# Iamdarika/Spotify_recommender

Hardware: AMD Instinct MI355X
Metric: queries/sec, cosine top-100 over a 10M x 12 fp32 catalogue (higher is better)
Workload: dtype f32 (every score is the exact fp32 chain; a 12 B/row 8-bit replica only rules rows out); 1 GPU; 10000000 synthetic tracks x 12 fp32 features, top-100, 1 MI355X (BASELINE configs[2], HBM-roofline run); rows=10000000, topn=100, rows_per_gpu=10000000, lanes=2, seed=12345, generator=torch.rand(seed) uniform[0,1) on device

## Files before the change

### include/mi355rec_diag.h

```cpp
#ifndef MI355REC_DIAG_H
#define MI355REC_DIAG_H

#include "mi355rec.h"

#ifdef __cplusplus
extern "C" {
#endif

typedef struct {
    int64_t rows;
    int64_t row_base;
    int32_t device;
    int32_t compute_units;
    int32_t grid_blocks;
    int32_t block_threads;
    int64_t bytes_per_query;
    float last_scan_ms;
    float last_merge_ms;
    float last_pass_ms;
    int32_t batched_grid_blocks;
    float batched_margin;
    int64_t replica_bytes_per_query;
    int32_t replica_active;
    int32_t replica_grid_blocks;
    float replica_build_ms;
    float replica_margin_single;
    float replica_margin_multi;
    int64_t replica_single_bytes_per_query;
    int32_t replica_single_row_bytes;
    int32_t lone_fused_queries;
    int64_t route_fp32;
    int64_t route_fp16;
    int64_t route_q8;
    int64_t route_q8_lone;
    int64_t route_multi_fp32;
    int64_t route_multi_fp16;
    int64_t route_multi_q8;
    int64_t route_mfma_two_pass;
    int64_t route_exact_queue;
    int32_t device_bytes_per_row;
    int64_t stream_pair_launches;
} mi355rec_stats_t;

#define MI355REC_BUILD_EXPERIMENTS 1
#define MI355REC_BUILD_PHASE_CLOCK 2
#define MI355REC_BUILD_TEST_HOOKS 4
int mi355rec_build_flags(void);

int mi355rec_device_count(void);

const char* mi355rec_last_global_error(void);

#define MI355REC_CREATE_NO_REPLICA 1
int mi355rec_create_ex(const float* feats_host, int64_t n, int dim, int device, int64_t row_base, int flags,
                       mi355rec_t** out);
int mi355rec_create_device_ex(const float* feats_dev, int64_t n, int dim, int device, int64_t row_base, int flags,
                              mi355rec_t** out);

#define MI355REC_REPLICA_AUTO 0
#define MI355REC_REPLICA_OFF 1
#define MI355REC_REPLICA_ON 2
#define MI355REC_REPLICA_FP16 3
int mi355rec_set_replica(mi355rec_t* h, int mode);
int mi355rec_rebuild_replica(mi355rec_t* h);
int mi355rec_replica_counters(mi355rec_t* h, int64_t* scans, int64_t* rescored_rows);

#define MI355REC_SAMPLE_AUTO 0
#define MI355REC_SAMPLE_STRIDED 1
#define MI355REC_SAMPLE_BUCKETED 2
#define MI355REC_SAMPLE_AUTO_MIN_ROWS 6000000
int mi355rec_set_sample(mi355rec_t* h, int mode);

#define MI355REC_PAIRING_AUTO 0
#define MI355REC_PAIRING_OFF 1
#define MI355REC_PAIRING_ON 2
#define MI355REC_PAIRING_AUTO_MIN_ROWS 2500000
int mi355rec_set_stream_pairing(mi355rec_t* h, int mode);
typedef struct {
    int64_t base_rows;
    int32_t regions;
    int32_t centroids;
    int64_t bytes;
    int64_t stride_rows;
    int64_t centroid_stride;
    int32_t picks;
    int32_t mode;
    int32_t last_used;
    float build_ms;
} mi355rec_bucket_sample_info_t;
int mi355rec_bucket_sample_info(const mi355rec_t* h, mi355rec_bucket_sample_info_t* out);
int mi355rec_bucket_sample_rows(mi355rec_t* h, int32_t* rows_out, int32_t* region_tab_out);

int mi355rec_lane_status(const mi355rec_t* h, int* stream_attempts, int* overlaps_parent);

int mi355rec_stats(const mi355rec_t* h, mi355rec_stats_t* out);
int mi355rec_stats_sized(const mi355rec_t* h, void* out, size_t out_size, size_t* written);


int mi355rec_scores_row(mi355rec_t* h, int64_t local_row, float* out_host);

int mi355rec_scores(mi355rec_t* h, const float* query12, float* out_host);

int mi355rec_row_ptr(mi355rec_t* h, int64_t local_row, const float** out_dev);
int mi355rec_enqueue_ptr_keys(mi355rec_t* h, const float* query12_dev, int64_t exclude_global, int topn,
                              mi355rec_key_t* out_keys_dev, int64_t* out_idx_dev, float* out_score_dev,
                              void* stream);
int mi355rec_enqueue_ptr_keys_streamed(mi355rec_t* h, const float* query12_dev, int64_t exclude_global,
                                       int topn, mi355rec_key_t* out_keys_dev, void* stream);

int mi355rec_batch_pointers_ok(const mi355rec_t* h, int topn);
int mi355rec_enqueue_batch_mixed_keys(mi355rec_t* h, const float* queries, const float* const* query_ptrs_dev,
                                      const int64_t* exclude_global, int batch, int topn,
                                      mi355rec_key_t* out_keys_dev, void* stream);
int mi355rec_enqueue_batch_mixed_keys_streamed(mi355rec_t* h, const float* queries, const float* const* query_ptrs_dev,
                                               const int64_t* exclude_global, int batch, int topn,
                                               mi355rec_key_t* out_keys_dev, void* stream);

#define MI355REC_BATCH_AUTO 0
#define MI355REC_BATCH_MULTI 1
#define MI355REC_BATCH_MFMA 2
#define MI355REC_BATCH_HALF 3
#define MI355REC_BATCH_Q8 4
int mi355rec_batched_pass2_pairs(mi355rec_t* h, int64_t* pairs_done, int64_t* pairs_total);

#define MI355REC_BATCH_MFMA_NOSKIP 5
int mi355rec_set_batch_path(mi355rec_t* h, int path);

int mi355rec_batched_last_counters(mi355rec_t* h, int32_t* special_rows,
                                   int32_t* queued_queries, int64_t* candidates_total,
                                   int32_t* candidates_max);

int mi355rec_enqueue_merge_keys(mi355rec_t* h, const mi355rec_key_t* lists_dev,
                                int n_lists, int list_len, int topn,
                                mi355rec_key_t* out_keys_dev,
                                int64_t* out_idx_dev, float* out_score_dev,
                                void* stream);

int mi355rec_enqueue_merge_keys_batch(mi355rec_t* h, const mi355rec_key_t* lists_dev,
                                      int n_lists, int list_len, int64_t list_stride,
                                      int64_t query_stride, int batch, int topn,
                                      mi355rec_key_t* out_keys_dev, int64_t* out_idx_dev,
                                      float* out_score_dev, void* stream);

int mi355rec_enqueue_scores(mi355rec_t* h, int64_t local_row,
                            const float* query12, float* out_scores_dev,
                            void* stream);

int mi355rec_enqueue_stream_probe(mi355rec_t* h, uint32_t* sink_dev, void* stream);
#define MI355REC_PROBE_FP32_ROWS 0
#define MI355REC_PROBE_FP16_REPLICA 1
#define MI355REC_PROBE_Q8_REPLICA 2
int mi355rec_enqueue_stream_probe_of(mi355rec_t* h, int which, uint32_t* sink_dev, void* stream);

int mi355rec_set_timing(mi355rec_t* h, int enabled);

int mi355rec_fetch_row(mi355rec_t* h, int64_t local_row, float* out12_host);
int mi355rec_fetch_rows(mi355rec_t* h, const int64_t* local_rows, int64_t count, float* out_host);


int mi355rec_create_sharded(const float* feats_host, int64_t n, int dim, int n_devices,
                            mi355rec_sharded_t** out);
int mi355rec_auto_shards(int64_t n, int visible_devices);
int mi355rec_sharded_placement(const mi355rec_sharded_t* h);

int mi355rec_create_sharded_on(const float* feats_host, int64_t n, int dim, const int* devices,
                               int n_shards, mi355rec_sharded_t** out);

int mi355rec_sharded_set_transport(mi355rec_sharded_t* h, int transport);

int mi355rec_sharded_info(const mi355rec_sharded_t* h, int* n_shards, int* transport,
                          int64_t* rows, int* devices_out, int64_t* shard_rows_out);

int mi355rec_sharded_set_timing(mi355rec_sharded_t* h, int enabled);
int mi355rec_sharded_shard_stats(const mi355rec_sharded_t* h, int shard, mi355rec_stats_t* out);
int mi355rec_sharded_set_replica(mi355rec_sharded_t* h, int mode);

int mi355rec_sharded_rows_by_pointer(const mi355rec_sharded_t* h);
const char* mi355rec_sharded_note(const mi355rec_sharded_t* h);

int mi355rec_sharded_scores_row(mi355rec_sharded_t* h, int64_t global_row, float* out_host);

int mi355rec_sharded_set_window(mi355rec_sharded_t* h, int window);
int mi355rec_sharded_set_window_mode(mi355rec_sharded_t* h, int batched);
int mi355rec_sharded_stream_stats(const mi355rec_sharded_t* h, int64_t* queries, int64_t* exchanges,
                                  int64_t* host_ns);

int mi355rec_sharded_rccl_ranks(const mi355rec_sharded_t* h, int* comms, int* ranks, int* ranks_agree);

#define MI355REC_MAX_LABELS 1024
int mi355rec_set_labels(mi355rec_t* h, const int32_t* labels_host, int64_t n);
int mi355rec_query_row_topn_labels(mi355rec_t* h, int64_t local_row, const int32_t* labels, int n_labels, int topn,
                                   int64_t* out_idx, float* out_score, int* out_count);
int mi355rec_query_topn_labels(mi355rec_t* h, const float* query12, int64_t exclude_global, const int32_t* labels,
                               int n_labels, int topn, int64_t* out_idx, float* out_score, int* out_count);
int mi355rec_label_counters(const mi355rec_t* h, int64_t* queries, int64_t* rows_scanned);
int mi355rec_sharded_set_labels(mi355rec_sharded_t* h, const int32_t* labels_host, int64_t n);
int mi355rec_sharded_query_row_topn_labels(mi355rec_sharded_t* h, int64_t global_row, const int32_t* labels, int n_labels,
                                           int topn, int64_t* out_idx, float* out_score, int* out_count);
int mi355rec_sharded_query_topn_labels(mi355rec_sharded_t* h, const float* query12, int64_t exclude_global,
                                       const int32_t* labels, int n_labels, int topn, int64_t* out_idx, float* out_score,
                                       int* out_count);

#define MI355REC_MAX_PLAYLIST 32
#define MI355REC_MAX_EXCLUDE 1024
int mi355rec_query_mean_topn(mi355rec_t* h, const float* queries, int k, const int64_t* exclude_global, int n_exclude, int topn,
                             int64_t* out_idx, float* out_score, int* out_count);
int mi355rec_query_playlist_topn(mi355rec_t* h, const int64_t* local_rows, int k, const int64_t* exclude_global, int n_exclude,
                                 int topn, int64_t* out_idx, float* out_score, int* out_count);
int mi355rec_playlist_counters(const mi355rec_t* h, int64_t* queries, int64_t* rows_exact);
int mi355rec_sharded_query_mean_topn(mi355rec_sharded_t* h, const float* queries, int k, const int64_t* exclude_global,
                                     int n_exclude, int topn, int64_t* out_idx, float* out_score, int* out_count);
int mi355rec_sharded_query_playlist_topn(mi355rec_sharded_t* h, const int64_t* global_rows, int k, const int64_t* exclude_global,
                                         int n_exclude, int topn, int64_t* out_idx, float* out_score, int* out_count);

typedef struct {
    uint32_t active;
    float lo[12];
    float hi[12];
} mi355rec_filter_t;
int mi355rec_query_mean_topn_where(mi355rec_t* h, const float* queries, int k, const int64_t* exclude_global, int n_exclude,
                                   const mi355rec_filter_t* filter, int topn, int64_t* out_idx, float* out_score, int* out_count);
int mi355rec_query_playlist_topn_where(mi355rec_t* h, const int64_t* local_rows, int k, const int64_t* exclude_global,
                                       int n_exclude, const mi355rec_filter_t* filter, int topn, int64_t* out_idx, float* out_score,
                                       int* out_count);
int mi355rec_sharded_query_mean_topn_where(mi355rec_sharded_t* h, const float* queries, int k, const int64_t* exclude_global,
                                           int n_exclude, const mi355rec_filter_t* filter, int topn, int64_t* out_idx,
                                           float* out_score, int* out_count);
int mi355rec_sharded_query_playlist_topn_where(mi355rec_sharded_t* h, const int64_t* global_rows, int k,
                                               const int64_t* exclude_global, int n_exclude, const mi355rec_filter_t* filter,
// ... 237 lines not shown
```

### spotify_recommender_amd/capi.py

```python
from __future__ import annotations

import ctypes
import os
from ctypes import POINTER, c_char_p, c_float, c_int, c_int32, c_int64, c_uint32, c_uint64, c_void_p
from pathlib import Path

PKG = Path(__file__).resolve().parent
LIB_PATH = Path(os.environ["MI355REC_LIB"]) if os.environ.get("MI355REC_LIB") else PKG / "libmi355rec.so"

DIM = 12
MAX_TOPN_FAST = 1024
BATCH_AUTO, BATCH_MULTI, BATCH_MFMA, BATCH_HALF, BATCH_Q8, BATCH_MFMA_NOSKIP = 0, 1, 2, 3, 4, 5
REPLICA_AUTO, REPLICA_OFF, REPLICA_ON, REPLICA_FP16 = 0, 1, 2, 3
SAMPLE_AUTO, SAMPLE_STRIDED, SAMPLE_BUCKETED = 0, 1, 2
SAMPLE_AUTO_MIN_ROWS = 6_000_000
PAIRING_AUTO, PAIRING_OFF, PAIRING_ON = 0, 1, 2
PAIRING_AUTO_MIN_ROWS = 2_500_000
TRANSPORT_PEER, TRANSPORT_RCCL = 1, 2
PLACEMENT_AUTO, PLACEMENT_SHARDED, PLACEMENT_REPLICATED, PLACEMENT_CPU = 0, 1, 2, 3
CREATE_NO_REPLICA = 1
DEBUG_HANDOFF_POISON, DEBUG_HANDOFF_DROP_STORES, DEBUG_HANDOFF_NO_LAST_RIDER = 1, 2, 4
BUILD_EXPERIMENTS, BUILD_PHASE_CLOCK, BUILD_TEST_HOOKS = 1, 2, 4
PROBE_FP32_ROWS, PROBE_FP16_REPLICA, PROBE_Q8_REPLICA = 0, 1, 2

OK = 0
ERR_INVALID_ARG = -1
ERR_NO_DEVICE = -2
ERR_HIP = -3
ERR_OUT_OF_MEMORY = -4
MAX_LABELS = 1024
MAX_PLAYLIST = 32
MAX_EXCLUDE = 1024
FEATURE_NAMES = ("danceability", "energy", "key", "loudness", "mode", "speechiness", "acousticness", "instrumentalness",
                 "liveness", "valence", "tempo", "genre_id")


class Filter(ctypes.Structure):
    _fields_ = [("active", c_uint32), ("lo", c_float * DIM), ("hi", c_float * DIM)]


PQ_DIVERSE, PQ_CAPPED, PQ_PRIOR = 1, 2, 4
MAX_PRIOR_WEIGHT = 4.0
MAX_FEATURE_SCALE = 1024.0


class PlaylistQuery(ctypes.Structure):
    _fields_ = [("size", c_uint32), ("flags", c_uint32), ("members", c_void_p), ("rows", c_void_p), ("weights", c_void_p),
                ("exclude_global", c_void_p), ("filter", POINTER(Filter)), ("labels", c_void_p), ("k", c_int32),
                ("n_exclude", c_int32), ("n_labels", c_int32), ("topn", c_int32), ("lambda_", c_float), ("pool", c_int32),
                ("max_per_group", c_int32), ("prior_weight", c_float)]


class PlaylistResult(ctypes.Structure):
    _fields_ = [("out_idx", c_void_p), ("out_score", c_void_p), ("out_mmr", c_void_p), ("out_count", POINTER(c_int)),
                ("out_pool_rows", POINTER(c_int))]


class DistanceQuery(ctypes.Structure):
    _fields_ = [("size", c_uint32), ("flags", c_uint32), ("members", c_void_p), ("rows", c_void_p), ("exclude_global", c_void_p),
                ("filter", POINTER(Filter)), ("labels", c_void_p), ("k", c_int32), ("n_exclude", c_int32), ("n_labels", c_int32),
                ("topn", c_int32)]


class DistanceResult(ctypes.Structure):
    _fields_ = [("out_idx", c_void_p), ("out_distance", c_void_p), ("out_count", POINTER(c_int))]


class AnyOfQuery(ctypes.Structure):
    _fields_ = [("size", c_uint32), ("flags", c_uint32), ("members", c_void_p), ("rows", c_void_p), ("exclude_global", c_void_p),
                ("filter", POINTER(Filter)), ("labels", c_void_p), ("k", c_int32), ("n_exclude", c_int32), ("n_labels", c_int32),
                ("topn", c_int32)]


class AnyOfResult(ctypes.Structure):
    _fields_ = [("out_idx", c_void_p), ("out_score", c_void_p), ("out_member", c_void_p), ("out_count", POINTER(c_int))]


class ManhattanQuery(ctypes.Structure):
    _fields_ = [("size", c_uint32), ("flags", c_uint32), ("members", c_void_p), ("rows", c_void_p), ("exclude_global", c_void_p),
                ("filter", POINTER(Filter)), ("labels", c_void_p), ("k", c_int32), ("n_exclude", c_int32), ("n_labels", c_int32),
                ("topn", c_int32)]


class ManhattanResult(ctypes.Structure):
    _fields_ = [("out_idx", c_void_p), ("out_distance", c_void_p), ("out_count", POINTER(c_int))]


ROWSET_EXCLUDE, ROWSET_ONLY = 0, 1
MAX_CANDIDATES = 1 << 20


class RequestExt(ctypes.Structure):
    _fields_ = [("size", c_uint32), ("rowset_mode", c_uint32), ("feature_scales", c_void_p), ("rowset", c_void_p)]


class BucketSampleInfo(ctypes.Structure):
    _fields_ = [("base_rows", c_int64), ("regions", c_int32), ("centroids", c_int32), ("bytes", c_int64), ("stride_rows", c_int64),
                ("centroid_stride", c_int64), ("picks", c_int32), ("mode", c_int32), ("last_used", c_int32), ("build_ms", c_float)]


class UpdateInfo(ctypes.Structure):
    _fields_ = [("size", c_uint32), ("last_ms", c_float), ("calls", c_int64), ("rows", c_int64), ("rows_since_snapshot", c_int64)]


class Stats(ctypes.Structure):
    _fields_ = [
        ("rows", c_int64),
        ("row_base", c_int64),
        ("device", c_int32),
        ("compute_units", c_int32),
        ("grid_blocks", c_int32),
        ("block_threads", c_int32),
        ("bytes_per_query", c_int64),
        ("last_scan_ms", c_float),
        ("last_merge_ms", c_float),
        ("last_pass_ms", c_float),
        ("batched_grid_blocks", c_int32),
        ("batched_margin", c_float),
        ("replica_bytes_per_query", c_int64),
        ("replica_active", c_int32),
        ("replica_grid_blocks", c_int32),
        ("replica_build_ms", c_float),
        ("replica_margin_single", c_float),
        ("replica_margin_multi", c_float),
        ("replica_single_bytes_per_query", c_int64),
        ("replica_single_row_bytes", c_int32),
        ("lone_fused_queries", c_int32),
        ("route_fp32", c_int64),
        ("route_fp16", c_int64),
        ("route_q8", c_int64),
        ("route_q8_lone", c_int64),
        ("route_multi_fp32", c_int64),
        ("route_multi_fp16", c_int64),
        ("route_multi_q8", c_int64),
        ("route_mfma_two_pass", c_int64),
        ("route_exact_queue", c_int64),
        ("device_bytes_per_row", c_int32),
        ("stream_pair_launches", c_int64),
    ]


SIGNATURES = {
    "mi355rec_build_flags": (c_int, []),
    "mi355rec_device_count": (c_int, []),
    "mi355rec_last_global_error": (c_char_p, []),
    "mi355rec_create": (c_int, [c_void_p, c_int64, c_int, c_int, c_int64, POINTER(c_void_p)]),
    "mi355rec_create_device": (c_int, [c_void_p, c_int64, c_int, c_int, c_int64, POINTER(c_void_p)]),
    "mi355rec_create_ex": (c_int, [c_void_p, c_int64, c_int, c_int, c_int64, c_int, POINTER(c_void_p)]),
    "mi355rec_create_device_ex": (c_int, [c_void_p, c_int64, c_int, c_int, c_int64, c_int, POINTER(c_void_p)]),
    "mi355rec_destroy": (None, [c_void_p]),
    "mi355rec_last_error": (c_char_p, [c_void_p]),
    "mi355rec_create_lane": (c_int, [c_void_p, POINTER(c_void_p)]),
    "mi355rec_own_stream": (c_void_p, [c_void_p]),
    "mi355rec_lane_status": (c_int, [c_void_p, POINTER(c_int), POINTER(c_int)]),
    "mi355rec_stats": (c_int, [c_void_p, POINTER(Stats)]),
    "mi355rec_stats_sized": (c_int, [c_void_p, c_void_p, ctypes.c_size_t, POINTER(ctypes.c_size_t)]),
    "mi355rec_scores_row": (c_int, [c_void_p, c_int64, c_void_p]),
    "mi355rec_scores": (c_int, [c_void_p, c_void_p, c_void_p]),
    "mi355rec_query_row_topn": (c_int, [c_void_p, c_int64, c_int, c_void_p, c_void_p, POINTER(c_int)]),
    "mi355rec_query_topn": (c_int, [c_void_p, c_void_p, c_int64, c_int, c_void_p, c_void_p, POINTER(c_int)]),
    "mi355rec_query_batch_topn": (c_int, [c_void_p, c_void_p, c_int, c_void_p, c_int, c_void_p, c_void_p, c_void_p]),
    "mi355rec_enqueue_row_keys": (c_int, [c_void_p, c_int64, c_int, c_void_p, c_void_p]),
    "mi355rec_enqueue_query_keys": (c_int, [c_void_p, c_void_p, c_int64, c_int, c_void_p, c_void_p]),
    "mi355rec_enqueue_row_keys_streamed": (c_int, [c_void_p, c_int64, c_int, c_void_p, c_void_p]),
    "mi355rec_enqueue_query_keys_streamed": (c_int, [c_void_p, c_void_p, c_int64, c_int, c_void_p, c_void_p]),
    "mi355rec_enqueue_flush": (c_int, [c_void_p, c_void_p]),
    "mi355rec_enqueue_batch_keys": (c_int, [c_void_p, c_void_p, c_void_p, c_int, c_int, c_void_p, c_void_p]),
    "mi355rec_enqueue_batch_keys_streamed": (c_int, [c_void_p, c_void_p, c_void_p, c_int, c_int, c_void_p, c_void_p]),
    "mi355rec_batch_pointers_ok": (c_int, [c_void_p, c_int]),
    "mi355rec_enqueue_batch_mixed_keys": (c_int, [c_void_p, c_void_p, c_void_p, c_void_p, c_int, c_int, c_void_p, c_void_p]),
    "mi355rec_enqueue_batch_mixed_keys_streamed": (c_int, [c_void_p, c_void_p, c_void_p, c_void_p, c_int, c_int, c_void_p, c_void_p]),
    "mi355rec_enqueue_batch_keys_dev": (c_int, [c_void_p, c_void_p, c_void_p, c_int, c_int, c_void_p, c_void_p]),
    "mi355rec_set_batch_path": (c_int, [c_void_p, c_int]),
    "mi355rec_set_replica": (c_int, [c_void_p, c_int]),
    "mi355rec_rebuild_replica": (c_int, [c_void_p]),
    "mi355rec_replica_counters": (c_int, [c_void_p, POINTER(c_int64), POINTER(c_int64)]),
    "mi355rec_set_sample": (c_int, [c_void_p, c_int]),
    "mi355rec_set_stream_pairing": (c_int, [c_void_p, c_int]),
    "mi355rec_bucket_sample_info": (c_int, [c_void_p, c_void_p]),
    "mi355rec_bucket_sample_rows": (c_int, [c_void_p, c_void_p, c_void_p]),
    "mi355rec_batched_last_counters": (c_int, [c_void_p, POINTER(c_int32), POINTER(c_int32), POINTER(c_int64),
                                               POINTER(c_int32)]),
    "mi355rec_batched_pass2_pairs": (c_int, [c_void_p, POINTER(c_int64), POINTER(c_int64)]),
    "mi355rec_enqueue_merge_keys": (c_int, [c_void_p, c_void_p, c_int, c_int, c_int, c_void_p, c_void_p, c_void_p, c_void_p]),
    "mi355rec_enqueue_merge_keys_batch": (c_int, [c_void_p, c_void_p, c_int, c_int, c_int64, c_int64, c_int, c_int,
                                                  c_void_p, c_void_p, c_void_p, c_void_p]),
    "mi355rec_enqueue_scores": (c_int, [c_void_p, c_int64, c_void_p, c_void_p, c_void_p]),
    "mi355rec_enqueue_stream_probe": (c_int, [c_void_p, c_void_p, c_void_p]),
    "mi355rec_enqueue_stream_probe_of": (c_int, [c_void_p, c_int, c_void_p, c_void_p]),
    "mi355rec_set_timing": (c_int, [c_void_p, c_int]),
    "mi355rec_fetch_row": (c_int, [c_void_p, c_int64, c_void_p]),
    "mi355rec_create_sharded": (c_int, [c_void_p, c_int64, c_int, c_int, POINTER(c_void_p)]),
    "mi355rec_create_sharded_on": (c_int, [c_void_p, c_int64, c_int, c_void_p, c_int, POINTER(c_void_p)]),
    "mi355rec_create_placed": (c_int, [c_void_p, c_int64, c_int, c_void_p, c_int, c_int, POINTER(c_void_p)]),
    "mi355rec_auto_shards": (c_int, [c_int64, c_int]),
    "mi355rec_sharded_placement": (c_int, [c_void_p]),
    "mi355rec_sharded_destroy": (None, [c_void_p]),
    "mi355rec_sharded_last_error": (c_char_p, [c_void_p]),
    "mi355rec_sharded_set_transport": (c_int, [c_void_p, c_int]),
    "mi355rec_sharded_info": (c_int, [c_void_p, POINTER(c_int), POINTER(c_int), POINTER(c_int64), c_void_p, c_void_p]),
    "mi355rec_sharded_query_row_topn": (c_int, [c_void_p, c_int64, c_int, c_void_p, c_void_p, POINTER(c_int)]),
    "mi355rec_sharded_query_topn": (c_int, [c_void_p, c_void_p, c_int64, c_int, c_void_p, c_void_p, POINTER(c_int)]),
    "mi355rec_sharded_query_batch_topn": (c_int, [c_void_p, c_void_p, c_int, c_void_p, c_int, c_void_p, c_void_p, c_void_p]),
    "mi355rec_sharded_scores_row": (c_int, [c_void_p, c_int64, c_void_p]),
    "mi355rec_row_ptr": (c_int, [c_void_p, c_int64, POINTER(c_void_p)]),
    "mi355rec_enqueue_ptr_keys": (c_int, [c_void_p, c_void_p, c_int64, c_int, c_void_p, c_void_p, c_void_p, c_void_p]),
    "mi355rec_enqueue_ptr_keys_streamed": (c_int, [c_void_p, c_void_p, c_int64, c_int, c_void_p, c_void_p]),
    "mi355rec_sharded_set_timing": (c_int, [c_void_p, c_int]),
    "mi355rec_sharded_shard_stats": (c_int, [c_void_p, c_int, POINTER(Stats)]),
    "mi355rec_sharded_set_replica": (c_int, [c_void_p, c_int]),
    "mi355rec_sharded_rows_by_pointer": (c_int, [c_void_p]),
    "mi355rec_sharded_note": (c_char_p, [c_void_p]),
    "mi355rec_sharded_set_window": (c_int, [c_void_p, c_int]),
    "mi355rec_sharded_set_window_mode": (c_int, [c_void_p, c_int]),
    "mi355rec_sharded_enqueue_row": (c_int, [c_void_p, c_int64, c_int, POINTER(c_int64)]),
    "mi355rec_sharded_enqueue_query": (c_int, [c_void_p, c_void_p, c_int64, c_int, POINTER(c_int64)]),
    "mi355rec_sharded_enqueue_flush": (c_int, [c_void_p]),
    "mi355rec_sharded_wait": (c_int, [c_void_p, c_int64, c_void_p, c_void_p, POINTER(c_int)]),
    "mi355rec_sharded_stream_stats": (c_int, [c_void_p, POINTER(c_int64), POINTER(c_int64), POINTER(c_int64)]),
    "mi355rec_debug_handoff": (c_int, [c_void_p, c_int]),
    "mi355rec_sharded_rccl_ranks": (c_int, [c_void_p, POINTER(c_int), POINTER(c_int), POINTER(c_int)]),
    "mi355rec_set_labels": (c_int, [c_void_p, c_void_p, c_int64]),
    "mi355rec_query_row_topn_labels": (c_int, [c_void_p, c_int64, c_void_p, c_int, c_int, c_void_p, c_void_p, POINTER(c_int)]),
    "mi355rec_query_topn_labels": (c_int, [c_void_p, c_void_p, c_int64, c_void_p, c_int, c_int, c_void_p, c_void_p, POINTER(c_int)]),
    "mi355rec_label_counters": (c_int, [c_void_p, POINTER(c_int64), POINTER(c_int64)]),
    "mi355rec_sharded_set_labels": (c_int, [c_void_p, c_void_p, c_int64]),
    "mi355rec_sharded_query_row_topn_labels": (c_int, [c_void_p, c_int64, c_void_p, c_int, c_int, c_void_p, c_void_p,
                                                       POINTER(c_int)]),
    "mi355rec_sharded_query_topn_labels": (c_int, [c_void_p, c_void_p, c_int64, c_void_p, c_int, c_int, c_void_p, c_void_p,
                                                   POINTER(c_int)]),
    "mi355rec_query_mean_topn": (c_int, [c_void_p, c_void_p, c_int, c_void_p, c_int, c_int, c_void_p, c_void_p, POINTER(c_int)]),
    "mi355rec_query_playlist_topn": (c_int, [c_void_p, c_void_p, c_int, c_void_p, c_int, c_int, c_void_p, c_void_p, POINTER(c_int)]),
    "mi355rec_playlist_counters": (c_int, [c_void_p, POINTER(c_int64), POINTER(c_int64)]),
    "mi355rec_sharded_query_mean_topn": (c_int, [c_void_p, c_void_p, c_int, c_void_p, c_int, c_int, c_void_p, c_void_p,
                                                 POINTER(c_int)]),
    "mi355rec_sharded_query_playlist_topn": (c_int, [c_void_p, c_void_p, c_int, c_void_p, c_int, c_int, c_void_p, c_void_p,
                                                     POINTER(c_int)]),
    "mi355rec_query_mean_topn_where": (c_int, [c_void_p, c_void_p, c_int, c_void_p, c_int, c_void_p, c_int, c_void_p, c_void_p,
                                               POINTER(c_int)]),
    "mi355rec_query_playlist_topn_where": (c_int, [c_void_p, c_void_p, c_int, c_void_p, c_int, c_void_p, c_int, c_void_p, c_void_p,
                                                   POINTER(c_int)]),
    "mi355rec_sharded_query_mean_topn_where": (c_int, [c_void_p, c_void_p, c_int, c_void_p, c_int, c_void_p, c_int, c_void_p,
                                                       c_void_p, POINTER(c_int)]),
    "mi355rec_sharded_query_playlist_topn_where": (c_int, [c_void_p, c_void_p, c_int, c_void_p, c_int, c_void_p, c_int, c_void_p,
                                                           c_void_p, POINTER(c_int)]),
    "mi355rec_query_mean_topn_weighted": (c_int, [c_void_p, c_void_p, c_void_p, c_int, c_void_p, c_int, c_void_p, c_int, c_void_p,
                                                  c_void_p, POINTER(c_int)]),
    "mi355rec_query_playlist_topn_weighted": (c_int, [c_void_p, c_void_p, c_void_p, c_int, c_void_p, c_int, c_void_p, c_int,
                                                      c_void_p, c_void_p, POINTER(c_int)]),
    "mi355rec_sharded_query_mean_topn_weighted": (c_int, [c_void_p, c_void_p, c_void_p, c_int, c_void_p, c_int, c_void_p, c_int,
                                                          c_void_p, c_void_p, POINTER(c_int)]),
    "mi355rec_sharded_query_playlist_topn_weighted": (c_int, [c_void_p, c_void_p, c_void_p, c_int, c_void_p, c_int, c_void_p,
                                                              c_int, c_void_p, c_void_p, POINTER(c_int)]),
    "mi355rec_query_mean_topn_diverse": (c_int, [c_void_p, c_void_p, c_void_p, c_int, c_void_p, c_int, c_void_p, c_float, c_int, c_int,
                                                 c_void_p, c_void_p, c_void_p, POINTER(c_int)]),
    "mi355rec_query_playlist_topn_diverse": (c_int, [c_void_p, c_void_p, c_void_p, c_int, c_void_p, c_int, c_void_p, c_float, c_int,
                                                     c_int, c_void_p, c_void_p, c_void_p, POINTER(c_int)]),
    "mi355rec_sharded_query_mean_topn_diverse": (c_int, [c_void_p, c_void_p, c_void_p, c_int, c_void_p, c_int, c_void_p, c_float, c_int,
                                                         c_int, c_void_p, c_void_p, c_void_p, POINTER(c_int)]),
    "mi355rec_sharded_query_playlist_topn_diverse": (c_int, [c_void_p, c_void_p, c_void_p, c_int, c_void_p, c_int, c_void_p, c_float,
                                                             c_int, c_int, c_void_p, c_void_p, c_void_p, POINTER(c_int)]),
    "mi355rec_fetch_rows": (c_int, [c_void_p, c_void_p, c_int64, c_void_p]),
    "mi355rec_set_groups": (c_int, [c_void_p, c_void_p, c_int64]),
    "mi355rec_sharded_set_groups": (c_int, [c_void_p, c_void_p, c_int64]),
    "mi355rec_query_mean_topn_capped": (c_int, [c_void_p, c_void_p, c_void_p, c_int, c_void_p, c_int, c_void_p, c_float, c_int, c_int, c_int,
        c_void_p, c_void_p, c_void_p, POINTER(c_int), POINTER(c_int)]),
    "mi355rec_query_playlist_topn_capped": (c_int, [c_void_p, c_void_p, c_void_p, c_int, c_void_p, c_int, c_void_p, c_float, c_int, c_int, c_int,
        c_void_p, c_void_p, c_void_p, POINTER(c_int), POINTER(c_int)]),
    "mi355rec_sharded_query_mean_topn_capped": (c_int, [c_void_p, c_void_p, c_void_p, c_int, c_void_p, c_int, c_void_p, c_float, c_int, c_int, c_int,
        c_void_p, c_void_p, c_void_p, POINTER(c_int), POINTER(c_int)]),
    "mi355rec_sharded_query_playlist_topn_capped": (c_int, [c_void_p, c_void_p, c_void_p, c_int, c_void_p, c_int, c_void_p, c_float, c_int, c_int, c_int,
        c_void_p, c_void_p, c_void_p, POINTER(c_int), POINTER(c_int)]),
    "mi355rec_set_priors": (c_int, [c_void_p, c_void_p, c_int64]),
    "mi355rec_sharded_set_priors": (c_int, [c_void_p, c_void_p, c_int64]),
    "mi355rec_query_playlist_request": (c_int, [c_void_p, POINTER(PlaylistQuery), POINTER(PlaylistResult)]),
    "mi355rec_sharded_query_playlist_request": (c_int, [c_void_p, POINTER(PlaylistQuery), POINTER(PlaylistResult)]),
    "mi355rec_query_distance_request": (c_int, [c_void_p, POINTER(DistanceQuery), POINTER(DistanceResult)]),
    "mi355rec_sharded_query_distance_request": (c_int, [c_void_p, POINTER(DistanceQuery), POINTER(DistanceResult)]),
    "mi355rec_query_playlist_request_scaled": (c_int, [c_void_p, POINTER(PlaylistQuery), c_void_p, POINTER(PlaylistResult)]),
    "mi355rec_query_distance_request_scaled": (c_int, [c_void_p, POINTER(DistanceQuery), c_void_p, POINTER(DistanceResult)]),
    "mi355rec_sharded_query_playlist_request_scaled": (c_int, [c_void_p, POINTER(PlaylistQuery), c_void_p, POINTER(PlaylistResult)]),
    "mi355rec_sharded_query_distance_request_scaled": (c_int, [c_void_p, POINTER(DistanceQuery), c_void_p, POINTER(DistanceResult)]),
    "mi355rec_rowset_create": (c_int, [c_void_p, c_void_p, c_int64, POINTER(c_void_p)]),
    "mi355rec_sharded_rowset_create": (c_int, [c_void_p, c_void_p, c_int64, POINTER(c_void_p)]),
    "mi355rec_rowset_add": (c_int, [c_void_p, c_void_p, c_int64]),
    "mi355rec_rowset_count": (c_int64, [c_void_p]),
    "mi355rec_rowset_destroy": (None, [c_void_p]),
    "mi355rec_query_playlist_request_ext": (c_int, [c_void_p, POINTER(PlaylistQuery), POINTER(RequestExt), POINTER(PlaylistResult)]),
    "mi355rec_query_distance_request_ext": (c_int, [c_void_p, POINTER(DistanceQuery), POINTER(RequestExt), POINTER(DistanceResult)]),
    "mi355rec_sharded_query_playlist_request_ext": (c_int, [c_void_p, POINTER(PlaylistQuery), POINTER(RequestExt), POINTER(PlaylistResult)]),
    "mi355rec_sharded_query_distance_request_ext": (c_int, [c_void_p, POINTER(DistanceQuery), POINTER(RequestExt), POINTER(DistanceResult)]),
# ... 87 lines not shown
```

### spotify_recommender_amd/csrc/engine_single.hip.h

```cpp
#pragma once

#include "engine_state.hip.h"

#include <type_traits>

namespace {

int flush_mstream(mi355rec* h, hipStream_t s);

bool use_half(const mi355rec* h, const uint64_t* upper_dev) {
    if (!h->d_half || upper_dev || h->replica_mode == MI355REC_REPLICA_OFF) return false;
    return h->replica_mode == MI355REC_REPLICA_ON || h->replica_mode == MI355REC_REPLICA_FP16 || h->n >= kHalfAutoMinRows;
}

bool use_q8(const mi355rec* h) { return h->d_q8 && h->replica_mode != MI355REC_REPLICA_FP16; }

int single_kind(const mi355rec* h, const uint64_t* upper_dev) {
    if (!use_half(h, upper_dev)) return kFp32;
    return use_q8(h) ? kQ8 : kFp16;
}

bool q8_exact_sample(const mi355rec* h) { return h->geom[kQ8].iters >= 3; }

constexpr int kBucketAutoMaxTopn = 128;
// ... 280 lines not shown
}

int wait_done(mi355rec* h, uint32_t want) {
    for (uint64_t spins = 1;; ++spins) {
        if (__atomic_load_n(h->h_done, __ATOMIC_ACQUIRE) == want) return MI355REC_OK;
        __builtin_ia32_pause();
        if ((spins & 0x3ffff) == 0) {
            const hipError_t e = hipStreamQuery(h->stream);
            if (e == hipSuccess) {
                if (__atomic_load_n(h->h_done, __ATOMIC_ACQUIRE) == want) return MI355REC_OK;
                return fail(h, MI355REC_ERR_HIP, "the query's stream drained without its completion word");
            }
            if (e != hipErrorNotReady) return fail(h, MI355REC_ERR_HIP, "hipStreamQuery: %s", hipGetErrorString(e));
        }
    }
}

int ensure_streamed_alloc(mi355rec* h);
int ensure_streamed(mi355rec* h) {
    if (h->streamed_ready) return MI355REC_OK;
    const int rc = ensure_streamed_alloc(h);
    if (rc != MI355REC_OK) {
        for (int i = 0; i < 2; ++i) {
            if (h->d_stream_lists[i]) (void)hipFree(h->d_stream_lists[i]);
            h->d_stream_lists[i] = nullptr;
        }
        return rc;
    }
    h->streamed_ready = true;
    return MI355REC_OK;
}

int ensure_streamed_alloc(mi355rec* h) {
    const size_t words = static_cast<size_t>(most(h, &ScanGeom::sgrid)) * kMaxTopK;
    for (int i = 0; i < 2; ++i) HIP_TRY(h, hipMalloc(&h->d_stream_lists[i], sizeof(uint64_t) * words));
    return MI355REC_OK;
}

int merge_pending(mi355rec* h, hipStream_t s) {
    h->pending = false;
    return enqueue_merge(h, h->d_stream_lists[h->pending_buf], h->pending_lists, h->pending_topn, h->pending_topn,
                         h->pending_out, nullptr, nullptr, s);
}

int launch_stashed(mi355rec* h, hipStream_t s, bool with_next, const float* next_ptr, const float* next_q,
                   int64_t next_exclude, int next_topn, int next_buf, uint32_t next_epoch_tag);

int drain_pairs(mi355rec* h, hipStream_t s);

int flush_single_stream(mi355rec* h, hipStream_t s);
int flush_streamed(mi355rec* h, hipStream_t s) {
    const int rc = drain_pairs(h, s);
    return rc ? rc : flush_single_stream(h, s);
}

int flush_single_stream(mi355rec* h, hipStream_t s) {
    if (h->stashed.has) {
        const int rc = launch_stashed(h, s, false, nullptr, nullptr, -1, 0, 0, 0u);
        if (rc) return rc;
    }
    return h->pending ? merge_pending(h, s) : MI355REC_OK;
}

int launch_stashed(mi355rec* h, hipStream_t s, bool with_next, const float* next_ptr, const float* next_q,
                   int64_t next_exclude, int next_topn, int next_buf, uint32_t next_epoch_tag) {
    auto& st = h->stashed;
    const bool next_bucketed = with_next && use_bucket(h, st.kind, next_topn, h->geom_bucket.riders > 0);
    const ScanGeom& g = stream_geom(h, st.kind, next_bucketed);
    if (st.kind == kFp32 && h->pending && h->pending_topn > kRideTopnMax) {
        const int rc = merge_pending(h, s);
        if (rc) return rc;
    }
    ScanLaunch L;
    L.kind = st.kind;
    L.streamed = true;
    const int buf = h->pending ? 1 - h->pending_buf : 0;
    if (h->pending) L.prev = PrevMerge{h->d_stream_lists[h->pending_buf], h->pending_lists, h->pending_topn, h->pending_out};
    int scanners = g.sgrid;
    L.iters = g.siters;
    if (with_next && (g.riders > 0 || g.nbhd)) {
        scanners = g.r_scan;
        L.iters = g.r_iters;
        L.next = make_next_seed(h, st.kind, g.riders, g.nbhd, next_ptr, next_q, next_exclude, next_topn, next_epoch_tag,
                                h->d_stream_seed[next_buf], g.hoists ? h->d_stream_ctl + next_buf : nullptr, h->ctl_done[next_buf],
                                next_bucketed);
    }
    L.grid = scanners + 1 + L.next.n_wgs + L.next.nbhd;
    L.lists = h->d_stream_lists[buf];
    L.sample = h->d_stream_seed[st.seed_buf];
    L.bound = st.cutoff_ready ? &h->d_stream_ctl[st.seed_buf].cutoff : nullptr;
    L.epoch = st.epoch;
    L.bucketed = st.bucketed;
    const int rc = launch_scan(h, L, st.qptr, st.q, st.exclude, st.topn, s);
    if (rc) return rc;
    if (L.next.ctl) h->ctl_done[next_buf] += static_cast<unsigned>(L.next.n_wgs);
    h->pending = true;
    h->pending_buf = buf;
    h->pending_topn = st.topn;
    h->pending_out = st.out;
    h->pending_lists = scanners;
    st.has = false;
    return MI355REC_OK;
}

int enqueue_streamed_single(mi355rec* h, const float* qptr, const float* query12, int64_t exclude_global, int topn,
                            uint64_t* out_keys, hipStream_t s, int accepted_kind = -1) {
    int rc = MI355REC_OK;
    if (MI355REC_EXP_FLAG("MI355REC_EXP_RIDE_NOMERGE") && h->pending) {
        rc = flush_single_stream(h, s);
        if (rc) return rc;
    }
    const int kind = accepted_kind >= 0 ? accepted_kind : single_kind(h, nullptr);
    int seed_buf = 0;
    bool sampled = false, nbhd_taken = false;
    const uint32_t epoch = next_epoch(h);
    const bool bucketed = use_bucket(h, kind, topn, h->stashed.has && h->stashed.kind == kind && h->geom_bucket.riders > 0);
    const ScanGeom& ng = stream_geom(h, kind, bucketed);
    if (kind == kQ8) h->last_sample = bucketed ? MI355REC_SAMPLE_BUCKETED : MI355REC_SAMPLE_STRIDED;
    if (h->stashed.has) {
        seed_buf = 1 - h->stashed.seed_buf;
        const bool same = h->stashed.kind == kind;
        sampled = same && ng.riders > 0;
        nbhd_taken = same && ng.nbhd;
        rc = launch_stashed(h, s, same, qptr, query12, exclude_global, topn, seed_buf, epoch);
        if (rc) return rc;
    }
    bool bound_ready = sampled && ng.hoists;
    if (!sampled) {
        if (kind == kFp32) {
            if (h->n >= kF32LoneSeedMinRows)
                bound_ready = enqueue_f32_seed(h, qptr, query12, exclude_global, topn, h->d_stream_seed[seed_buf], h->d_stream_ctl + seed_buf,
                                               &h->ctl_done[seed_buf], epoch, s);
        } else if (!nbhd_taken) {
            enqueue_half_seed(h, kind, qptr, query12, exclude_global, topn, h->d_stream_seed[seed_buf], epoch, s, bucketed);
        }
        HIP_TRY(h, hipGetLastError());
    }
    auto& st = h->stashed;
    st.has = true;
    st.qptr = qptr;
    if (!qptr) std::memcpy(st.q, query12, sizeof st.q);
    st.exclude = exclude_global;
    st.topn = topn;
    st.out = out_keys;
    st.seed_buf = seed_buf;
    st.epoch = epoch;
    st.kind = kind;
    st.bucketed = bucketed;
    st.cutoff_ready = bound_ready;
    return MI355REC_OK;
}

bool pairing_on(const mi355rec* h) {
    if (h->pairing == MI355REC_PAIRING_ON) return true;
    if (h->pairing == MI355REC_PAIRING_OFF) return false;
    return h->n >= MI355REC_PAIRING_AUTO_MIN_ROWS;
}
bool pairs_open(const mi355rec* h) { return h->pairs.waiting || h->pairs.has_first || h->pairs.pending; }

void free_pairs(mi355rec* h) {
    auto& P = h->pairs;
    for (int i = 0; i < 4; ++i) {
        if (P.lists[i]) (void)hipFree(P.lists[i]);
        if (P.seed[i]) (void)hipFree(P.seed[i]);
        P.lists[i] = nullptr;
        P.seed[i] = nullptr;
    }
    if (P.ctl) (void)hipFree(P.ctl);
    P.ctl = nullptr;
    P.ready = false;
}

int ensure_pairs_alloc(mi355rec* h) {
    auto& P = h->pairs;
    const size_t words = static_cast<size_t>(h->geom[kQ8].grid > 0 ? h->geom[kQ8].grid : 1) * kPairMaxTopk;
    for (int i = 0; i < 4; ++i) {
        HIP_TRY(h, hipMalloc(&P.lists[i], sizeof(uint64_t) * words));
        HIP_TRY(h, hipMalloc(&P.seed[i], sizeof(unsigned long long) * kSampleSlots));
        HIP_TRY(h, hipMemset(P.seed[i], 0, sizeof(unsigned long long) * kSampleSlots));
    }
    HIP_TRY(h, hipMalloc(&P.ctl, sizeof(SeedCtl) * 4));
    HIP_TRY(h, hipMemset(P.ctl, 0, sizeof(SeedCtl) * 4));
    return MI355REC_OK;
}
int ensure_pairs(mi355rec* h) {
    if (h->pairs.ready) return MI355REC_OK;
    const int rc = ensure_pairs_alloc(h);
    if (rc != MI355REC_OK) {
        free_pairs(h);
        return rc;
    }
    for (unsigned& d : h->pairs.ctl_done) d = 0u;
    h->pairs.ready = true;
    return MI355REC_OK;
}

int merge_pair_pending(mi355rec* h, hipStream_t s) {
    auto& P = h->pairs;
    P.pending = false;
    for (int x = 0; x < 2; ++x) {
        const int rc = enqueue_merge(h, P.lists[2 * P.pending_set + x], P.pending_lists, P.pending_topn, P.pending_topn, P.pending_out[x],
                                     nullptr, nullptr, s);
        if (rc) return rc;
    }
    return MI355REC_OK;
}

int launch_pair(mi355rec* h, hipStream_t s, const mi355rec::Stashed* next, bool next_bucketed) {
    auto& P = h->pairs;
    const mi355rec::Stashed& a = P.wait[0];
    const mi355rec::Stashed& b = P.wait[1];
    const int topn = a.topn;
    if (P.pending) {
        const uint64_t* lo = P.pending_out[0] < P.pending_out[1] ? P.pending_out[0] : P.pending_out[1];
        const uint64_t* hi = P.pending_out[0] < P.pending_out[1] ? P.pending_out[1] : P.pending_out[0];
        if (hi < lo + P.pending_topn) {
            const int rc = merge_pair_pending(h, s);
            if (rc) return rc;
        }
    }
    const ScanGeom& g = stream_geom(h, kQ8, next != nullptr && next_bucketed);
    const bool riders = next != nullptr && (g.riders > 0 || g.nbhd);
    const int extra = 2 + (riders ? 2 * (g.riders + (g.nbhd ? 1 : 0)) : 0);
    const int64_t tiles = (h->n + Q8PairConfig::kTileRows - 1) / Q8PairConfig::kTileRows;
    int64_t scanners = g.grid - extra;
    if (scanners > kRideMaxLists - 1) scanners = kRideMaxLists - 1;
    if (scanners > tiles) scanners = tiles;
    if (scanners < 1) scanners = 1;
    const int iters = static_cast<int>((tiles + scanners - 1) / scanners);
    const int set = P.pending ? 1 - P.pending_set : 0;
    Q8PairSide side;
    std::memset(&side, 0, sizeof side);
    side.prev[0] = side.prev[1] = no_prev_merge();
    if (P.pending)
        for (int x = 0; x < 2; ++x) side.prev[x] = PrevMerge{P.lists[2 * P.pending_set + x], P.pending_lists, P.pending_topn, P.pending_out[x]};
    if (riders)
        for (int x = 0; x < 2; ++x)
            side.next[x] = make_next_seed(h, kQ8, g.riders, g.nbhd, next[x].qptr, next[x].q, next[x].exclude, next[x].topn, next[x].epoch,
                                          P.seed[next[x].seed_buf], g.hoists ? P.ctl + next[x].seed_buf : nullptr,
                                          P.ctl_done[next[x].seed_buf], next_bucketed);
    Q8PairArg arg[2];
    const mi355rec::Stashed* const q[2] = {&a, &b};
    for (int x = 0; x < 2; ++x) {
        std::memset(&arg[x], 0, sizeof arg[x]);
        arg[x].qarg = make_query_arg(h, q[x]->qptr, q[x]->q);
        arg[x].query_ptr = q[x]->qptr;
        arg[x].exclude_global = q[x]->exclude;
        arg[x].block_lists = P.lists[2 * set + x];
        arg[x].seed_vals = P.seed[q[x]->seed_buf];
        arg[x].cutoff_ready = q[x]->cutoff_ready ? &P.ctl[q[x]->seed_buf].cutoff : nullptr;
        arg[x].n_seed = q8_seed_count(h, q[x]->bucketed);
        arg[x].epoch = q[x]->epoch;
    }
    const dim3 grid(static_cast<unsigned>(scanners + 2 + 2 * (side.next[0].n_wgs + side.next[0].nbhd)));
    LAUNCH_TIMED(h, h->ev_scan, h->n_scan_pairs, h->scan_launches, scan_q8_kernel_pair<Q8PairConfig>, grid, dim3(Q8PairConfig::kBlock), s,
                 h->d_feats, h->d_q8, h->n, iters, h->row_base, arg[0], arg[1], topn, h->d_half_rescored, side);
    HIP_TRY(h, hipGetLastError());
    h->half_scans += 2;
    h->q8_scans += 2;
    h->routes.q8 += 2;
    ++h->stream_pair_launches;
    for (int x = 0; x < 2; ++x)
        if (side.next[x].ctl) P.ctl_done[next[x].seed_buf] += static_cast<unsigned>(side.next[x].n_wgs);
    P.pending = true;
    P.pending_set = set;
    P.pending_lists = static_cast<int>(scanners);
    P.pending_topn = topn;
    P.pending_out[0] = a.out;
    P.pending_out[1] = b.out;
    P.waiting = false;
    return MI355REC_OK;
}

int drain_pairs(mi355rec* h, hipStream_t s) {
    auto& P = h->pairs;
    if (P.waiting) {
        const int rc = launch_pair(h, s, nullptr, false);
        if (rc) return rc;
    }
    if (P.pending) {
        const int rc = merge_pair_pending(h, s);
        if (rc) return rc;
    }
    if (P.has_first) {
        const mi355rec::Stashed f = P.first;
        P.has_first = false;
        return enqueue_streamed_single(h, f.qptr, f.q, f.exclude, f.topn, f.out, s, h->d_q8 ? f.kind : -1);
    }
    return MI355REC_OK;
}

int enqueue_streamed(mi355rec* h, const float* qptr, const float* query12, int64_t exclude_global, int topn,
                     uint64_t* out_keys, hipStream_t s) {
    int rc = ensure_streamed(h);
    if (rc) return rc;
    rc = flush_mstream(h, s);
    if (rc) return rc;
    auto& P = h->pairs;
    bool pair = single_kind(h, nullptr) == kQ8 && topn <= kPairMaxTopk && pairing_on(h);
    if (pair && ensure_pairs(h) != MI355REC_OK) {
        (void)hipGetLastError();
        pair = false;
    }
    if (pair && P.has_first && (P.first.topn != topn || P.first_replica_mode != h->replica_mode || P.first_sample_mode != h->sample_mode)) {
        rc = drain_pairs(h, s);
        if (rc) return rc;
    }
    if (!pair) {
        if (pairs_open(h)) {
            rc = drain_pairs(h, s);
            if (rc) return rc;
        }
        return enqueue_streamed_single(h, qptr, query12, exclude_global, topn, out_keys, s);
    }
    if (h->stashed.has || h->pending) {
        rc = flush_single_stream(h, s);
        if (rc) return rc;
    }
    mi355rec::Stashed x;
    x.has = true;
    x.qptr = qptr;
    if (!qptr) std::memcpy(x.q, query12, sizeof x.q);
    x.exclude = exclude_global;
    x.topn = topn;
    x.out = out_keys;
    x.kind = kQ8;
    if (!P.has_first) {
        P.first = x;
        P.has_first = true;
        P.first_replica_mode = h->replica_mode;
        P.first_sample_mode = h->sample_mode;
        return MI355REC_OK;
    }
    const int set = P.waiting ? 1 - (P.wait[0].seed_buf >> 1) : 0;
    const bool bucketed = use_bucket(h, kQ8, topn, h->geom_bucket.riders > 0);
    const ScanGeom& ng = stream_geom(h, kQ8, bucketed);
    mi355rec::Stashed nx[2] = {P.first, x};
    for (int i = 0; i < 2; ++i) {
        nx[i].seed_buf = 2 * set + i;
        nx[i].epoch = next_epoch(h);
        nx[i].bucketed = bucketed;
    }
    h->last_sample = bucketed ? MI355REC_SAMPLE_BUCKETED : MI355REC_SAMPLE_STRIDED;
    bool sampled = false;
    if (P.waiting) {
        sampled = ng.riders > 0;
        rc = launch_pair(h, s, nx, bucketed);
        if (rc) return rc;
    }
    if (!sampled) {
        for (int i = 0; i < 2; ++i)
            enqueue_half_seed(h, kQ8, nx[i].qptr, nx[i].q, nx[i].exclude, topn, P.seed[nx[i].seed_buf], nx[i].epoch, s, bucketed);
        HIP_TRY(h, hipGetLastError());
    }
    for (int i = 0; i < 2; ++i) {
        nx[i].cutoff_ready = sampled && ng.hoists;
        P.wait[i] = nx[i];
    }
    P.waiting = true;
    P.has_first = false;
    return MI355REC_OK;
}

}
```

### spotify_recommender_amd/csrc/engine_state.hip.h

```cpp
#pragma once

#if defined(MI355REC_EXPERIMENTS) && !defined(MI355REC_TEST_HOOKS)
#define MI355REC_TEST_HOOKS 1
#endif
#include "mi355rec_diag.h"

#include <hip/hip_runtime.h>
#include <hip/hip_ext.h>

#include <cstdarg>
#include <cstdio>
#include <cstdlib>
#include <atomic>
#include <chrono>
#include <new>
#include <cstring>
#include <string>
#include <vector>

#include "batched.hip.h"
#include "bucket_sample.h"
#include "kernels.hip.h"
#include "replica.hip.h"
#include "replica_q8.hip.h"
// ... 12 lines not shown
        if (hipGetDevice(&prev) != hipSuccess) prev = -1;
        if (prev != dev) ok = (hipSetDevice(dev) == hipSuccess);
    }
    ~DeviceGuard() {
        int cur = -1;
        if (prev >= 0 && hipGetDevice(&cur) == hipSuccess && cur != prev) (void)hipSetDevice(prev);
    }
};

constexpr int kTimingPairs = 8192;
constexpr int kDirectResultSlots = 2048;

using ScanConfig = DefaultScanCfg;
using MultiConfig = DefaultMultiCfg;
using HalfConfig = DefaultHalfCfg;
using Q8Config = DefaultQ8Cfg;
using Q8PairConfig = DefaultQ8PairCfg;
constexpr int kRideTopnMax = 640;
constexpr int64_t kReplicaMinRows = 65536;
constexpr int64_t kHalfAutoMinRows = 1000000;
constexpr int kScanBlock = ScanConfig::kBlock;
constexpr int kScanTileRows = ScanConfig::kTileRows;
constexpr int64_t kF32SampleMinRows = 2000000;
constexpr int kFp32 = 0, kFp16 = 1, kQ8 = 2;
const float* const kNoQueryPtr = nullptr;

struct ScanGeom {
    int grid = 0, iters = 0;
    int sgrid = 0, siters = 0;
    int seed_grid = 0;
    int64_t seed_stride = 0;
    int riders = 0;
    bool nbhd = false;
    bool hoists = false;
    int r_scan = 0, r_iters = 0;
};

}

struct BucketBufs {
    void* q8 = nullptr;
    int32_t* rows = nullptr;
    float* centroids = nullptr;
    int32_t* region_tab = nullptr;
    int regions = 0, n_centroids = 0;
    int64_t base_rows = 0;
    int64_t stride = 0;
    int64_t centroid_stride = 0;
    float build_ms = 0.f;
    int64_t bytes() const {
        return rows ? static_cast<int64_t>(regions) * 2048 * (12 + 4) + static_cast<int64_t>(n_centroids) * 48 + static_cast<int64_t>(regions) * 8 : 0;
    }
};

struct mi355rec_labels;
struct mi355rec_playlist;

struct RowSide {
    mi355rec_labels* labels = nullptr;
    int32_t* d_groups = nullptr;
    float* d_priors = nullptr;
};

struct mi355rec {
    int device = 0;
    int64_t n = 0;
    int64_t row_base = 0;
    const float* d_feats = nullptr;
    float* owned_feats = nullptr;
    struct SharedRows {
        std::atomic<int> refs{1};
        void* owned_feats = nullptr;
        void* d_half = nullptr;
        void* d_q8 = nullptr;
        BucketBufs bsample;
        float margin_mix = 0.0f, margin_mfma = 0.0f;
        RowSide side;
        std::vector<mi355rec*> members;
    };
    SharedRows* shared = nullptr;
    bool is_lane = false;
    int lane_stream_attempts = 0;
    int lane_overlaps = -1;
    RowSide own_side;
    RowSide* side = &own_side;
    int64_t label_queries = 0;
    int64_t label_rows_scanned = 0;
    mi355rec_playlist* playlist = nullptr;
    int64_t playlist_queries = 0;

    int cus = 0;
    ScanGeom geom[3];
    ScanGeom geom_bucket;
    BucketBufs bsample;
    int sample_mode = 0;
    int last_sample = 0;
    int mgrid = 0;
    int64_t mrows_per_block = 0;
    int miters = 0;

    uint64_t* d_block_lists = nullptr;
    uint64_t* d_stream_lists[2] = {nullptr, nullptr};
    bool streamed_ready = false;
    bool pending = false;
    int pending_buf = 0, pending_topn = 0;
    uint64_t* pending_out = nullptr;
    uint4* d_half = nullptr;
    unsigned long long* d_half_seed = nullptr;
    SeedCtl* d_lone_ctl = nullptr;
    unsigned lone_ctl_done = 0;
    unsigned long long* d_half_mseed = nullptr;
    unsigned long long* d_half_mcuts = nullptr;
    SeedCtl* d_half_mctl = nullptr;
    unsigned half_mctl_done = 0;
    uint32_t epoch_ctr = 0;
    unsigned ctl_done[2] = {0u, 0u};
    unsigned mctl_done[2] = {0u, 0u};
    unsigned lone_base[9] = {0u, 0u, 0u, 0u, 0u, 0u, 0u, 0u, 0u};
    int dbg_skip_regions = 0;
    bool dbg_no_last = false;
    unsigned long long* d_half_rescored = nullptr;
    unsigned* d_lone_ctr = nullptr;
    int64_t lone_fused = 0;
    int64_t half_scans = 0;
    int64_t q8_scans = 0;
    struct Routes {
        int64_t fp32 = 0, fp16 = 0, q8 = 0, q8_lone = 0, multi_fp32 = 0, multi_fp16 = 0, multi_q8 = 0, mfma_two_pass = 0;
    } routes;
    uint4* d_q8 = nullptr;
    float* d_anchor = nullptr;
    int replica_mode = 0;
    bool replica_allowed = true;
    float replica_build_ms = 0.f;
    float margin_mix = kBqMarginFlush;
    float margin_mfma = kBqMarginFlush;
    int pending_lists = 0;
    struct Stashed {
        bool has = false;
        const float* qptr = nullptr;
        float q[kDim] = {0};
        int64_t exclude = -1;
        int topn = 0;
        uint64_t* out = nullptr;
        int seed_buf = 0;
        uint32_t epoch = 0;
        int kind = 0;
        bool cutoff_ready = false;
        bool bucketed = false;
    } stashed;
    unsigned long long* d_stream_seed[2] = {nullptr, nullptr};
    SeedCtl* d_stream_ctl = nullptr;
    int pairing = 0;
    int64_t stream_pair_launches = 0;
    struct Pairs {
        bool ready = false;
        uint64_t* lists[4] = {nullptr, nullptr, nullptr, nullptr};
        unsigned long long* seed[4] = {nullptr, nullptr, nullptr, nullptr};
        SeedCtl* ctl = nullptr;
        unsigned ctl_done[4] = {0u, 0u, 0u, 0u};
        bool waiting = false;
        Stashed wait[2];
        bool has_first = false;
        Stashed first;
        int first_replica_mode = 0, first_sample_mode = 0;
        bool pending = false;
        int pending_set = 0, pending_lists = 0, pending_topn = 0;
        uint64_t* pending_out[2] = {nullptr, nullptr};
    } pairs;
    bool mstream_ready = false;
    uint64_t* d_mstream_lists[2] = {nullptr, nullptr};
    unsigned long long* d_mstream_seed[2] = {nullptr, nullptr};
    unsigned long long* d_mstream_cuts = nullptr;
    SeedCtl* d_mstream_ctl = nullptr;
    struct MStash {
        bool has = false;
        HalfMultiArg arg;
        int nq = 0, topn = 0;
        uint64_t* out = nullptr;
        int seed_buf = 0;
        uint32_t epoch = 0;
        bool cuts_ready = false;
    } mstash;
    struct MPending {
        bool has = false;
        int buf = 0, nq = 0, topn = 0, n_lists = 0;
        uint64_t* out = nullptr;
    } mpending;
    uint32_t* d_seed_vals = nullptr;
    uint64_t* d_seed_keys = nullptr;

    hipStream_t last_stream = nullptr;
    bool has_last_stream = false;
    hipEvent_t order_ev = nullptr;

    hipStream_t stream = nullptr;
    size_t slot_cap = 0;
    uint64_t* d_keys = nullptr;
    int64_t* d_idx = nullptr;
    float* d_score = nullptr;
    int64_t* h_idx = nullptr;
    float* h_score = nullptr;
    int64_t* hd_idx = nullptr;
    float* hd_score = nullptr;
    uint32_t* h_done = nullptr;
    uint32_t* hd_done = nullptr;
    uint32_t done_seq = 0;
    float* d_scores_full = nullptr;

    struct Batched {
        bool ready = false;
        int grid = 0;
        int grid2 = 0;
        int occ1 = 0, occ2 = 0;
        float margin = kBqMarginFlush;
        int step1 = 4;
        int qgrid = 0, qiters = 0;
        uint32_t* bfrag = nullptr;
        float* qnorm = nullptr;
        float* qthr = nullptr;
        uint32_t* qflags = nullptr;
        int* cand_count = nullptr;
        uint64_t* cand_rows = nullptr;
        int* cand_examined = nullptr;
        int cand_cap = 0;
        int* counters = nullptr;
        uint32_t* special_rows = nullptr;
        uint32_t* nb_vals = nullptr;
        volatile int* h_nb_report = nullptr;
        int* d_nb_report = nullptr;
        int nb_skipped = 0;
        bool nb_sparse = false;
        bool nbhd_this_chunk = false;
        float* gmax = nullptr;
        uint4* tile_max = nullptr;
        int64_t tile_max_tiles = 0;
        int* queue = nullptr;
        uint64_t* qlists = nullptr;
        float* d_queries = nullptr;
        long long* d_exclude = nullptr;
        static constexpr int kSlots = 4;
        float* h_queries[kSlots] = {nullptr, nullptr, nullptr, nullptr};
        long long* h_exclude[kSlots] = {nullptr, nullptr, nullptr, nullptr};
        hipEvent_t slot_ev[kSlots] = {nullptr, nullptr, nullptr, nullptr};
        bool slot_used[kSlots] = {false, false, false, false};
        int next_slot = 0;
        int launches = 0;
        int last_count = 0;
    } bq;
    int batch_path = 0;

    struct Update {
        int64_t calls = 0, rows = 0;
        int64_t rows_since_snapshot = 0;
        float last_ms = 0.f;
        int64_t cap = 0;
        char* h_stage = nullptr;
        char* d_stage = nullptr;
    } upd;

    bool timing = false;
    int timing_stride = 1;
    int scan_launches = 0, merge_launches = 0;
    std::vector<hipEvent_t> ev_scan, ev_merge, ev_pass;
    int n_scan_pairs = 0, n_merge_pairs = 0, n_pass_pairs = 0;
    int pass_launches = 0;
    float last_scan_ms = 0.f, last_merge_ms = 0.f, last_pass_ms = 0.f;

    std::string err;
};

namespace {

int fail(mi355rec* h, int code, const char* fmt, ...) {
    char buf[512];
    va_list ap;
    va_start(ap, fmt);
    vsnprintf(buf, sizeof buf, fmt, ap);
    va_end(ap);
    if (h) h->err = buf;
    g_last_error = buf;
    return code;
}

uint32_t next_epoch(mi355rec* h) {
    if (++h->epoch_ctr == 0u) ++h->epoch_ctr;
    return h->epoch_ctr;
}

#define HIP_TRY(h, expr)                                                          \
    do {                                                                          \
        hipError_t e_ = (expr);                                                   \
        if (e_ != hipSuccess)                                                     \
            return fail((h), e_ == hipErrorOutOfMemory ? MI355REC_ERR_OUT_OF_MEMORY \
                                                       : MI355REC_ERR_HIP,        \
                        "%s failed: %s (%s:%d)", #expr, hipGetErrorString(e_),   \
                        __FILE__, __LINE__);                                      \
    } while (0)

int order_stream(mi355rec* h, hipStream_t s) {
    if (h->has_last_stream && h->last_stream != s) {
        if (hipEventRecord(h->order_ev, h->last_stream) == hipSuccess) {
            HIP_TRY(h, hipStreamWaitEvent(s, h->order_ev, 0));
        } else {
            (void)hipGetLastError();
        }
    }
    h->last_stream = s;
    h->has_last_stream = true;
    return MI355REC_OK;
}

int most(const mi355rec* h, int ScanGeom::*field) {
    int m = 0;
    for (const ScanGeom& g : h->geom)
        if (g.*field > m) m = g.*field;
    return m;
}

int sync_api_begin(mi355rec* h) { return order_stream(h, h->stream); }

// ... 478 lines not shown
```

### spotify_recommender_amd/csrc/mi355rec.hip

```cpp
#include "engine_batch.hip.h"
#include "engine_sync.hip.h"
#include "engine_labels.hip.h"
#include "engine_playlist.hip.h"
#include "engine_diverse.hip.h"
#include "engine_update.hip.h"

extern "C" {

int mi355rec_build_flags(void) {
    int flags = 0;
#ifdef MI355REC_EXPERIMENTS
    flags |= MI355REC_BUILD_EXPERIMENTS;
#endif
#ifdef MI355REC_PHASE_CLOCK
    flags |= MI355REC_BUILD_PHASE_CLOCK;
#endif
#ifdef MI355REC_TEST_HOOKS
    flags |= MI355REC_BUILD_TEST_HOOKS;
#endif
    return flags;
}

int mi355rec_device_count(void) {
    int count = 0;
// ... 166 lines not shown
        return rc;
    }
    lane->is_lane = true;
    lane->replica_allowed = parent->replica_allowed;
    lane->replica_mode = parent->replica_mode;
    lane->batch_path = parent->batch_path;
    lane->pairing = parent->pairing;
    if (parent->d_half) {
        const int src = alloc_replica_state(lane);
        if (src != MI355REC_OK) {
            parent->err = lane->err;
            mi355rec_destroy(lane);
            return src;
        }
        if (hipStreamSynchronize(lane->stream) != hipSuccess) {
            mi355rec_destroy(lane);
            return fail(parent, MI355REC_ERR_HIP, "hipStreamSynchronize(lane)");
        }
    }
    if (!parent->shared) {
        mi355rec::SharedRows* group = new (std::nothrow) mi355rec::SharedRows();
        if (group) {
            try {
                group->members.reserve(8);
                group->members.push_back(parent);
            } catch (const std::bad_alloc&) {
                delete group;
                group = nullptr;
            }
        }
        if (!group) {
            mi355rec_destroy(lane);
            return fail(parent, MI355REC_ERR_OUT_OF_MEMORY, "out of host memory for the lane group");
        }
        parent->shared = group;
        group->owned_feats = parent->owned_feats;
        group->d_half = parent->d_half;
        group->d_q8 = parent->d_q8;
        group->bsample = parent->bsample;
        group->margin_mix = parent->margin_mix;
        group->margin_mfma = parent->margin_mfma;
        group->side = parent->own_side;
        parent->own_side = RowSide();
        parent->side = &group->side;
    }
    try {
        parent->shared->members.push_back(lane);
    } catch (const std::bad_alloc&) {
        mi355rec_destroy(lane);
        return fail(parent, MI355REC_ERR_OUT_OF_MEMORY, "out of host memory for the lane group");
    }
    parent->shared->refs.fetch_add(1);
    lane->shared = parent->shared;
    lane->upd.rows_since_snapshot = parent->upd.rows_since_snapshot;
    lane->side = &parent->shared->side;
    lane->d_half = parent->d_half;
    lane->d_q8 = parent->d_q8;
    lane->bsample = parent->bsample;
    lane->sample_mode = parent->sample_mode;
    lane->margin_mix = parent->margin_mix;
    lane->margin_mfma = parent->margin_mfma;
    lane->replica_build_ms = 0.f;
    constexpr int kLaneStreamAttempts = 6;
    for (int attempt = 1; attempt <= kLaneStreamAttempts; ++attempt) {
        lane->lane_stream_attempts = attempt;
        lane->lane_overlaps = streams_overlap(parent, lane);
        if (lane->lane_overlaps != 0 || attempt == kLaneStreamAttempts) break;
        hipStream_t fresh = nullptr;
        if (hipStreamCreateWithFlags(&fresh, hipStreamNonBlocking) != hipSuccess) break;
        (void)hipStreamDestroy(lane->stream);
        lane->stream = fresh;
    }
    preallocate_stream_state(lane);
    *out = lane;
    return MI355REC_OK;
}

const char* mi355rec_last_error(const mi355rec_t* h) {
    return h ? h->err.c_str() : g_last_error.c_str();
}

int mi355rec_set_timing(mi355rec_t* h, int enabled) {
    if (!h) return fail(nullptr, MI355REC_ERR_INVALID_ARG, "null handle");
    h->timing = enabled != 0;
    h->timing_stride = enabled > 1 ? enabled : 1;
    h->n_scan_pairs = 0;
    h->n_merge_pairs = 0;
    h->n_pass_pairs = 0;
    h->scan_launches = 0;
    h->merge_launches = 0;
    h->pass_launches = 0;
    return MI355REC_OK;
}

int mi355rec_stats(const mi355rec_t* hc, mi355rec_stats_t* out) {
    mi355rec_t* h = const_cast<mi355rec_t*>(hc);
    if (!h || !out) return fail(h, MI355REC_ERR_INVALID_ARG, "null argument");
    DeviceGuard guard(h->device);
    auto avg = [&](std::vector<hipEvent_t>& evs, int pairs, float& last) {
        if (pairs <= 0) return;
        double sum = 0.0;
        int good = 0;
        for (int i = 0; i < pairs; ++i) {
            float ms = 0.f;
            if (hipEventSynchronize(evs[2 * i + 1]) == hipSuccess &&
                hipEventElapsedTime(&ms, evs[2 * i], evs[2 * i + 1]) == hipSuccess) {
                sum += ms;
                ++good;
            }
        }
        if (good) last = static_cast<float>(sum / good);
    };
    avg(h->ev_scan, h->n_scan_pairs, h->last_scan_ms);
    avg(h->ev_merge, h->n_merge_pairs, h->last_merge_ms);
    avg(h->ev_pass, h->n_pass_pairs, h->last_pass_ms);
    out->rows = h->n;
    out->row_base = h->row_base;
    out->device = h->device;
    out->compute_units = h->cus;
    out->grid_blocks = h->geom[kFp32].grid;
    out->block_threads = kScanBlock;
    out->bytes_per_query = h->n * kDim * static_cast<int64_t>(sizeof(float));
    out->last_scan_ms = h->last_scan_ms;
    out->last_merge_ms = h->last_merge_ms;
    out->last_pass_ms = h->last_pass_ms;
    out->batched_grid_blocks = h->bq.ready ? h->bq.grid : 0;
    out->batched_margin = h->bq.ready ? h->bq.margin : 0.0f;
    out->replica_bytes_per_query = h->d_half ? ((h->n + 1) / 2) * 48 : 0;
    out->replica_active = use_half(h, nullptr) ? 1 : 0;
    out->replica_grid_blocks = h->d_half ? h->geom[use_q8(h) ? kQ8 : kFp16].grid : 0;
    out->replica_build_ms = h->replica_build_ms;
    out->replica_margin_single = h->d_half ? h->margin_mix : 0.0f;
    out->replica_margin_multi = h->d_half ? h->margin_mfma : 0.0f;
    out->replica_single_row_bytes = !h->d_half ? 0 : (use_q8(h) ? 12 : 24);
    out->replica_single_bytes_per_query = !h->d_half ? 0 : (use_q8(h) ? ((h->n + 3) / 4) * 48 : ((h->n + 1) / 2) * 48);
    out->lone_fused_queries = static_cast<int32_t>(h->lone_fused & 0x7fffffff);
    out->route_fp32 = h->routes.fp32;
    out->route_fp16 = h->routes.fp16;
    out->route_q8 = h->routes.q8;
    out->route_q8_lone = h->routes.q8_lone;
    out->route_multi_fp32 = h->routes.multi_fp32;
    out->route_multi_fp16 = h->routes.multi_fp16;
    out->route_multi_q8 = h->routes.multi_q8;
    out->route_mfma_two_pass = h->routes.mfma_two_pass;
    out->route_exact_queue = 0;
    if (h->bq.ready) {
        int queued = 0;
        if (hipMemcpyAsync(&queued, h->bq.counters + 5, sizeof queued, hipMemcpyDeviceToHost, h->stream) == hipSuccess &&
            hipStreamSynchronize(h->stream) == hipSuccess)
            out->route_exact_queue = queued;
    }
    out->device_bytes_per_row = 48 + (h->d_half ? 24 : 0) + (h->d_q8 ? 12 : 0);
    out->stream_pair_launches = h->stream_pair_launches;
    return MI355REC_OK;
}

int mi355rec_stats_sized(const mi355rec_t* h, void* out, size_t out_size, size_t* written) {
    if (!out || out_size == 0) return fail(const_cast<mi355rec_t*>(h), MI355REC_ERR_INVALID_ARG, "null argument");
    mi355rec_stats_t full;
    std::memset(&full, 0, sizeof full);
    const int rc = mi355rec_stats(h, &full);
    if (rc) return rc;
    const size_t n = out_size < sizeof full ? out_size : sizeof full;
    std::memcpy(out, &full, n);
    if (written) *written = n;
    return MI355REC_OK;
}


namespace {

struct EnqueueCall {
    DeviceGuard guard;
    hipStream_t s;
    int rc;
    EnqueueCall(mi355rec* h, int topn, bool allow_rounds, void* stream)
        : guard(h->device), s(static_cast<hipStream_t>(stream)), rc(check_topn(h, topn, allow_rounds)) {
        if (!rc) rc = order_stream(h, s);
    }
};

static int answer_empty(mi355rec* h, mi355rec_key_t* out_keys_dev, size_t slots, hipStream_t s) {
    HIP_TRY(h, hipMemsetAsync(out_keys_dev, 0, sizeof(uint64_t) * slots, s));
    return MI355REC_OK;
}

}

int mi355rec_enqueue_row_keys(mi355rec_t* h, int64_t local_row, int topn,
                              mi355rec_key_t* out_keys_dev, void* stream) {
    if (!h || !out_keys_dev) return fail(h, MI355REC_ERR_INVALID_ARG, "null argument");
    if (local_row < 0 || local_row >= h->n)
        return fail(h, MI355REC_ERR_INVALID_ARG, "Invalid song index: %lld", (long long)local_row);
    EnqueueCall call(h, topn, true, stream);
    if (call.rc) return call.rc;
    return enqueue_query(h, h->d_feats + local_row * kDim, nullptr, h->row_base + local_row, topn, out_keys_dev, nullptr,
                         nullptr, call.s);
}

int mi355rec_enqueue_query_keys(mi355rec_t* h, const float* query12, int64_t exclude_global,
                                int topn, mi355rec_key_t* out_keys_dev, void* stream) {
    if (!h || !out_keys_dev || !query12) return fail(h, MI355REC_ERR_INVALID_ARG, "null argument");
    EnqueueCall call(h, topn, true, stream);
    if (call.rc) return call.rc;
    return enqueue_query(h, nullptr, query12, exclude_global, topn, out_keys_dev, nullptr, nullptr, call.s);
}

int mi355rec_enqueue_row_keys_streamed(mi355rec_t* h, int64_t local_row, int topn, mi355rec_key_t* out_keys_dev,
                                       void* stream) {
    if (!h || !out_keys_dev) return fail(h, MI355REC_ERR_INVALID_ARG, "null argument");
    if (local_row < 0 || local_row >= h->n)
        return fail(h, MI355REC_ERR_INVALID_ARG, "Invalid song index: %lld", (long long)local_row);
    EnqueueCall call(h, topn, false, stream);
    if (call.rc) return call.rc;
    return enqueue_streamed(h, h->d_feats + local_row * kDim, nullptr, h->row_base + local_row, topn, out_keys_dev, call.s);
}

int mi355rec_enqueue_query_keys_streamed(mi355rec_t* h, const float* query12, int64_t exclude_global, int topn,
                                         mi355rec_key_t* out_keys_dev, void* stream) {
    if (!h || !out_keys_dev || !query12) return fail(h, MI355REC_ERR_INVALID_ARG, "null argument");
    EnqueueCall call(h, topn, false, stream);
    if (call.rc) return call.rc;
    if (h->n < 1) return answer_empty(h, out_keys_dev, static_cast<size_t>(topn), call.s);
    return enqueue_streamed(h, nullptr, query12, exclude_global, topn, out_keys_dev, call.s);
}

int mi355rec_enqueue_batch_keys_streamed(mi355rec_t* h, const float* queries, const int64_t* exclude_global, int batch,
                                         int topn, mi355rec_key_t* out_keys_dev, void* stream) {
    if (!queries) return fail(h, MI355REC_ERR_INVALID_ARG, "null argument");
    return mi355rec_enqueue_batch_mixed_keys_streamed(h, queries, nullptr, exclude_global, batch, topn, out_keys_dev, stream);
}

int mi355rec_enqueue_batch_mixed_keys_streamed(mi355rec_t* h, const float* queries, const float* const* query_ptrs_dev,
                                               const int64_t* exclude_global, int batch, int topn,
                                               mi355rec_key_t* out_keys_dev, void* stream) {
    if (!h || !out_keys_dev || (!queries && !query_ptrs_dev)) return fail(h, MI355REC_ERR_INVALID_ARG, "null argument");
    if (batch < 1) return fail(h, MI355REC_ERR_INVALID_ARG, "batch must be positive");
    const bool streamable = h->n >= kBqMinRows && half_multi_ok(h, topn) && h->batch_path != MI355REC_BATCH_MULTI &&
                            h->batch_path != MI355REC_BATCH_MFMA && h->batch_path != MI355REC_BATCH_MFMA_NOSKIP;
    if (!streamable) {
        if (query_ptrs_dev) return mi355rec_enqueue_batch_mixed_keys(h, queries, query_ptrs_dev, exclude_global, batch, topn, out_keys_dev, stream);
        return mi355rec_enqueue_batch_keys(h, queries, exclude_global, batch, topn, out_keys_dev, stream);
    }
    EnqueueCall call(h, topn, false, stream);
    if (call.rc) return call.rc;
    hipStream_t s = call.s;
    int rc = flush_streamed(h, s);
    if (rc) return rc;
    for (int g0 = 0; g0 < batch; g0 += kHmQueries) {
        const int nq = batch - g0 < kHmQueries ? batch - g0 : kHmQueries;
        rc = enqueue_mstream(h, queries, query_ptrs_dev, exclude_global, g0, nq, topn, out_keys_dev + static_cast<size_t>(g0) * topn, s);
        if (rc) return rc;
    }
    return MI355REC_OK;
}


int mi355rec_batch_pointers_ok(const mi355rec_t* h, int topn) {
    return h && h->n >= kBqMinRows && half_multi_ok(h, topn) ? 1 : 0;
}

int mi355rec_enqueue_batch_mixed_keys(mi355rec_t* h, const float* queries, const float* const* query_ptrs_dev,
                                      const int64_t* exclude_global, int batch, int topn, mi355rec_key_t* out_keys_dev,
                                      void* stream) {
    if (!h || !out_keys_dev || (!queries && !query_ptrs_dev)) return fail(h, MI355REC_ERR_INVALID_ARG, "null argument");
    if (batch < 1) return fail(h, MI355REC_ERR_INVALID_ARG, "batch must be positive");
    EnqueueCall call(h, topn, false, stream);
    if (call.rc) return call.rc;
    hipStream_t s = call.s;
    int rc = MI355REC_OK;
    if (h->n < 1) return answer_empty(h, out_keys_dev, static_cast<size_t>(batch) * topn, s);
    if (batch >= 2 && mi355rec_batch_pointers_ok(h, topn) && h->batch_path != MI355REC_BATCH_MULTI) {
        for (int b = 0; b < batch; b += kMultiChain) {
            const int count = batch - b < kMultiChain ? batch - b : kMultiChain;
            rc = enqueue_half_multi(h, queries ? queries + static_cast<size_t>(b) * kDim : nullptr,
                                    query_ptrs_dev ? query_ptrs_dev + b : nullptr, exclude_global ? exclude_global + b : nullptr,
                                    count, topn, out_keys_dev + static_cast<size_t>(b) * topn, nullptr, nullptr, s);
            if (rc) return rc;
        }
        return MI355REC_OK;
    }
    for (int b = 0; b < batch; ++b) {
        const float* ptr = query_ptrs_dev ? query_ptrs_dev[b] : nullptr;
        if (!ptr && !queries) return fail(h, MI355REC_ERR_INVALID_ARG, "query %d has neither a vector nor a pointer", b);
        rc = enqueue_query(h, ptr, queries ? queries + static_cast<size_t>(b) * kDim : nullptr,
                           exclude_global ? exclude_global[b] : -1, topn, out_keys_dev + static_cast<size_t>(b) * topn, nullptr,
                           nullptr, s);
        if (rc) return rc;
    }
    return MI355REC_OK;
}


int mi355rec_row_ptr(mi355rec_t* h, int64_t local_row, const float** out_dev) {
    if (!h || !out_dev) return fail(h, MI355REC_ERR_INVALID_ARG, "null argument");
    if (local_row < 0 || local_row >= h->n)
        return fail(h, MI355REC_ERR_INVALID_ARG, "Invalid song index: %lld", (long long)local_row);
    *out_dev = h->d_feats + local_row * kDim;
    return MI355REC_OK;
}

int mi355rec_enqueue_ptr_keys(mi355rec_t* h, const float* query12_dev, int64_t exclude_global, int topn,
                              mi355rec_key_t* out_keys_dev, int64_t* out_idx_dev, float* out_score_dev, void* stream) {
    if (!h || !out_keys_dev || !query12_dev) return fail(h, MI355REC_ERR_INVALID_ARG, "null argument");
    EnqueueCall call(h, topn, true, stream);
    if (call.rc) return call.rc;
// ... 21 lines not shown
    return flush_mstream(h, s);
}

int mi355rec_enqueue_batch_keys(mi355rec_t* h, const float* queries, const int64_t* exclude_global,
                                int batch, int topn, mi355rec_key_t* out_keys_dev, void* stream) {
    if (!h || !queries || !out_keys_dev) return fail(h, MI355REC_ERR_INVALID_ARG, "null argument");
    if (batch < 1) return fail(h, MI355REC_ERR_INVALID_ARG, "batch must be positive");
    EnqueueCall call(h, topn, true, stream);
    if (call.rc) return call.rc;
    return enqueue_batch(h, queries, exclude_global, batch, topn, out_keys_dev, nullptr, nullptr, call.s);
}

int mi355rec_enqueue_batch_keys_dev(mi355rec_t* h, const float* queries_dev, const int64_t* exclude_global_dev,
                                    int batch, int topn, mi355rec_key_t* out_keys_dev, void* stream) {
    if (!h || !queries_dev || !out_keys_dev) return fail(h, MI355REC_ERR_INVALID_ARG, "null argument");
    if (batch < 1) return fail(h, MI355REC_ERR_INVALID_ARG, "batch must be positive");
    if (topn <= 0 || topn > kMultiMaxTopK)
        return fail(h, MI355REC_ERR_INVALID_ARG, "topn must be in [1, %d] for device-resident batches, got %d",
                    kMultiMaxTopK, topn);
    if (h->n < 1) return fail(h, MI355REC_ERR_INVALID_ARG, "empty shard: use the host-query entry point");
    DeviceGuard guard(h->device);
    hipStream_t s = static_cast<hipStream_t>(stream);
    int rc = order_stream(h, s);
    if (rc) return rc;
    rc = ensure_bq(h);
    if (rc) return rc;
    static_assert(sizeof(long long) == sizeof(int64_t), "exclude ids are passed through unchanged");
    for (int b0 = 0; b0 < batch; b0 += kBqMaxQueries) {
        const int count = batch - b0 < kBqMaxQueries ? batch - b0 : kBqMaxQueries;
        rc = enqueue_bq_chunk(h, queries_dev + static_cast<size_t>(b0) * kDim,
                              exclude_global_dev ? reinterpret_cast<const long long*>(exclude_global_dev) + b0 : nullptr,
                              count, topn, out_keys_dev + static_cast<size_t>(b0) * topn, nullptr, nullptr, s);
        if (rc) return rc;
    }
    return MI355REC_OK;
}

int mi355rec_batched_last_counters(mi355rec_t* h, int32_t* special_rows, int32_t* queued_queries,
                                   int64_t* candidates_total, int32_t* candidates_max) {
    if (!h) return fail(nullptr, MI355REC_ERR_INVALID_ARG, "null handle");
    if (!h->bq.ready) return fail(h, MI355REC_ERR_INVALID_ARG, "no batched call has been made on this handle");
    DeviceGuard guard(h->device);
    HIP_TRY(h, hipDeviceSynchronize());
    int counters[4] = {0, 0, 0, 0};
    std::vector<int> cand(kBqMaxQueries);
    std::vector<uint32_t> flags(kBqMaxQueries);
    HIP_TRY(h, hipMemcpy(counters, h->bq.counters, sizeof counters, hipMemcpyDeviceToHost));
    HIP_TRY(h, hipMemcpy(cand.data(), h->bq.cand_examined, sizeof(int) * kBqMaxQueries, hipMemcpyDeviceToHost));
    HIP_TRY(h, hipMemcpy(flags.data(), h->bq.qflags, sizeof(uint32_t) * kBqMaxQueries, hipMemcpyDeviceToHost));
    int64_t total = 0;
    int mx = 0;
    for (int q = 0; q < h->bq.last_count; ++q) {
        if (flags[q] != kBqFlagOk) continue;
        total += cand[q];
        if (cand[q] > mx) mx = cand[q];
    }
    if (special_rows) *special_rows = counters[0];
    if (queued_queries) *queued_queries = counters[1];
    if (candidates_total) *candidates_total = total;
    if (candidates_max) *candidates_max = mx;
    return MI355REC_OK;
}

int mi355rec_batched_pass2_pairs(mi355rec_t* h, int64_t* pairs_done, int64_t* pairs_total) {
    if (!h) return fail(nullptr, MI355REC_ERR_INVALID_ARG, "null handle");
    if (!h->bq.ready) return fail(h, MI355REC_ERR_INVALID_ARG, "no batched call has been made on this handle");
    DeviceGuard guard(h->device);
    HIP_TRY(h, hipDeviceSynchronize());
    int counters[4] = {0, 0, 0, 0};
    HIP_TRY(h, hipMemcpy(counters, h->bq.counters, sizeof counters, hipMemcpyDeviceToHost));
    const int blocks = (h->bq.last_count + 31) / 32;
    int nb = 1;
    while (nb < blocks) nb *= 2;
    const int64_t total = ((h->n + 63) / 64) * nb;
    if (pairs_total) *pairs_total = total;
    if (pairs_done) *pairs_done = counters[3] > 0 ? counters[3] : total;
    return MI355REC_OK;
}

int mi355rec_set_batch_path(mi355rec_t* h, int path) {
    if (!h) return fail(nullptr, MI355REC_ERR_INVALID_ARG, "null handle");
    if (path != MI355REC_BATCH_AUTO && path != MI355REC_BATCH_MULTI && path != MI355REC_BATCH_MFMA && path != MI355REC_BATCH_HALF &&
        path != MI355REC_BATCH_Q8 && path != MI355REC_BATCH_MFMA_NOSKIP)
        return fail(h, MI355REC_ERR_INVALID_ARG, "unknown batch path %d", path);
#ifndef MI355REC_EXPERIMENTS
    if (path == MI355REC_BATCH_Q8)
        return fail(h, MI355REC_ERR_INVALID_ARG, "MI355REC_BATCH_Q8 (the 8-bit front end of the multi-query pass) exists in MI355REC_EXPERIMENTS builds only");
#endif
    h->batch_path = path;
    return MI355REC_OK;
}

namespace {
int adopt_group_replica(mi355rec* h) {
    if (!h->shared || h->d_half || !h->shared->d_half) return MI355REC_OK;
    DeviceGuard guard(h->device);
    const int rc = alloc_replica_state(h);
    if (rc == MI355REC_OK && hipStreamSynchronize(h->stream) != hipSuccess)
        return fail(h, MI355REC_ERR_HIP, "hipStreamSynchronize(replica state)");
    if (rc != MI355REC_OK) {
        void* bufs[] = {h->d_half_mseed, h->d_half_rescored, h->d_half_mcuts, h->d_half_mctl};
        for (void* b : bufs)
            if (b) (void)hipFree(b);
        h->d_half_mseed = nullptr;
        h->d_half_rescored = nullptr;
        h->d_half_mcuts = nullptr;
        h->d_half_mctl = nullptr;
        return rc;
    }
    h->d_half = static_cast<decltype(h->d_half)>(h->shared->d_half);
    h->d_q8 = static_cast<decltype(h->d_q8)>(h->shared->d_q8);
    h->bsample = h->shared->bsample;
    h->margin_mix = h->shared->margin_mix;
    h->margin_mfma = h->shared->margin_mfma;
    return MI355REC_OK;
}
}

int mi355rec_set_replica(mi355rec_t* h, int mode) {
    if (!h) return fail(nullptr, MI355REC_ERR_INVALID_ARG, "null handle");
    if (mode != MI355REC_REPLICA_AUTO && mode != MI355REC_REPLICA_OFF && mode != MI355REC_REPLICA_ON && mode != MI355REC_REPLICA_FP16)
        return fail(h, MI355REC_ERR_INVALID_ARG, "unknown replica mode %d", mode);
#ifndef MI355REC_EXPERIMENTS
    if (mode == MI355REC_REPLICA_FP16)
        return fail(h, MI355REC_ERR_INVALID_ARG, "MI355REC_REPLICA_FP16 (single queries over the fp16 replica) exists in MI355REC_EXPERIMENTS builds only");
#endif
    if ((mode == MI355REC_REPLICA_ON || mode == MI355REC_REPLICA_FP16) && !h->d_half && h->n > 0) {
        if (!h->replica_allowed)
            return fail(h, MI355REC_ERR_INVALID_ARG, "this handle was created without a replica (MI355REC_CREATE_NO_REPLICA)");
        int rc = adopt_group_replica(h);
        if (rc) return rc;
        if (!h->d_half) {
            rc = mi355rec_rebuild_replica(h);
            if (rc) return rc;
        }
        preallocate_stream_state(h);
    }
    h->replica_mode = mode;
    return MI355REC_OK;
}

int mi355rec_set_sample(mi355rec_t* h, int mode) {
    if (!h) return fail(nullptr, MI355REC_ERR_INVALID_ARG, "null handle");
    if (mode != MI355REC_SAMPLE_AUTO && mode != MI355REC_SAMPLE_STRIDED && mode != MI355REC_SAMPLE_BUCKETED)
        return fail(h, MI355REC_ERR_INVALID_ARG, "unknown sample mode %d", mode);
    if (mode == MI355REC_SAMPLE_BUCKETED && !h->bsample.rows)
        return fail(h, MI355REC_ERR_INVALID_ARG, "this handle has no bucketed sample (mi355rec_bucket_sample_info)");
    h->sample_mode = mode;
    return MI355REC_OK;
}

int mi355rec_set_stream_pairing(mi355rec_t* h, int mode) {
    if (!h) return fail(nullptr, MI355REC_ERR_INVALID_ARG, "null handle");
    if (mode != MI355REC_PAIRING_AUTO && mode != MI355REC_PAIRING_OFF && mode != MI355REC_PAIRING_ON)
        return fail(h, MI355REC_ERR_INVALID_ARG, "unknown pairing mode %d", mode);
    h->pairing = mode;
    return MI355REC_OK;
}

int mi355rec_bucket_sample_info(const mi355rec_t* h, mi355rec_bucket_sample_info_t* out) {
    if (!h || !out) return fail(nullptr, MI355REC_ERR_INVALID_ARG, "null argument");
    std::memset(out, 0, sizeof *out);
    const BucketBufs& b = h->bsample;
    out->mode = h->sample_mode;
    out->last_used = h->last_sample;
    if (!b.rows) return MI355REC_OK;
    out->base_rows = b.base_rows;
    out->regions = b.regions;
    out->centroids = b.n_centroids;
    out->bytes = b.bytes();
    out->stride_rows = b.stride;
    out->centroid_stride = b.centroid_stride;
    out->picks = b.regions < kBucketPicks ? b.regions : kBucketPicks;
    out->build_ms = b.build_ms;
    return MI355REC_OK;
}

int mi355rec_bucket_sample_rows(mi355rec_t* h, int32_t* rows_out, int32_t* region_tab_out) {
    if (!h) return fail(nullptr, MI355REC_ERR_INVALID_ARG, "null handle");
    const BucketBufs& b = h->bsample;
    if (!b.rows) return fail(h, MI355REC_ERR_INVALID_ARG, "this handle has no bucketed sample (mi355rec_bucket_sample_info)");
    DeviceGuard guard(h->device);
    HIP_TRY(h, hipStreamSynchronize(h->stream));
    if (rows_out) HIP_TRY(h, hipMemcpy(rows_out, b.rows, sizeof(int32_t) * static_cast<size_t>(b.regions) * kBucketRegionRows, hipMemcpyDeviceToHost));
    if (region_tab_out) HIP_TRY(h, hipMemcpy(region_tab_out, b.region_tab, sizeof(int32_t) * 2 * static_cast<size_t>(b.regions), hipMemcpyDeviceToHost));
    return MI355REC_OK;
}

#ifdef MI355REC_TEST_HOOKS
int mi355rec_debug_handoff(mi355rec_t* h, int flags) {
    if (!h) return fail(nullptr, MI355REC_ERR_INVALID_ARG, "null handle");
    DeviceGuard guard(h->device);
    if (flags & MI355REC_DEBUG_HANDOFF_POISON) {
        HIP_TRY(h, hipDeviceSynchronize());
        const uint32_t one = score_to_ordered(1.0f);
        const size_t per = static_cast<size_t>(kSampleSlots);
        std::vector<unsigned long long> vals(static_cast<size_t>(kHmSampleSlots));
        for (size_t i = 0; i < vals.size(); ++i)
            vals[i] = (static_cast<unsigned long long>(h->epoch_ctr - 1u - static_cast<uint32_t>(i % 3)) << 32) | one;
        unsigned long long* single[] = {h->d_half_seed, h->d_stream_seed[0], h->d_stream_seed[1]};
        for (unsigned long long* b : single)
            if (b) HIP_TRY(h, hipMemcpy(b, vals.data(), sizeof(unsigned long long) * per, hipMemcpyHostToDevice));
        unsigned long long* multi[] = {h->d_half_mseed, h->d_mstream_seed[0], h->d_mstream_seed[1]};
        for (unsigned long long* b : multi)
            if (b) HIP_TRY(h, hipMemcpy(b, vals.data(), sizeof(unsigned long long) * vals.size(), hipMemcpyHostToDevice));
        unsigned int one_bits;
        const float onef = 1.0f;
        std::memcpy(&one_bits, &onef, sizeof one_bits);
        const unsigned long long stale_cut = (static_cast<unsigned long long>(h->epoch_ctr - 1u) << 32) | one_bits;
        if (h->d_stream_ctl) {
            SeedCtl ctl[2];
            HIP_TRY(h, hipMemcpy(ctl, h->d_stream_ctl, sizeof ctl, hipMemcpyDeviceToHost));
            ctl[0].cutoff = ctl[1].cutoff = stale_cut;
            HIP_TRY(h, hipMemcpy(h->d_stream_ctl, ctl, sizeof ctl, hipMemcpyHostToDevice));
        }
        if (h->pairs.ready) {
            std::vector<unsigned long long> older(per);
            for (size_t i = 0; i < per; ++i)
                older[i] = (static_cast<unsigned long long>(h->epoch_ctr - 2u - static_cast<uint32_t>(i % 3)) << 32) | one;
            for (unsigned long long* b : h->pairs.seed)
                if (b) HIP_TRY(h, hipMemcpy(b, older.data(), sizeof(unsigned long long) * per, hipMemcpyHostToDevice));
            SeedCtl ctl[4];
            HIP_TRY(h, hipMemcpy(ctl, h->pairs.ctl, sizeof ctl, hipMemcpyDeviceToHost));
            for (SeedCtl& c : ctl) c.cutoff = (static_cast<unsigned long long>(h->epoch_ctr - 2u) << 32) | one_bits;
            HIP_TRY(h, hipMemcpy(h->pairs.ctl, ctl, sizeof ctl, hipMemcpyHostToDevice));
        }
        if (h->d_lone_ctl) {
            SeedCtl ctl;
            HIP_TRY(h, hipMemcpy(&ctl, h->d_lone_ctl, sizeof ctl, hipMemcpyDeviceToHost));
            ctl.cutoff = stale_cut;
            HIP_TRY(h, hipMemcpy(h->d_lone_ctl, &ctl, sizeof ctl, hipMemcpyHostToDevice));
        }
        std::vector<unsigned long long> cuts(2 * kHmQueries, stale_cut);
        if (h->d_mstream_cuts)
            HIP_TRY(h, hipMemcpy(h->d_mstream_cuts, cuts.data(), sizeof(unsigned long long) * cuts.size(), hipMemcpyHostToDevice));
        if (h->d_half_mcuts)
            HIP_TRY(h, hipMemcpy(h->d_half_mcuts, cuts.data(), sizeof(unsigned long long) * kHmQueries, hipMemcpyHostToDevice));
    }
    if (flags & MI355REC_DEBUG_HANDOFF_DROP_STORES) h->dbg_skip_regions = kHalfSeedMaxGrid / 2;
    if (flags & MI355REC_DEBUG_HANDOFF_NO_LAST_RIDER) h->dbg_no_last = true;
    return MI355REC_OK;
}

#endif

#ifdef MI355REC_PHASE_CLOCK
int mi355rec_debug_phase_clock(unsigned long long* out, int n_words) {
    if (hipDeviceSynchronize() != hipSuccess) return MI355REC_ERR_HIP;
    return hipMemcpyFromSymbol(out, HIP_SYMBOL(mi355::g_phase_clock), sizeof(unsigned long long) * n_words) == hipSuccess
               ? MI355REC_OK : MI355REC_ERR_HIP;
}
#endif

int mi355rec_replica_counters(mi355rec_t* h, int64_t* scans, int64_t* rescored_rows) {
    if (!h) return fail(nullptr, MI355REC_ERR_INVALID_ARG, "null handle");
    if (scans) *scans = h->half_scans;
    if (rescored_rows) *rescored_rows = 0;
    if (!h->d_half_rescored || !rescored_rows) return MI355REC_OK;
    DeviceGuard guard(h->device);
    std::vector<unsigned long long> slots(kRideMaxLists);
    HIP_TRY(h, hipDeviceSynchronize());
    HIP_TRY(h, hipMemcpy(slots.data(), h->d_half_rescored, sizeof(unsigned long long) * kRideMaxLists, hipMemcpyDeviceToHost));
    unsigned long long sum = 0;
    for (unsigned long long v : slots) sum += v;
    *rescored_rows = static_cast<int64_t>(sum);
    return MI355REC_OK;
}

int mi355rec_rebuild_replica(mi355rec_t* h) {
    if (!h) return fail(nullptr, MI355REC_ERR_INVALID_ARG, "null handle");
    if (h->n == 0) return MI355REC_OK;
    if (!h->replica_allowed)
        return fail(h, MI355REC_ERR_INVALID_ARG, "this handle was created without a replica (MI355REC_CREATE_NO_REPLICA)");
    if (h->shared && h->shared->d_half)
        return fail(h, MI355REC_ERR_INVALID_ARG, "the replicas are shared with lanes (mi355rec_create_lane): destroy the lanes, rebuild, create them again");
    DeviceGuard guard(h->device);
    int rc = sync_api_begin(h);
    if (rc) return rc;
    rc = flush_streamed(h, h->stream);
    if (rc) return rc;
    rc = flush_mstream(h, h->stream);
    if (rc) return rc;
    rc = build_anchors(h);
    if (rc) return rc;
    rc = build_replica(h);
    drop_distance_norms(h);
    if (rc == MI355REC_OK && h->shared) {
        h->shared->d_half = h->d_half;
        h->shared->d_q8 = h->d_q8;
        h->shared->bsample = h->bsample;
        h->shared->margin_mix = h->margin_mix;
        h->shared->margin_mfma = h->margin_mfma;
    }
    return rc;
}

int mi355rec_enqueue_merge_keys(mi355rec_t* h, const mi355rec_key_t* lists_dev, int n_lists,
                                int list_len, int topn, mi355rec_key_t* out_keys_dev,
                                int64_t* out_idx_dev, float* out_score_dev, void* stream) {
    if (!h || !lists_dev || !out_keys_dev) return fail(h, MI355REC_ERR_INVALID_ARG, "null argument");
    if (n_lists < 1 || n_lists > kMergeMaxLists || list_len < 1)
        return fail(h, MI355REC_ERR_INVALID_ARG, "n_lists %d / list_len %d out of range", n_lists, list_len);
    int rc = check_topn(h, topn, false);
    if (rc) return rc;
    DeviceGuard guard(h->device);
    rc = order_stream(h, static_cast<hipStream_t>(stream));
    if (rc) return rc;
    return enqueue_merge(h, lists_dev, n_lists, list_len, topn, out_keys_dev, out_idx_dev,
                         out_score_dev, static_cast<hipStream_t>(stream));
}

int mi355rec_enqueue_merge_keys_batch(mi355rec_t* h, const mi355rec_key_t* lists_dev, int n_lists,
                                      int list_len, int64_t list_stride, int64_t query_stride, int batch,
                                      int topn, mi355rec_key_t* out_keys_dev, int64_t* out_idx_dev,
                                      float* out_score_dev, void* stream) {
    if (!h || !lists_dev || !out_keys_dev) return fail(h, MI355REC_ERR_INVALID_ARG, "null argument");
    if (n_lists < 1 || n_lists > kMergeMaxLists || list_len < 1 || batch < 1 || list_stride < list_len)
        return fail(h, MI355REC_ERR_INVALID_ARG, "merge geometry out of range");
    int rc = check_topn(h, topn, false);
    if (rc) return rc;
    DeviceGuard guard(h->device);
    hipStream_t s = static_cast<hipStream_t>(stream);
    rc = order_stream(h, s);
    if (rc) return rc;
    const int slot = timing_begin(h, h->ev_merge, h->n_merge_pairs, h->merge_launches, s);
    hipLaunchKernelGGL(merge_kernel, dim3(batch), dim3(kMergeBlock), 0, s, lists_dev, n_lists, list_len,
                       list_stride, query_stride, topn, out_keys_dev, out_idx_dev, out_score_dev,
                       static_cast<int64_t>(topn), static_cast<uint32_t*>(nullptr), 0u);
    timing_end(h, h->ev_merge, h->n_merge_pairs, slot, s);
    HIP_TRY(h, hipGetLastError());
    return MI355REC_OK;
}

int mi355rec_enqueue_scores(mi355rec_t* h, int64_t local_row, const float* query12,
                            float* out_scores_dev, void* stream) {
    if (!h || !out_scores_dev) return fail(h, MI355REC_ERR_INVALID_ARG, "null argument");
    if (local_row >= h->n) return fail(h, MI355REC_ERR_INVALID_ARG, "Invalid song index: %lld", (long long)local_row);
    if (local_row < 0 && !query12) return fail(h, MI355REC_ERR_INVALID_ARG, "null query");
    if (h->n == 0) return MI355REC_OK;
    DeviceGuard guard(h->device);
    hipStream_t s = static_cast<hipStream_t>(stream);
    int rc = order_stream(h, s);
    if (rc) return rc;
    const float* const qrow = local_row >= 0 ? h->d_feats + local_row * kDim : nullptr;
    const QueryArg qa = make_query_arg(h, qrow, query12);
    const ScanGeom& g = h->geom[kFp32];
    hipLaunchKernelGGL((scan_kernel<ScanConfig, false, true>), dim3(g.grid), dim3(kScanBlock), 0, s, h->d_feats,
                       h->n, static_cast<int64_t>(0), g.iters, h->row_base, qa, qrow,
                       static_cast<int64_t>(-1), 1, static_cast<uint64_t*>(nullptr), out_scores_dev,
                       static_cast<const uint64_t*>(nullptr), no_prev_merge(),
                       static_cast<const unsigned long long*>(nullptr), static_cast<const unsigned long long*>(nullptr), 0u, no_next_seed());
    HIP_TRY(h, hipGetLastError());
    return MI355REC_OK;
}

int mi355rec_enqueue_stream_probe(mi355rec_t* h, uint32_t* sink_dev, void* stream) {
    return mi355rec_enqueue_stream_probe_of(h, MI355REC_PROBE_FP32_ROWS, sink_dev, stream);
}

int mi355rec_enqueue_stream_probe_of(mi355rec_t* h, int which, uint32_t* sink_dev, void* stream) {
    if (!h || !sink_dev) return fail(h, MI355REC_ERR_INVALID_ARG, "null argument");
    if (h->n == 0) return MI355REC_OK;
    const float4* buf = nullptr;
    int64_t n_vec = 0;
    if (which == MI355REC_PROBE_FP32_ROWS) {
        buf = reinterpret_cast<const float4*>(h->d_feats);
        n_vec = h->n * 3;
    } else if (which == MI355REC_PROBE_FP16_REPLICA && h->d_half) {
        buf = reinterpret_cast<const float4*>(h->d_half);
        n_vec = ((h->n + 1) / 2) * 3;
    } else if (which == MI355REC_PROBE_Q8_REPLICA && h->d_q8) {
        buf = reinterpret_cast<const float4*>(h->d_q8);
        n_vec = ((h->n + 3) / 4) * 3;
    } else {
        return fail(h, MI355REC_ERR_INVALID_ARG, "no such buffer to probe (%d)", which);
    }
    DeviceGuard guard(h->device);
// ... 104 lines not shown
```

### spotify_recommender_amd/csrc/replica_q8.hip.h

```cpp
#pragma once

#include "replica.hip.h"

#ifndef MI355_Q8_QUERY_BITS
#define MI355_Q8_QUERY_BITS 16
#endif

namespace mi355 {

constexpr int kQ8QueryBits = MI355_Q8_QUERY_BITS;
static_assert(kQ8QueryBits == 16 || kQ8QueryBits == 8, "the query is one or two int8 digits per component");
constexpr float kQ8Step = 1.0f / 254.0f;
constexpr float kQ8QueryScale = kQ8QueryBits == 16 ? 32000.0f : 127.0f;
constexpr float kQ8DotScale = 127.0f * kQ8QueryScale;
constexpr float kQ8QueryResidual = 3.4642f * 0.5f / kQ8QueryScale;
constexpr float kQ8Slack = 3e-5f;
constexpr uint32_t kQ8Special = 0x80u;


__device__ __forceinline__ void q8_pack_row(const float4& a, const float4& b, const float4& c, float tot, uint32_t& d0, uint32_t& d1,
                                            uint32_t& d2) {
    const bool valid = tot >= kBqMinNorm2 && tot <= kBqMaxNorm2;
    if (valid || tot == 0.0f) {
        const float inv = valid ? __builtin_amdgcn_rsqf(tot) * 127.0f : 0.0f;
        auto q = [&](float x) {
            int k = static_cast<int>(__builtin_rintf(x * inv));
            k = k > 127 ? 127 : (k < -127 ? -127 : k);
            return static_cast<uint32_t>(k) & 0xffu;
        };
        d0 = q(a.x) | (q(a.y) << 8) | (q(a.z) << 16) | (q(a.w) << 24);
        d1 = q(b.x) | (q(b.y) << 8) | (q(b.z) << 16) | (q(b.w) << 24);
        d2 = q(c.x) | (q(c.y) << 8) | (q(c.z) << 16) | (q(c.w) << 24);
    }
}

__global__ __launch_bounds__(256) void q8_build_kernel(const float* __restrict__ feats, int64_t n, int64_t n_padded,
                                                       uint32_t* __restrict__ q8, float* __restrict__ norms,
                                                       const int32_t* __restrict__ pick, const float* __restrict__ centroids,
                                                       int n_centroids, int32_t* __restrict__ bucket,
                                                       const int64_t* __restrict__ upd_src, const int64_t* __restrict__ upd_dst,
                                                       uint2* __restrict__ half, float* __restrict__ rows_out) {
    __shared__ float s_inv[1024];
    if (centroids) {
        n_centroids = n_centroids < 1024 ? n_centroids : 1024;
        for (int c = threadIdx.x; c < n_centroids; c += blockDim.x) {
            float tot = 0.0f;
            for (int j = 0; j < kDim; ++j) tot = __builtin_fmaf(centroids[c * kDim + j], centroids[c * kDim + j], tot);
            const float inv = 1.0f / sqrtf(tot);
            s_inv[c] = (tot > 0.0f && inv == inv && inv < 3.0e38f) ? inv : 0.0f;
        }
        __syncthreads();
    }
    const int64_t slot = static_cast<int64_t>(blockIdx.x) * blockDim.x + threadIdx.x;
    if (slot >= n_padded) return;
    int64_t row = slot, out = slot;
    if (pick) {
        row = pick[slot];
        row = row >= 0 ? row : n;
    }
    if (upd_dst) {
        row = upd_src ? upd_src[slot] : slot;
        out = upd_dst[slot];
        if (row < 0 || row >= n) return;
    }
    uint32_t d0 = 0x80808080u, d1 = 0x80808080u, d2 = 0x80808080u;
    uint32_t hp[6] = {kHalfNaN2, kHalfNaN2, kHalfNaN2, kHalfNaN2, kHalfNaN2, kHalfNaN2};
    float seq = 0.0f;
    if (row < n) {
        const float4* p = reinterpret_cast<const float4*>(feats) + row * 3;
        const float4 a = p[0], b = p[1], c = p[2];
        if (rows_out) {
            float4* dst = reinterpret_cast<float4*>(rows_out) + out * 3;
            dst[0] = a;
            dst[1] = b;
            dst[2] = c;
        }
        if (centroids) {
            const float f[kDim] = {a.x, a.y, a.z, a.w, b.x, b.y, b.z, b.w, c.x, c.y, c.z, c.w};
            float best = -__builtin_inff();
            int best_c = 0;
            for (int k = 0; k < n_centroids; ++k) {
                float dot = 0.0f;
#pragma unroll
                for (int j = 0; j < kDim; ++j) dot = __builtin_fmaf(f[j], centroids[k * kDim + j], dot);
                const float v = dot * s_inv[k];
                if (v > best) {
                    best = v;
                    best_c = k;
                }
            }
            bucket[slot] = best_c;
        }
        if (norms) {
            const float f[kDim] = {a.x, a.y, a.z, a.w, b.x, b.y, b.z, b.w, c.x, c.y, c.z, c.w};
#pragma unroll
            for (int j = 0; j < kDim; ++j) seq = seq + f[j] * f[j];
        }
        const float tot = replica_norm2(a, b, c);
        q8_pack_row(a, b, c, tot, d0, d1, d2);
        if (half) half_pack_row(a, b, c, tot, hp);
    } else if (centroids) {
        bucket[slot] = 0;
    }
    if (q8) {
        uint32_t* dst = q8 + out * 3;
        dst[0] = d0;
        dst[1] = d1;
        dst[2] = d2;
    }
    if (half) {
        uint2* dst = half + out * 3;
        dst[0] = make_uint2(hp[0], hp[1]);
        dst[1] = make_uint2(hp[2], hp[3]);
        dst[2] = make_uint2(hp[4], hp[5]);
    }
    if (norms) norms[out] = sqrtf(seq);
}

struct Q8Query {
    int hi[3];
    int lo[3];
    float inv;
    float margin;
    bool ok;
};

__device__ __forceinline__ Q8Query q8_query(const float (&q)[kDim], float qn) {
    Q8Query r;
    r.ok = qn >= kBqMinNorm && qn <= kBqMaxNorm;
    const float inv = r.ok ? 1.0f / qn : 0.0f;
    r.hi[0] = r.hi[1] = r.hi[2] = 0;
    r.lo[0] = r.lo[1] = r.lo[2] = 0;
    int l1 = 0;
    constexpr int kMax = static_cast<int>(kQ8QueryScale);
#pragma unroll
    for (int j = 0; j < kDim; ++j) {
        int Q = static_cast<int>(__builtin_rintf(q[j] * inv * kQ8QueryScale));
        Q = Q > kMax ? kMax : (Q < -kMax ? -kMax : Q);
        l1 += Q < 0 ? -Q : Q;
        if constexpr (kQ8QueryBits == 16) {
            const int h = (Q + 128) >> 8;
            const int l = Q - 256 * h;
            r.hi[j >> 2] |= (h & 0xff) << (8 * (j & 3));
            r.lo[j >> 2] |= (l & 0xff) << (8 * (j & 3));
        } else {
            r.hi[j >> 2] |= (Q & 0xff) << (8 * (j & 3));
        }
    }
    r.inv = 1.0f / kQ8DotScale;
    r.margin = static_cast<float>(l1) * (kQ8Step / kQ8QueryScale) * (1.0f + 1e-5f) + kQ8QueryResidual + kQ8Slack;
    return r;
}

__device__ __forceinline__ int q8_dot(const Q8Query& q, uint32_t d0, uint32_t d1, uint32_t d2, bool& special) {
    special = (d0 & 0xffu) == kQ8Special;
// ... 430 lines not shown
        dst.t0 = p[0];
        dst.t1 = p[1];
        dst.t2 = p[2];
    };

    constexpr int kDepth = Cfg::kDepth;
    float cutoff_left = 0.0f;
    const unsigned long long nbhd_raw = seed_vals[kNbhdSlot];
    SampleRaw sample_raw;
#pragma unroll
    for (int r = 0; r < kHalfSeedPerThread; ++r) sample_raw.t[r] = 0ull;
    const int n_sample = n_seed < 0 ? -n_seed : n_seed;
    if (cutoff_ready) {
        cutoff_left = untag_cutoff(*cutoff_ready, epoch);
    } else {
        sample_raw = sample_request<kBlock>(seed_vals, n_sample);
    }
    HalfTile ring[kDepth];
#pragma unroll
    for (int d = 0; d < kDepth - 1; ++d) load_tile(ring[d], d);
    float q[kDim];
    q8_load_query((kQueryFromRow || kWithMerge) ? query_ptr : nullptr, qarg.q, q);
    const float qn = query_norm(q);
    const Q8Query hq = q8_query(q, qn);
    const Sample sample = sample_finish(sample_raw, epoch);
    if (hq.hi[0] != 0 || n >= 0) MI355REC_PHASE(1);
    if (sample.v[0] != 0x12345u || n >= 0) MI355REC_PHASE(6);

    if (tid == 0) {
        s_count = 0;
        sm->seeds = 0;
        sm->rescored = 0;
    }
    int n_rescored = 0;
    __syncthreads();
    float cutoff;
    if (cutoff_ready) {
        cutoff = cutoff_left;
    } else {
        cutoff = q8_cutoff_from_sample<kBlock>(sample, n_sample, topk, n_seed < 0, hq, &sm->seeds, s_sel, reinterpret_cast<int*>(s_cand));
    }
    uint64_t thr = 0;
    if (const uint32_t nbv = untag_value(nbhd_raw, epoch)) {
        thr = (static_cast<uint64_t>(nbv) << 32) - 1ull;
        if (hq.ok) {
            const float nb_cut = ordered_to_score(nbv) - hq.margin;
            cutoff = nb_cut > cutoff ? nb_cut : cutoff;
        }
    }
    int cut_d = q8_threshold(cutoff);
    MI355REC_PHASE(2);
    int compact_at = 2 * topk > 256 ? 2 * topk : 256;
    if (compact_at > kCandLimit) compact_at = kCandLimit;

    Row pend;
    pend.a = pend.b = pend.c = make_float4(0.0f, 0.0f, 0.0f, 0.0f);
    int64_t pend_r = 0;
    bool pend_on = false;

    auto append = [&](bool have, const Row& row, int64_t r) {
        const float s = cosine_score(q, qn, row);
        const int64_t g = row_base + r;
        uint64_t key = pack_key(s, static_cast<uint32_t>(g));
        if (g == exclude_global) key = 0;
        const bool pass = have && key > thr;
        const uint64_t ballot = __ballot(pass);
        if (ballot) {
            int base = 0;
            if (lane == 0) base = atomicAdd(&s_count, __popcll(ballot));
            base = __builtin_amdgcn_readfirstlane(base);
            const int pos = base + lanes_below(ballot);
            if (pass) s_cand[pos] = key;
        }
    };
    auto consume = [&]() {
        if (__ballot(pend_on)) append(pend_on, pend, pend_r);
        pend_on = false;
    };

    auto process_tile = [&](const HalfTile& t, int it) {
        const int64_t quad = quad_begin + static_cast<int64_t>(it) * quad_stride;
        const int64_t r0 = quad * 4;
        int a[4];
        bool special[4];
        q8_dot4(hq, t, a, special);
        bool hit[4];
#pragma unroll
        for (int u = 0; u < 4; ++u) hit[u] = special[u] | (a[u] >= cut_d);
        const uint64_t maybe = __ballot(hit[0] | hit[1] | hit[2] | hit[3]);
        consume();
        uint32_t mask = 0u;
        if (maybe) {
            const int64_t left = n - r0;
            const int valid = quad < n_quads ? (left < 4 ? static_cast<int>(left) : 4) : 0;
#pragma unroll
            for (int u = 0; u < 4; ++u) mask |= (hit[u] && u < valid) ? (1u << u) : 0u;
        }
        const uint64_t any = maybe ? __ballot(mask != 0u) : 0ull;
        if (any) {
            n_rescored += __popcll(any);
            const int first = mask ? __builtin_ctz(mask) : 0;
            pend_r = r0 + first;
            pend = load_row(feats, mask ? pend_r : static_cast<int64_t>(0));
            pend_on = mask != 0u;
            uint32_t rest = mask & (mask - 1u);
            while (__ballot(rest != 0u)) {
                const int u = rest ? __builtin_ctz(rest) : 0;
                const bool have = rest != 0u;
                n_rescored += __popcll(__ballot(have));
                const Row extra = load_row(feats, have ? r0 + u : static_cast<int64_t>(0));
                append(have, extra, r0 + u);
                rest &= rest - 1u;
            }
        }
        __syncthreads();
        const int c = s_count;
        __syncthreads();
        if (c >= compact_at) {
            const uint64_t local_thr = compact_candidates<kBlock, Cfg::kCandPerThread>(s_cand, &s_count, topk, false, s_sel);
            if (local_thr > thr) {
                thr = local_thr;
                if (hq.ok) {
                    const float local_cut = ordered_to_score(static_cast<uint32_t>(thr >> 32)) - hq.margin;
                    cutoff = local_cut > cutoff ? local_cut : cutoff;
                    cut_d = q8_threshold(cutoff);
                }
            }
        }
    };

    for (int it = 0; it < iters; it += kDepth) {
#pragma unroll
        for (int sidx = 0; sidx < kDepth; ++sidx) {
            load_tile(ring[(sidx + kDepth - 1) % kDepth], it + sidx + kDepth - 1);
            if (it + sidx < iters) process_tile(ring[sidx], it + sidx);
        }
    }
    consume();

    if (lane == 0 && n_rescored) atomicAdd(&sm->rescored, n_rescored);
    __syncthreads();
    MI355REC_PHASE(3);
    if (tid == 0) rescored[bid] += static_cast<unsigned long long>(sm->rescored);
    if (s_count > kRankCountMax && s_count > topk)
        compact_candidates<kBlock, Cfg::kCandPerThread>(s_cand, &s_count, topk, false, s_sel);
    __syncthreads();
    block_rank_and_store<kBlock, kLoneTail>(s_cand, s_count, block_lists + static_cast<int64_t>(bid) * topk, topk);
    if constexpr (kLoneTail) lone_tail(s_mem.merge, &s_lone_flag, block_lists, topk, lone);
    __syncthreads();
    MI355REC_PHASE(4);
}

constexpr int kPairMaxTopk = 128;

__device__ __forceinline__ int q8_uniform(int v) { return __builtin_amdgcn_readfirstlane(v); }
__device__ __forceinline__ float q8_uniform(float v) { return __int_as_float(__builtin_amdgcn_readfirstlane(__float_as_int(v))); }
__device__ __forceinline__ uint64_t q8_uniform(uint64_t v) {
    const uint32_t lo = static_cast<uint32_t>(__builtin_amdgcn_readfirstlane(static_cast<int>(static_cast<uint32_t>(v))));
    const uint32_t hi = static_cast<uint32_t>(__builtin_amdgcn_readfirstlane(static_cast<int>(static_cast<uint32_t>(v >> 32))));
    return (static_cast<uint64_t>(hi) << 32) | lo;
}
__device__ __forceinline__ Q8Query q8_uniform(const Q8Query& q) {
    Q8Query r;
#pragma unroll
    for (int j = 0; j < 3; ++j) {
        r.hi[j] = q8_uniform(q.hi[j]);
        r.lo[j] = q8_uniform(q.lo[j]);
    }
    r.inv = q.inv;
    r.margin = q8_uniform(q.margin);
    r.ok = q8_uniform(q.ok ? 1 : 0) != 0;
    return r;
}
constexpr int kPairCandLimit = 2 * kPairMaxTopk;

template <int kBlockT, int kMinWavesT, int kDepthT>
struct Q8PairCfg {
    static constexpr int kBlock = kBlockT;
    static constexpr int kMinWaves = kMinWavesT;
    static constexpr int kDepth = kDepthT;
    static constexpr int kTileRows = 4 * kBlockT;
    static constexpr int kCandCap = kPairCandLimit + kTileRows;
    static constexpr int kCandPerThread = (kCandCap + kBlockT - 1) / kBlockT;
};
using DefaultQ8PairCfg = Q8PairCfg<512, 4, 2>;

template <typename Cfg>
struct Q8PairSmemT {
    uint64_t cand[2][Cfg::kCandCap];
    SelectSmem sel;
    int count[2];
    int seeds[2];
    int rescored;
};
template <typename Cfg>
union Q8PairOrMergeSmem {
    Q8PairSmemT<Cfg> scan;
    MergeSmemT<Cfg::kBlock, kRideMaxLists, kHalfRideSurvCap> merge;
};

struct Q8PairArg {
    QueryArg qarg;
    const float* query_ptr;
    long long exclude_global;
    uint64_t* block_lists;
    const unsigned long long* seed_vals;
    const unsigned long long* cutoff_ready;
    int n_seed;
    uint32_t epoch;
};

struct Q8PairSide {
    PrevMerge prev[2];
    NextSeed next[2];
};

template <typename Cfg>
__global__ __launch_bounds__(Cfg::kBlock, Cfg::kMinWaves) void scan_q8_kernel_pair(
    const float* __restrict__ feats, const uint4* __restrict__ q8, int64_t n, int iters, int64_t row_base, Q8PairArg arg_a,
    Q8PairArg arg_b, int topk, unsigned long long* __restrict__ rescored , Q8PairSide side) {
    constexpr int kBlock = Cfg::kBlock;
    __shared__ Q8PairOrMergeSmem<Cfg> s_mem;
    const unsigned riders = static_cast<unsigned>(side.next[0].n_wgs), nbhds = static_cast<unsigned>(side.next[0].nbhd);
    const unsigned extra = 2u + 2u * (riders + nbhds);
    const unsigned nblocks = gridDim.x - extra;
    const unsigned vb = blockIdx.x >= extra ? blockIdx.x - extra : nblocks + blockIdx.x;
    if (vb >= nblocks) {
        static_assert(kBlock == kHalfSeedBlock && sizeof(s_mem.scan.cand) >= sizeof(int) * kBucketScratch &&
                          sizeof(s_mem.scan.cand) >= sizeof(int) * Nbhd<kBlock>::kScratch, "the riders' geometry");
        int* const s_scratch = reinterpret_cast<int*>(s_mem.scan.cand);
        const unsigned e = vb - nblocks;
        if (e < 2u) {
            q8_ride_merge(s_mem.merge, side.prev[e]);
        } else if (e < 2u + 2u * riders) {
            const unsigned which = e - 2u >= riders ? 1u : 0u;
            q8_ride_sample<kBlock>(feats, q8, n, row_base, side.next[which], static_cast<int>(e - 2u - which * riders), s_scratch,
                                   &s_mem.scan.count[0], &s_mem.scan.seeds[0], s_mem.scan.sel);
        } else {
            q8_ride_nbhd<kBlock>(feats, n, row_base, side.next[e - 2u - 2u * riders], s_scratch);
        }
        __syncthreads();
        return;
    }
    Q8PairSmemT<Cfg>* const sm = &s_mem.scan;
    SelectSmem& s_sel = sm->sel;

    const unsigned bid = vb;
    const int tid = threadIdx.x;
    const int lane = tid & 63;

    const int64_t n_quads = (n + 3) >> 2;
    const int64_t last_quad = n_quads - 1;
    const int64_t quad_begin = static_cast<int64_t>(bid) * kBlock + tid;
    const int64_t quad_stride = static_cast<int64_t>(nblocks) * kBlock;

    auto load_tile = [&](HalfTile& dst, int it) {
        int64_t quad = quad_begin + static_cast<int64_t>(it) * quad_stride;
        quad = quad < n_quads ? quad : last_quad;
        const uint4* p = q8 + quad * 3;
        dst.t0 = p[0];
        dst.t1 = p[1];
        dst.t2 = p[2];
    };

    struct Mine {
        float q[kDim];
        float qn;
        Q8Query hq;
        float cutoff;
        uint64_t thr;
        int cut_d;
        int n_rescored;
        uint64_t* s_cand;
        int* s_count;
    };
    Mine A, B;
    A.s_cand = sm->cand[0];
    B.s_cand = sm->cand[1];
    A.s_count = &sm->count[0];
    B.s_count = &sm->count[1];

    constexpr int kDepth = Cfg::kDepth;
    const unsigned long long nbhd_raw_a = arg_a.seed_vals[kNbhdSlot], nbhd_raw_b = arg_b.seed_vals[kNbhdSlot];
    float left_a = 0.0f, left_b = 0.0f;
    SampleRaw raw_a, raw_b;
#pragma unroll
    for (int r = 0; r < kHalfSeedPerThread; ++r) raw_a.t[r] = raw_b.t[r] = 0ull;
    const int n_sample_a = arg_a.n_seed < 0 ? -arg_a.n_seed : arg_a.n_seed, n_sample_b = arg_b.n_seed < 0 ? -arg_b.n_seed : arg_b.n_seed;
    if (arg_a.cutoff_ready) left_a = untag_cutoff(*arg_a.cutoff_ready, arg_a.epoch);
    else raw_a = sample_request<kBlock>(arg_a.seed_vals, n_sample_a);
    if (arg_b.cutoff_ready) left_b = untag_cutoff(*arg_b.cutoff_ready, arg_b.epoch);
    else raw_b = sample_request<kBlock>(arg_b.seed_vals, n_sample_b);
    HalfTile ring[kDepth];
#pragma unroll
    for (int d = 0; d < kDepth - 1; ++d) load_tile(ring[d], d);
    q8_load_query(arg_a.query_ptr, arg_a.qarg.q, A.q);
    q8_load_query(arg_b.query_ptr, arg_b.qarg.q, B.q);
    A.qn = q8_uniform(query_norm(A.q));
    B.qn = q8_uniform(query_norm(B.q));
    A.hq = q8_uniform(q8_query(A.q, A.qn));
    B.hq = q8_uniform(q8_query(B.q, B.qn));

    if (tid == 0) {
        sm->count[0] = sm->count[1] = 0;
        sm->seeds[0] = sm->seeds[1] = 0;
        sm->rescored = 0;
    }
    __syncthreads();
    auto start = [&](Mine& m, const Q8PairArg& arg, const SampleRaw& raw, int n_sample, float left, unsigned long long nbhd_raw, int* s_seeds) {
        if (arg.cutoff_ready) {
            m.cutoff = left;
        } else {
            const Sample sample = sample_finish(raw, arg.epoch);
            m.cutoff = q8_cutoff_from_sample<kBlock>(sample, n_sample, topk, arg.n_seed < 0, m.hq, s_seeds, s_sel, reinterpret_cast<int*>(m.s_cand));
        }
        m.thr = 0;
        if (const uint32_t nbv = untag_value(nbhd_raw, arg.epoch)) {
            m.thr = (static_cast<uint64_t>(nbv) << 32) - 1ull;
            if (m.hq.ok) {
                const float nb_cut = ordered_to_score(nbv) - m.hq.margin;
                m.cutoff = nb_cut > m.cutoff ? nb_cut : m.cutoff;
            }
        }
        m.cutoff = q8_uniform(m.cutoff);
        m.thr = q8_uniform(m.thr);
        m.cut_d = q8_uniform(q8_threshold(m.cutoff));
        m.n_rescored = 0;
    };
    start(A, arg_a, raw_a, n_sample_a, left_a, nbhd_raw_a, &sm->seeds[0]);
    __syncthreads();
    start(B, arg_b, raw_b, n_sample_b, left_b, nbhd_raw_b, &sm->seeds[1]);
    int compact_at = 2 * topk > 256 ? 2 * topk : 256;
    if (compact_at > kPairCandLimit) compact_at = kPairCandLimit;

    auto append = [&](Mine& m, int64_t exclude_global, bool have, const Row& row, int64_t r) {
        const float s = cosine_score(m.q, m.qn, row);
        const int64_t g = row_base + r;
        uint64_t key = pack_key(s, static_cast<uint32_t>(g));
        if (g == exclude_global) key = 0;
        const bool pass = have && key > m.thr;
        const uint64_t ballot = __ballot(pass);
        if (ballot) {
            int base = 0;
            if (lane == 0) base = atomicAdd(m.s_count, __popcll(ballot));
            base = __builtin_amdgcn_readfirstlane(base);
            const int pos = base + lanes_below(ballot);
            if (pass) m.s_cand[pos] = key;
        }
    };
    Row pend;
    pend.a = pend.b = pend.c = make_float4(0.0f, 0.0f, 0.0f, 0.0f);
    int64_t pend_r = 0;
    uint32_t pend_for = 0u;
    auto score_row = [&](uint32_t who, const Row& row, int64_t r) {
        if (__ballot((who & 1u) != 0u)) append(A, arg_a.exclude_global, (who & 1u) != 0u, row, r);
        if (__ballot((who & 2u) != 0u)) append(B, arg_b.exclude_global, (who & 2u) != 0u, row, r);
    };
    auto consume = [&]() {
        if (__ballot(pend_for != 0u)) score_row(pend_for, pend, pend_r);
        pend_for = 0u;
    };
    auto fetch = [&](uint32_t mask_a, uint32_t mask_b, int64_t r0) {
        const uint32_t both = mask_a | mask_b;
        if (!__ballot(both != 0u)) return;
        auto whose = [&](int u) { return ((mask_a >> u) & 1u) | (((mask_b >> u) & 1u) << 1); };
        auto count = [&](uint32_t who) {
            A.n_rescored += __popcll(__ballot((who & 1u) != 0u));
            B.n_rescored += __popcll(__ballot((who & 2u) != 0u));
        };
        const int first = both ? __builtin_ctz(both) : 0;
        pend_r = r0 + first;
        pend = load_row(feats, both ? pend_r : static_cast<int64_t>(0));
        pend_for = both ? whose(first) : 0u;
        count(pend_for);
        uint32_t rest = both & (both - 1u);
        while (__ballot(rest != 0u)) {
            const int u = rest ? __builtin_ctz(rest) : 0;
            const uint32_t who = rest ? whose(u) : 0u;
            count(who);
            const Row extra = load_row(feats, rest ? r0 + u : static_cast<int64_t>(0));
            score_row(who, extra, r0 + u);
            rest &= rest - 1u;
        }
    };
    auto tighten = [&](Mine& m) {
        const uint64_t local_thr = compact_candidates<kBlock, Cfg::kCandPerThread>(m.s_cand, m.s_count, topk, false, s_sel);
        if (local_thr > m.thr) {
            m.thr = q8_uniform(local_thr);
            if (m.hq.ok) {
                const float local_cut = ordered_to_score(static_cast<uint32_t>(m.thr >> 32)) - m.hq.margin;
                m.cutoff = q8_uniform(local_cut > m.cutoff ? local_cut : m.cutoff);
                m.cut_d = q8_uniform(q8_threshold(m.cutoff));
            }
        }
    };

    auto process_tile = [&](const HalfTile& t, int it) {
        const int64_t quad = quad_begin + static_cast<int64_t>(it) * quad_stride;
        const int64_t r0 = quad * 4;
        uint32_t hit_a = 0u, hit_b = 0u;
        {
            int a[4];
            bool special[4];
            q8_dot4(A.hq, t, a, special);
#pragma unroll
            for (int u = 0; u < 4; ++u) hit_a |= (special[u] | (a[u] >= A.cut_d)) ? (1u << u) : 0u;
            q8_dot4(B.hq, t, a, special);
#pragma unroll
            for (int u = 0; u < 4; ++u) hit_b |= (special[u] | (a[u] >= B.cut_d)) ? (1u << u) : 0u;
        }
        const uint64_t maybe = __ballot((hit_a | hit_b) != 0u);
        consume();
        if (maybe) {
            const int64_t left = n - r0;
            const int valid = quad < n_quads ? (left < 4 ? static_cast<int>(left) : 4) : 0;
            const uint32_t inside = (1u << valid) - 1u;
            fetch(hit_a & inside, hit_b & inside, r0);
        }
        __syncthreads();
        const int ca = *A.s_count, cb = *B.s_count;
        __syncthreads();
        if (ca >= compact_at) tighten(A);
        if (cb >= compact_at) tighten(B);
    };

    for (int it = 0; it < iters; it += kDepth) {
#pragma unroll
        for (int sidx = 0; sidx < kDepth; ++sidx) {
            load_tile(ring[(sidx + kDepth - 1) % kDepth], it + sidx + kDepth - 1);
            if (it + sidx < iters) process_tile(ring[sidx], it + sidx);
        }
    }
    consume();

    if (lane == 0 && A.n_rescored + B.n_rescored) atomicAdd(&sm->rescored, A.n_rescored + B.n_rescored);
    __syncthreads();
    if (tid == 0) rescored[bid] += static_cast<unsigned long long>(sm->rescored);
    auto finish = [&](Mine& m, uint64_t* block_lists) {
        if (*m.s_count > kRankCountMax && *m.s_count > topk)
            compact_candidates<kBlock, Cfg::kCandPerThread>(m.s_cand, m.s_count, topk, false, s_sel);
        __syncthreads();
        block_rank_and_store<kBlock>(m.s_cand, *m.s_count, block_lists + static_cast<int64_t>(bid) * topk, topk);
        __syncthreads();
    };
    finish(A, arg_a.block_lists);
    finish(B, arg_b.block_lists);
}

}
```

Baseline: 106,000 queries/s.

## Generalize paired Q8 stream scan to groups of up to four queries

Replaces the fixed two-query paired scan with a grouping state machine that can batch up to four streamed queries into one Q8 scan launch, so each pass over the catalogue replica serves more queries. The kernel now keeps per-query thresholds, candidate lists and merges in arrays and adds a two-stage high/low digit pre-filter. Group mode only turns on automatically above an effectively unreachable row threshold, so by default it still forms pairs, now through the new generalized kernel with extra per-slot bookkeeping and register pressure.

After: 106,100 queries/s, median of 5. No clear change (+0.0%).

```diff
diff --git a/include/mi355rec_diag.h b/include/mi355rec_diag.h
--- a/include/mi355rec_diag.h
+++ b/include/mi355rec_diag.h
@@ -40,6 +40,8 @@
     int64_t route_exact_queue;
     int32_t device_bytes_per_row;
     int64_t stream_pair_launches;
+    int64_t stream_group_launches;
+    int64_t stream_group_queries;
 } mi355rec_stats_t;
 
 #define MI355REC_BUILD_EXPERIMENTS 1
@@ -74,7 +76,9 @@
 #define MI355REC_PAIRING_AUTO 0
 #define MI355REC_PAIRING_OFF 1
 #define MI355REC_PAIRING_ON 2
+#define MI355REC_PAIRING_GROUPS 3
 #define MI355REC_PAIRING_AUTO_MIN_ROWS 2500000
+#define MI355REC_GROUPS_AUTO_MIN_ROWS 9223372036854775807
 int mi355rec_set_stream_pairing(mi355rec_t* h, int mode);
 typedef struct {
     int64_t base_rows;
diff --git a/spotify_recommender_amd/capi.py b/spotify_recommender_amd/capi.py
--- a/spotify_recommender_amd/capi.py
+++ b/spotify_recommender_amd/capi.py
@@ -14,8 +14,9 @@
 REPLICA_AUTO, REPLICA_OFF, REPLICA_ON, REPLICA_FP16 = 0, 1, 2, 3
 SAMPLE_AUTO, SAMPLE_STRIDED, SAMPLE_BUCKETED = 0, 1, 2
 SAMPLE_AUTO_MIN_ROWS = 6_000_000
-PAIRING_AUTO, PAIRING_OFF, PAIRING_ON = 0, 1, 2
+PAIRING_AUTO, PAIRING_OFF, PAIRING_ON, PAIRING_GROUPS = 0, 1, 2, 3
 PAIRING_AUTO_MIN_ROWS = 2_500_000
+GROUPS_AUTO_MIN_ROWS = 9223372036854775807
 TRANSPORT_PEER, TRANSPORT_RCCL = 1, 2
 PLACEMENT_AUTO, PLACEMENT_SHARDED, PLACEMENT_REPLICATED, PLACEMENT_CPU = 0, 1, 2, 3
 CREATE_NO_REPLICA = 1
@@ -137,6 +138,8 @@
         ("route_exact_queue", c_int64),
         ("device_bytes_per_row", c_int32),
         ("stream_pair_launches", c_int64),
+        ("stream_group_launches", c_int64),
+        ("stream_group_queries", c_int64),
     ]
 
 
diff --git a/spotify_recommender_amd/csrc/engine_single.hip.h b/spotify_recommender_amd/csrc/engine_single.hip.h
--- a/spotify_recommender_amd/csrc/engine_single.hip.h
+++ b/spotify_recommender_amd/csrc/engine_single.hip.h
@@ -456,15 +456,19 @@
 }
 
 bool pairing_on(const mi355rec* h) {
-    if (h->pairing == MI355REC_PAIRING_ON) return true;
+    if (h->pairing == MI355REC_PAIRING_ON || h->pairing == MI355REC_PAIRING_GROUPS) return true;
     if (h->pairing == MI355REC_PAIRING_OFF) return false;
-    return h->n >= MI355REC_PAIRING_AUTO_MIN_ROWS;
-}
-bool pairs_open(const mi355rec* h) { return h->pairs.waiting || h->pairs.has_first || h->pairs.pending; }
+    return h->n >= MI355REC_PAIRING_AUTO_MIN_ROWS || h->n >= MI355REC_GROUPS_AUTO_MIN_ROWS;
+}
+bool groups_on(const mi355rec* h) {
+    if (h->pairing == MI355REC_PAIRING_GROUPS) return true;
+    return h->pairing == MI355REC_PAIRING_AUTO && h->n >= MI355REC_GROUPS_AUTO_MIN_ROWS;
+}
+bool pairs_open(const mi355rec* h) { return h->pairs.sg.open(); }
 
 void free_pairs(mi355rec* h) {
     auto& P = h->pairs;
-    for (int i = 0; i < 4; ++i) {
+    for (int i = 0; i < mi355rec::Pairs::kBufs; ++i) {
         if (P.lists[i]) (void)hipFree(P.lists[i]);
         if (P.seed[i]) (void)hipFree(P.seed[i]);
         P.lists[i] = nullptr;
@@ -477,14 +481,15 @@
 
 int ensure_pairs_alloc(mi355rec* h) {
     auto& P = h->pairs;
+    constexpr int kBufs = mi355rec::Pairs::kBufs;
     const size_t words = static_cast<size_t>(h->geom[kQ8].grid > 0 ? h->geom[kQ8].grid : 1) * kPairMaxTopk;
-    for (int i = 0; i < 4; ++i) {
+    for (int i = 0; i < kBufs; ++i) {
         HIP_TRY(h, hipMalloc(&P.lists[i], sizeof(uint64_t) * words));
         HIP_TRY(h, hipMalloc(&P.seed[i], sizeof(unsigned long long) * kSampleSlots));
         HIP_TRY(h, hipMemset(P.seed[i], 0, sizeof(unsigned long long) * kSampleSlots));
     }
-    HIP_TRY(h, hipMalloc(&P.ctl, sizeof(SeedCtl) * 4));
-    HIP_TRY(h, hipMemset(P.ctl, 0, sizeof(SeedCtl) * 4));
+    HIP_TRY(h, hipMalloc(&P.ctl, sizeof(SeedCtl) * kBufs));
+    HIP_TRY(h, hipMemset(P.ctl, 0, sizeof(SeedCtl) * kBufs));
     return MI355REC_OK;
 }
 int ensure_pairs(mi355rec* h) {
@@ -499,99 +504,164 @@
     return MI355REC_OK;
 }
 
-int merge_pair_pending(mi355rec* h, hipStream_t s) {
+int group_cap(const mi355rec* h, int topn) {
+    if (!groups_on(h)) return 2;
+    const ScanGeom& g = stream_geom(h, kQ8, use_bucket(h, kQ8, topn, h->geom_bucket.riders > 0));
+    if (g.riders == 0) return kGroupMax;
+    const int extra = kGroupMax * (1 + g.riders + (g.nbhd ? 1 : 0));
+    return 4 * extra <= g.grid ? kGroupMax : 2;
+}
+
+int merge_pair_pending(mi355rec* h, hipStream_t s, int count) {
     auto& P = h->pairs;
-    P.pending = false;
-    for (int x = 0; x < 2; ++x) {
-        const int rc = enqueue_merge(h, P.lists[2 * P.pending_set + x], P.pending_lists, P.pending_topn, P.pending_topn, P.pending_out[x],
+    for (int x = 0; x < count; ++x) {
+        const int rc = enqueue_merge(h, P.lists[kGroupMax * P.pending_set + x], P.pending_lists, P.pending_topn, P.pending_topn, P.pending_out[x],
                                      nullptr, nullptr, s);
         if (rc) return rc;
     }
     return MI355REC_OK;
 }
 
-int launch_pair(mi355rec* h, hipStream_t s, const mi355rec::Stashed* next, bool next_bucketed) {
+int launch_group(mi355rec* h, hipStream_t s, int nq, int n_pend, mi355rec::Stashed* next, int n_next, bool next_bucketed, bool* sampled) {
     auto& P = h->pairs;
-    const mi355rec::Stashed& a = P.wait[0];
-    const mi355rec::Stashed& b = P.wait[1];
-    const int topn = a.topn;
-    if (P.pending) {
-        const uint64_t* lo = P.pending_out[0] < P.pending_out[1] ? P.pending_out[0] : P.pending_out[1];
-        const uint64_t* hi = P.pending_out[0] < P.pending_out[1] ? P.pending_out[1] : P.pending_out[0];
-        if (hi < lo + P.pending_topn) {
-            const int rc = merge_pair_pending(h, s);
-            if (rc) return rc;
-        }
-    }
-    const ScanGeom& g = stream_geom(h, kQ8, next != nullptr && next_bucketed);
-    const bool riders = next != nullptr && (g.riders > 0 || g.nbhd);
-    const int extra = 2 + (riders ? 2 * (g.riders + (g.nbhd ? 1 : 0)) : 0);
+    const int topn = P.wait[0].topn;
+    bool overlap = false;
+    for (int i = 0; i < n_pend; ++i)
+        for (int j = i + 1; j < n_pend; ++j) {
+            const uint64_t* lo = P.pending_out[i] < P.pending_out[j] ? P.pending_out[i] : P.pending_out[j];
+            const uint64_t* hi = P.pending_out[i] < P.pending_out[j] ? P.pending_out[j] : P.pending_out[i];
+            overlap = overlap || hi < lo + P.pending_topn;
+        }
+    if (overlap) {
+        const int rc = merge_pair_pending(h, s, n_pend);
+        if (rc) return rc;
+        n_pend = 0;
+    }
+    const ScanGeom& g = stream_geom(h, kQ8, n_next > 0 && next_bucketed);
+    const bool riders = n_next > 0 && (g.riders > 0 || g.nbhd);
+    const int n_merge = n_pend > 0 ? n_pend : 2;
+    const int extra = n_merge + (riders ? n_next * (g.riders + (g.nbhd ? 1 : 0)) : 0);
     const int64_t tiles = (h->n + Q8PairConfig::kTileRows - 1) / Q8PairConfig::kTileRows;
     int64_t scanners = g.grid - extra;
     if (scanners > kRideMaxLists - 1) scanners = kRideMaxLists - 1;
     if (scanners > tiles) scanners = tiles;
     if (scanners < 1) scanners = 1;
     const int iters = static_cast<int>((tiles + scanners - 1) / scanners);
-    const int set = P.pending ? 1 - P.pending_set : 0;
+    const int set = n_pend > 0 ? 1 - P.pending_set : 0;
     Q8PairSide side;
     std::memset(&side, 0, sizeof side);
-    side.prev[0] = side.prev[1] = no_prev_merge();
-    if (P.pending)
-        for (int x = 0; x < 2; ++x) side.prev[x] = PrevMerge{P.lists[2 * P.pending_set + x], P.pending_lists, P.pending_topn, P.pending_out[x]};
-    if (riders)
-        for (int x = 0; x < 2; ++x)
+    for (int x = 0; x < kGroupMax; ++x) side.prev[x] = no_prev_merge();
+    for (int x = 0; x < n_pend; ++x)
+        side.prev[x] = PrevMerge{P.lists[kGroupMax * P.pending_set + x], P.pending_lists, P.pending_topn, P.pending_out[x]};
+    side.n_merge = n_merge;
+    if (riders) {
+        side.nq_next = n_next;
+        for (int x = 0; x < n_next; ++x)
             side.next[x] = make_next_seed(h, kQ8, g.riders, g.nbhd, next[x].qptr, next[x].q, next[x].exclude, next[x].topn, next[x].epoch,
                                           P.seed[next[x].seed_buf], g.hoists ? P.ctl + next[x].seed_buf : nullptr,
                                           P.ctl_done[next[x].seed_buf], next_bucketed);
-    Q8PairArg arg[2];
-    const mi355rec::Stashed* const q[2] = {&a, &b};
-    for (int x = 0; x < 2; ++x) {
-        std::memset(&arg[x], 0, sizeof arg[x]);
-        arg[x].qarg = make_query_arg(h, q[x]->qptr, q[x]->q);
-        arg[x].query_ptr = q[x]->qptr;
-        arg[x].exclude_global = q[x]->exclude;
-        arg[x].block_lists = P.lists[2 * set + x];
-        arg[x].seed_vals = P.seed[q[x]->seed_buf];
-        arg[x].cutoff_ready = q[x]->cutoff_ready ? &P.ctl[q[x]->seed_buf].cutoff : nullptr;
-        arg[x].n_seed = q8_seed_count(h, q[x]->bucketed);
-        arg[x].epoch = q[x]->epoch;
-    }
-    const dim3 grid(static_cast<unsigned>(scanners + 2 + 2 * (side.next[0].n_wgs + side.next[0].nbhd)));
+    }
+    Q8GroupArgs args;
+    std::memset(&args, 0, sizeof args);
+    for (int x = 0; x < nq; ++x) {
+        const mi355rec::Stashed& q = P.wait[x];
+        Q8PairArg& a = args.a[x];
+        a.qarg = make_query_arg(h, q.qptr, q.q);
+        a.query_ptr = q.qptr;
+        a.exclude_global = q.exclude;
+        a.block_lists = P.lists[kGroupMax * set + x];
+        a.seed_vals = P.seed[q.seed_buf];
+        a.cutoff_ready = q.cutoff_ready ? &P.ctl[q.seed_buf].cutoff : nullptr;
+        a.n_seed = q8_seed_count(h, q.bucketed);
+        a.epoch = q.epoch;
+    }
+    const dim3 grid(static_cast<unsigned>(scanners + side.n_merge + side.nq_next * (side.next[0].n_wgs + side.next[0].nbhd)));
     LAUNCH_TIMED(h, h->ev_scan, h->n_scan_pairs, h->scan_launches, scan_q8_kernel_pair<Q8PairConfig>, grid, dim3(Q8PairConfig::kBlock), s,
-                 h->d_feats, h->d_q8, h->n, iters, h->row_base, arg[0], arg[1], topn, h->d_half_rescored, side);
+                 h->d_feats, h->d_q8, h->n, iters, h->row_base, args, nq, topn, h->d_half_rescored, side);
     HIP_TRY(h, hipGetLastError());
-    h->half_scans += 2;
-    h->q8_scans += 2;
-    h->routes.q8 += 2;
-    ++h->stream_pair_launches;
-    for (int x = 0; x < 2; ++x)
+    h->half_scans += nq;
+    h->q8_scans += nq;
+    h->routes.q8 += nq;
+    if (nq == 2) {
+        ++h->stream_pair_launches;
+    } else {
+        ++h->stream_group_launches;
+        h->stream_group_queries += nq;
+    }
+    for (int x = 0; x < side.nq_next; ++x)
         if (side.next[x].ctl) P.ctl_done[next[x].seed_buf] += static_cast<unsigned>(side.next[x].n_wgs);
-    P.pending = true;
+    if (sampled) *sampled = riders && g.riders > 0;
     P.pending_set = set;
     P.pending_lists = static_cast<int>(scanners);
     P.pending_topn = topn;
-    P.pending_out[0] = a.out;
-    P.pending_out[1] = b.out;
-    P.waiting = false;
+    for (int x = 0; x < nq; ++x) P.pending_out[x] = P.wait[x].out;
+    return MI355REC_OK;
+}
+
+int run_group_steps(mi355rec* h, hipStream_t s, const GroupSteps& steps, int n_pend_before) {
+    auto& P = h->pairs;
+    int n_pend = n_pend_before;
+    bool sampled = false, bucketed = false;
+    for (int i = 0; i < steps.count; ++i) {
+        const GroupStep& st = steps.step[i];
+        if (st.kind == kGroupLaunch) {
+            const int set = 1 - P.wait_set;
+            if (st.n_next > 0) {
+                bucketed = use_bucket(h, kQ8, P.form[0].topn, h->geom_bucket.riders > 0);
+                for (int x = 0; x < st.n_next; ++x) {
+                    P.form[x].seed_buf = kGroupMax * set + x;
+                    P.form[x].epoch = next_epoch(h);
+                    P.form[x].bucketed = bucketed;
+                }
+            }
+            sampled = false;
+            const int rc = launch_group(h, s, st.n, n_pend, st.n_next > 0 ? P.form : nullptr, st.n_next, bucketed, &sampled);
+            if (rc) return rc;
+            n_pend = st.n;
+        } else if (st.kind == kGroupPromote) {
+            const int topn = P.form[0].topn;
+            if (!st.sampled) {
+                const int set = 0;
+                bucketed = use_bucket(h, kQ8, topn, h->geom_bucket.riders > 0);
+                for (int x = 0; x < st.n; ++x) {
+                    P.form[x].seed_buf = kGroupMax * set + x;
+                    P.form[x].epoch = next_epoch(h);
+                    P.form[x].bucketed = bucketed;
+                }
+                sampled = false;
+            }
+            const ScanGeom& ng = stream_geom(h, kQ8, bucketed);
+            h->last_sample = bucketed ? MI355REC_SAMPLE_BUCKETED : MI355REC_SAMPLE_STRIDED;
+            if (!sampled) {
+                for (int x = 0; x < st.n; ++x)
+                    enqueue_half_seed(h, kQ8, P.form[x].qptr, P.form[x].q, P.form[x].exclude, topn, P.seed[P.form[x].seed_buf], P.form[x].epoch, s,
+                                      bucketed);
+                HIP_TRY(h, hipGetLastError());
+            }
+            for (int x = 0; x < st.n; ++x) {
+                P.form[x].cutoff_ready = sampled && ng.hoists;
+                P.wait[x] = P.form[x];
+            }
+            P.wait_set = P.wait[0].seed_buf / kGroupMax;
+        } else if (st.kind == kGroupMerge) {
+            const int rc = merge_pair_pending(h, s, st.n);
+            if (rc) return rc;
+            n_pend = 0;
+        } else {
+            const mi355rec::Stashed f = P.form[0];
+            const int rc = enqueue_streamed_single(h, f.qptr, f.q, f.exclude, f.topn, f.out, s, h->d_q8 ? f.kind : -1);
+            if (rc) return rc;
+        }
+    }
     return MI355REC_OK;
 }
 
 int drain_pairs(mi355rec* h, hipStream_t s) {
     auto& P = h->pairs;
-    if (P.waiting) {
-        const int rc = launch_pair(h, s, nullptr, false);
-        if (rc) return rc;
-    }
-    if (P.pending) {
-        const int rc = merge_pair_pending(h, s);
-        if (rc) return rc;
-    }
-    if (P.has_first) {
-        const mi355rec::Stashed f = P.first;
-        P.has_first = false;
-        return enqueue_streamed_single(h, f.qptr, f.q, f.exclude, f.topn, f.out, s, h->d_q8 ? f.kind : -1);
-    }
-    return MI355REC_OK;
+    GroupSteps steps;
+    const int n_pend = P.sg.n_pend;
+    P.sg.drain(steps);
+    return run_group_steps(h, s, steps, n_pend);
 }
 
 int enqueue_streamed(mi355rec* h, const float* qptr, const float* query12, int64_t exclude_global, int topn,
@@ -606,10 +676,6 @@
         (void)hipGetLastError();
         pair = false;
     }
-    if (pair && P.has_first && (P.first.topn != topn || P.first_replica_mode != h->replica_mode || P.first_sample_mode != h->sample_mode)) {
-        rc = drain_pairs(h, s);
-        if (rc) return rc;
-    }
     if (!pair) {
         if (pairs_open(h)) {
             rc = drain_pairs(h, s);
@@ -617,10 +683,11 @@
         }
         return enqueue_streamed_single(h, qptr, query12, exclude_global, topn, out_keys, s);
     }
-    if (h->stashed.has || h->pending) {
-        rc = flush_single_stream(h, s);
-        if (rc) return rc;
-    }
+    const uint64_t key = static_cast<uint64_t>(static_cast<uint32_t>(topn)) | (static_cast<uint64_t>(static_cast<uint32_t>(h->replica_mode) & 0xffu) << 32) |
+                         (static_cast<uint64_t>(static_cast<uint32_t>(h->sample_mode) & 0xffu) << 40);
+    GroupSteps steps;
+    const int n_pend = P.sg.n_pend;
+    const int slot = (P.sg.n_form > 0 && key != P.sg.key) ? 0 : P.sg.n_form;
     mi355rec::Stashed x;
     x.has = true;
     x.qptr = qptr;
@@ -629,41 +696,19 @@
     x.topn = topn;
     x.out = out_keys;
     x.kind = kQ8;
-    if (!P.has_first) {
-        P.first = x;
-        P.has_first = true;
-        P.first_replica_mode = h->replica_mode;
-        P.first_sample_mode = h->sample_mode;
-        return MI355REC_OK;
-    }
-    const int set = P.waiting ? 1 - (P.wait[0].seed_buf >> 1) : 0;
-    const bool bucketed = use_bucket(h, kQ8, topn, h->geom_bucket.riders > 0);
-    const ScanGeom& ng = stream_geom(h, kQ8, bucketed);
-    mi355rec::Stashed nx[2] = {P.first, x};
-    for (int i = 0; i < 2; ++i) {
-        nx[i].seed_buf = 2 * set + i;
-        nx[i].epoch = next_epoch(h);
-        nx[i].bucketed = bucketed;
-    }
-    h->last_sample = bucketed ? MI355REC_SAMPLE_BUCKETED : MI355REC_SAMPLE_STRIDED;
-    bool sampled = false;
-    if (P.waiting) {
-        sampled = ng.riders > 0;
-        rc = launch_pair(h, s, nx, bucketed);
-        if (rc) return rc;
-    }
-    if (!sampled) {
-        for (int i = 0; i < 2; ++i)
-            enqueue_half_seed(h, kQ8, nx[i].qptr, nx[i].q, nx[i].exclude, topn, P.seed[nx[i].seed_buf], nx[i].epoch, s, bucketed);
-        HIP_TRY(h, hipGetLastError());
-    }
-    for (int i = 0; i < 2; ++i) {
-        nx[i].cutoff_ready = sampled && ng.hoists;
-        P.wait[i] = nx[i];
-    }
-    P.waiting = true;
-    P.has_first = false;
-    return MI355REC_OK;
-}
-
-}
+    P.sg.add(key, group_cap(h, topn), steps);
+    if (slot == 0 && steps.count > 0) {
+        rc = run_group_steps(h, s, steps, n_pend);
+        if (rc) return rc;
+        steps.count = 0;
+    }
+    if (h->stashed.has || h->pending) {
+        rc = flush_single_stream(h, s);
+        if (rc) return rc;
+    }
+    P.form[slot] = x;
+    return run_group_steps(h, s, steps, n_pend);
+}
+
+
+}
diff --git a/spotify_recommender_amd/csrc/engine_state.hip.h b/spotify_recommender_amd/csrc/engine_state.hip.h
--- a/spotify_recommender_amd/csrc/engine_state.hip.h
+++ b/spotify_recommender_amd/csrc/engine_state.hip.h
@@ -188,20 +188,21 @@
     SeedCtl* d_stream_ctl = nullptr;
     int pairing = 0;
     int64_t stream_pair_launches = 0;
+    int64_t stream_group_launches = 0;
+    int64_t stream_group_queries = 0;
     struct Pairs {
+        static constexpr int kBufs = 2 * kGroupMax;
         bool ready = false;
-        uint64_t* lists[4] = {nullptr, nullptr, nullptr, nullptr};
-        unsigned long long* seed[4] = {nullptr, nullptr, nullptr, nullptr};
+        uint64_t* lists[kBufs] = {};
+        unsigned long long* seed[kBufs] = {};
         SeedCtl* ctl = nullptr;
-        unsigned ctl_done[4] = {0u, 0u, 0u, 0u};
-        bool waiting = false;
-        Stashed wait[2];
-        bool has_first = false;
-        Stashed first;
-        int first_replica_mode = 0, first_sample_mode = 0;
-        bool pending = false;
+        unsigned ctl_done[kBufs] = {};
+        StreamGroups sg;
+        Stashed wait[kGroupMax];
+        int wait_set = 0;
+        Stashed form[kGroupMax];
         int pending_set = 0, pending_lists = 0, pending_topn = 0;
-        uint64_t* pending_out[2] = {nullptr, nullptr};
+        uint64_t* pending_out[kGroupMax] = {};
     } pairs;
     bool mstream_ready = false;
     uint64_t* d_mstream_lists[2] = {nullptr, nullptr};
diff --git a/spotify_recommender_amd/csrc/mi355rec.hip b/spotify_recommender_amd/csrc/mi355rec.hip
--- a/spotify_recommender_amd/csrc/mi355rec.hip
+++ b/spotify_recommender_amd/csrc/mi355rec.hip
@@ -342,6 +342,8 @@
     }
     out->device_bytes_per_row = 48 + (h->d_half ? 24 : 0) + (h->d_q8 ? 12 : 0);
     out->stream_pair_launches = h->stream_pair_launches;
+    out->stream_group_launches = h->stream_group_launches;
+    out->stream_group_queries = h->stream_group_queries;
     return MI355REC_OK;
 }
 
@@ -669,7 +671,7 @@
 
 int mi355rec_set_stream_pairing(mi355rec_t* h, int mode) {
     if (!h) return fail(nullptr, MI355REC_ERR_INVALID_ARG, "null handle");
-    if (mode != MI355REC_PAIRING_AUTO && mode != MI355REC_PAIRING_OFF && mode != MI355REC_PAIRING_ON)
+    if (mode != MI355REC_PAIRING_AUTO && mode != MI355REC_PAIRING_OFF && mode != MI355REC_PAIRING_ON && mode != MI355REC_PAIRING_GROUPS)
         return fail(h, MI355REC_ERR_INVALID_ARG, "unknown pairing mode %d", mode);
     h->pairing = mode;
     return MI355REC_OK;
@@ -732,14 +734,15 @@
             HIP_TRY(h, hipMemcpy(h->d_stream_ctl, ctl, sizeof ctl, hipMemcpyHostToDevice));
         }
         if (h->pairs.ready) {
+            constexpr uint32_t kLive = static_cast<uint32_t>(kGroupMax);
             std::vector<unsigned long long> older(per);
             for (size_t i = 0; i < per; ++i)
-                older[i] = (static_cast<unsigned long long>(h->epoch_ctr - 2u - static_cast<uint32_t>(i % 3)) << 32) | one;
+                older[i] = (static_cast<unsigned long long>(h->epoch_ctr - kLive - static_cast<uint32_t>(i % 3)) << 32) | one;
             for (unsigned long long* b : h->pairs.seed)
                 if (b) HIP_TRY(h, hipMemcpy(b, older.data(), sizeof(unsigned long long) * per, hipMemcpyHostToDevice));
-            SeedCtl ctl[4];
+            SeedCtl ctl[mi355rec::Pairs::kBufs];
             HIP_TRY(h, hipMemcpy(ctl, h->pairs.ctl, sizeof ctl, hipMemcpyDeviceToHost));
-            for (SeedCtl& c : ctl) c.cutoff = (static_cast<unsigned long long>(h->epoch_ctr - 2u) << 32) | one_bits;
+            for (SeedCtl& c : ctl) c.cutoff = (static_cast<unsigned long long>(h->epoch_ctr - kLive) << 32) | one_bits;
             HIP_TRY(h, hipMemcpy(h->pairs.ctl, ctl, sizeof ctl, hipMemcpyHostToDevice));
         }
         if (h->d_lone_ctl) {
diff --git a/spotify_recommender_amd/csrc/replica_q8.hip.h b/spotify_recommender_amd/csrc/replica_q8.hip.h
--- a/spotify_recommender_amd/csrc/replica_q8.hip.h
+++ b/spotify_recommender_amd/csrc/replica_q8.hip.h
@@ -1,6 +1,7 @@
 #pragma once
 
 #include "replica.hip.h"
+#include "stream_groups.h"
 
 #ifndef MI355_Q8_QUERY_BITS
 #define MI355_Q8_QUERY_BITS 16
@@ -737,6 +738,7 @@
 }
 
 constexpr int kPairMaxTopk = 128;
+static_assert(kGroupMax >= 2 && kGroupMax <= 4, "the hot loop is unrolled for up to four queries");
 
 __device__ __forceinline__ int q8_uniform(int v) { return __builtin_amdgcn_readfirstlane(v); }
 __device__ __forceinline__ float q8_uniform(float v) { return __int_as_float(__builtin_amdgcn_readfirstlane(__float_as_int(v))); }
@@ -758,6 +760,21 @@
     return r;
 }
 constexpr int kPairCandLimit = 2 * kPairMaxTopk;
+
+__device__ __forceinline__ int q8_low_bound(const Q8Query& q) {
+    int sq = 0;
+#pragma unroll
+    for (int j = 0; j < kDim; ++j) {
+        const int l = static_cast<int>(static_cast<int8_t>((static_cast<uint32_t>(q.lo[j >> 2]) >> (8 * (j & 3))) & 0xffu));
+        sq += l * l;
+    }
+    return static_cast<int>(129.0f * sqrtf(static_cast<float>(sq)) * (1.0f + 1e-6f)) + 2;
+}
+__device__ __forceinline__ int q8_hi_threshold(int cut_d, int low_bound) {
+    if (cut_d == static_cast<int>(0x80000000u)) return cut_d;
+    const long long c = static_cast<long long>(cut_d) - low_bound;
+    return static_cast<int>((c + 255) >> 8);
+}
 
 template <int kBlockT, int kMinWavesT, int kDepthT>
 struct Q8PairCfg {
@@ -770,13 +787,28 @@
 };
 using DefaultQ8PairCfg = Q8PairCfg<512, 4, 2>;
 
+struct alignas(16) Q8GroupCold {
+    float q[kDim];
+    float qn;
+    float margin;
+    float cutoff;
+    int ok;
+    uint64_t thr;
+    long long exclude_global;
+    uint64_t* block_lists;
+    int cut_d;
+    int low_bound;
+};
+
 template <typename Cfg>
 struct Q8PairSmemT {
-    uint64_t cand[2][Cfg::kCandCap];
+    uint64_t cand[kGroupMax][Cfg::kCandCap];
     SelectSmem sel;
-    int count[2];
-    int seeds[2];
+    int count[kGroupMax];
+    int seeds[kGroupMax];
     int rescored;
+    int pad;
+    Q8GroupCold cold[kGroupMax];
 };
 template <typename Cfg>
 union Q8PairOrMergeSmem {
@@ -796,18 +828,25 @@
 };
 
 struct Q8PairSide {
-    PrevMerge prev[2];
-    NextSeed next[2];
+    PrevMerge prev[kGroupMax];
+    NextSeed next[kGroupMax];
+    int n_merge;
+    int nq_next;
+};
+
+struct Q8GroupArgs {
+    Q8PairArg a[kGroupMax];
 };
 
 template <typename Cfg>
 __global__ __launch_bounds__(Cfg::kBlock, Cfg::kMinWaves) void scan_q8_kernel_pair(
-    const float* __restrict__ feats, const uint4* __restrict__ q8, int64_t n, int iters, int64_t row_base, Q8PairArg arg_a,
-    Q8PairArg arg_b, int topk, unsigned long long* __restrict__ rescored , Q8PairSide side) {
+    const float* __restrict__ feats, const uint4* __restrict__ q8, int64_t n, int iters, int64_t row_base, Q8GroupArgs args,
+    int nq , int topk, unsigned long long* __restrict__ rescored , Q8PairSide side) {
     constexpr int kBlock = Cfg::kBlock;
     __shared__ Q8PairOrMergeSmem<Cfg> s_mem;
     const unsigned riders = static_cast<unsigned>(side.next[0].n_wgs), nbhds = static_cast<unsigned>(side.next[0].nbhd);
-    const unsigned extra = 2u + 2u * (riders + nbhds);
+    const unsigned mergers = static_cast<unsigned>(side.n_merge), after = static_cast<unsigned>(side.nq_next);
+    const unsigned extra = mergers + after * (riders + nbhds);
     const unsigned nblocks = gridDim.x - extra;
     const unsigned vb = blockIdx.x >= extra ? blockIdx.x - extra : nblocks + blockIdx.x;
     if (vb >= nblocks) {
@@ -815,14 +854,14 @@
                           sizeof(s_mem.scan.cand) >= sizeof(int) * Nbhd<kBlock>::kScratch, "the riders' geometry");
         int* const s_scratch = reinterpret_cast<int*>(s_mem.scan.cand);
         const unsigned e = vb - nblocks;
-        if (e < 2u) {
+        if (e < mergers) {
             q8_ride_merge(s_mem.merge, side.prev[e]);
-        } else if (e < 2u + 2u * riders) {
-            const unsigned which = e - 2u >= riders ? 1u : 0u;
-            q8_ride_sample<kBlock>(feats, q8, n, row_base, side.next[which], static_cast<int>(e - 2u - which * riders), s_scratch,
+        } else if (e < mergers + after * riders) {
+            const unsigned which = (e - mergers) / riders;
+            q8_ride_sample<kBlock>(feats, q8, n, row_base, side.next[which], static_cast<int>(e - mergers - which * riders), s_scratch,
                                    &s_mem.scan.count[0], &s_mem.scan.seeds[0], s_mem.scan.sel);
         } else {
-            q8_ride_nbhd<kBlock>(feats, n, row_base, side.next[e - 2u - 2u * riders], s_scratch);
+            q8_ride_nbhd<kBlock>(feats, n, row_base, side.next[e - mergers - after * riders], s_scratch);
         }
         __syncthreads();
         return;
@@ -848,89 +887,303 @@
         dst.t2 = p[2];
     };
 
-    struct Mine {
-        float q[kDim];
-        float qn;
-        Q8Query hq;
-        float cutoff;
-        uint64_t thr;
-        int cut_d;
-        int n_rescored;
-        uint64_t* s_cand;
-        int* s_count;
-    };
-    Mine A, B;
-    A.s_cand = sm->cand[0];
-    B.s_cand = sm->cand[1];
-    A.s_count = &sm->count[0];
-    B.s_count = &sm->count[1];
+    if (nq == 2) {
+        struct Mine {
+            float q[kDim];
+            float qn;
+            Q8Query hq;
+            float cutoff;
+            uint64_t thr;
+            int cut_d;
+            int n_rescored;
+            uint64_t* s_cand;
+            int* s_count;
+        };
+        Mine A, B;
+        A.s_cand = sm->cand[0];
+        B.s_cand = sm->cand[1];
+        A.s_count = &sm->count[0];
+        B.s_count = &sm->count[1];
+
+        constexpr int kDepth = Cfg::kDepth;
+        const unsigned long long nbhd_raw_a = args.a[0].seed_vals[kNbhdSlot], nbhd_raw_b = args.a[1].seed_vals[kNbhdSlot];
+        float left_a = 0.0f, left_b = 0.0f;
+        SampleRaw raw_a, raw_b;
+    #pragma unroll
+        for (int r = 0; r < kHalfSeedPerThread; ++r) raw_a.t[r] = raw_b.t[r] = 0ull;
+        const int n_sample_a = args.a[0].n_seed < 0 ? -args.a[0].n_seed : args.a[0].n_seed, n_sample_b = args.a[1].n_seed < 0 ? -args.a[1].n_seed : args.a[1].n_seed;
+        if (args.a[0].cutoff_ready) left_a = untag_cutoff(*args.a[0].cutoff_ready, args.a[0].epoch);
+        else raw_a = sample_request<kBlock>(args.a[0].seed_vals, n_sample_a);
+        if (args.a[1].cutoff_ready) left_b = untag_cutoff(*args.a[1].cutoff_ready, args.a[1].epoch);
+        else raw_b = sample_request<kBlock>(args.a[1].seed_vals, n_sample_b);
+        HalfTile ring[kDepth];
+    #pragma unroll
+        for (int d = 0; d < kDepth - 1; ++d) load_tile(ring[d], d);
+        q8_load_query(args.a[0].query_ptr, args.a[0].qarg.q, A.q);
+        q8_load_query(args.a[1].query_ptr, args.a[1].qarg.q, B.q);
+        A.qn = q8_uniform(query_norm(A.q));
+        B.qn = q8_uniform(query_norm(B.q));
+        A.hq = q8_uniform(q8_query(A.q, A.qn));
+        B.hq = q8_uniform(q8_query(B.q, B.qn));
+
+        if (tid == 0) {
+            sm->count[0] = sm->count[1] = 0;
+            sm->seeds[0] = sm->seeds[1] = 0;
+            sm->rescored = 0;
+        }
+        __syncthreads();
+        auto start = [&](Mine& m, const Q8PairArg& arg, const SampleRaw& raw, int n_sample, float left, unsigned long long nbhd_raw, int* s_seeds) {
+            if (arg.cutoff_ready) {
+                m.cutoff = left;
+            } else {
+                const Sample sample = sample_finish(raw, arg.epoch);
+                m.cutoff = q8_cutoff_from_sample<kBlock>(sample, n_sample, topk, arg.n_seed < 0, m.hq, s_seeds, s_sel, reinterpret_cast<int*>(m.s_cand));
+            }
+            m.thr = 0;
+            if (const uint32_t nbv = untag_value(nbhd_raw, arg.epoch)) {
+                m.thr = (static_cast<uint64_t>(nbv) << 32) - 1ull;
+                if (m.hq.ok) {
+                    const float nb_cut = ordered_to_score(nbv) - m.hq.margin;
+                    m.cutoff = nb_cut > m.cutoff ? nb_cut : m.cutoff;
+                }
+            }
+            m.cutoff = q8_uniform(m.cutoff);
+            m.thr = q8_uniform(m.thr);
+            m.cut_d = q8_uniform(q8_threshold(m.cutoff));
+            m.n_rescored = 0;
+        };
+        start(A, args.a[0], raw_a, n_sample_a, left_a, nbhd_raw_a, &sm->seeds[0]);
+        __syncthreads();
+        start(B, args.a[1], raw_b, n_sample_b, left_b, nbhd_raw_b, &sm->seeds[1]);
+        int compact_at = 2 * topk > 256 ? 2 * topk : 256;
+        if (compact_at > kPairCandLimit) compact_at = kPairCandLimit;
+
+        auto append = [&](Mine& m, int64_t exclude_global, bool have, const Row& row, int64_t r) {
+            const float s = cosine_score(m.q, m.qn, row);
+            const int64_t g = row_base + r;
+            uint64_t key = pack_key(s, static_cast<uint32_t>(g));
+            if (g == exclude_global) key = 0;
+            const bool pass = have && key > m.thr;
+            const uint64_t ballot = __ballot(pass);
+            if (ballot) {
+                int base = 0;
+                if (lane == 0) base = atomicAdd(m.s_count, __popcll(ballot));
+                base = __builtin_amdgcn_readfirstlane(base);
+                const int pos = base + lanes_below(ballot);
+                if (pass) m.s_cand[pos] = key;
+            }
+        };
+        Row pend;
+        pend.a = pend.b = pend.c = make_float4(0.0f, 0.0f, 0.0f, 0.0f);
+        int64_t pend_r = 0;
+        uint32_t pend_for = 0u;
+        auto score_row = [&](uint32_t who, const Row& row, int64_t r) {
+            if (__ballot((who & 1u) != 0u)) append(A, args.a[0].exclude_global, (who & 1u) != 0u, row, r);
+            if (__ballot((who & 2u) != 0u)) append(B, args.a[1].exclude_global, (who & 2u) != 0u, row, r);
+        };
+        auto consume = [&]() {
+            if (__ballot(pend_for != 0u)) score_row(pend_for, pend, pend_r);
+            pend_for = 0u;
+        };
+        auto fetch = [&](uint32_t mask_a, uint32_t mask_b, int64_t r0) {
+            const uint32_t both = mask_a | mask_b;
+            if (!__ballot(both != 0u)) return;
+            auto whose = [&](int u) { return ((mask_a >> u) & 1u) | (((mask_b >> u) & 1u) << 1); };
+            auto count = [&](uint32_t who) {
+                A.n_rescored += __popcll(__ballot((who & 1u) != 0u));
+                B.n_rescored += __popcll(__ballot((who & 2u) != 0u));
+            };
+            const int first = both ? __builtin_ctz(both) : 0;
+            pend_r = r0 + first;
+            pend = load_row(feats, both ? pend_r : static_cast<int64_t>(0));
+            pend_for = both ? whose(first) : 0u;
+            count(pend_for);
+            uint32_t rest = both & (both - 1u);
+            while (__ballot(rest != 0u)) {
+                const int u = rest ? __builtin_ctz(rest) : 0;
+                const uint32_t who = rest ? whose(u) : 0u;
+                count(who);
+                const Row extra = load_row(feats, rest ? r0 + u : static_cast<int64_t>(0));
+                score_row(who, extra, r0 + u);
+                rest &= rest - 1u;
+            }
+        };
+        auto tighten = [&](Mine& m) {
+            const uint64_t local_thr = compact_candidates<kBlock, Cfg::kCandPerThread>(m.s_cand, m.s_count, topk, false, s_sel);
+            if (local_thr > m.thr) {
+                m.thr = q8_uniform(local_thr);
+                if (m.hq.ok) {
+                    const float local_cut = ordered_to_score(static_cast<uint32_t>(m.thr >> 32)) - m.hq.margin;
+                    m.cutoff = q8_uniform(local_cut > m.cutoff ? local_cut : m.cutoff);
+                    m.cut_d = q8_uniform(q8_threshold(m.cutoff));
+                }
+            }
+        };
+
+        auto process_tile = [&](const HalfTile& t, int it) {
+            const int64_t quad = quad_begin + static_cast<int64_t>(it) * quad_stride;
+            const int64_t r0 = quad * 4;
+            uint32_t hit_a = 0u, hit_b = 0u;
+            {
+                int a[4];
+                bool special[4];
+                q8_dot4(A.hq, t, a, special);
+    #pragma unroll
+                for (int u = 0; u < 4; ++u) hit_a |= (special[u] | (a[u] >= A.cut_d)) ? (1u << u) : 0u;
+                q8_dot4(B.hq, t, a, special);
+    #pragma unroll
+                for (int u = 0; u < 4; ++u) hit_b |= (special[u] | (a[u] >= B.cut_d)) ? (1u << u) : 0u;
+            }
+            const uint64_t maybe = __ballot((hit_a | hit_b) != 0u);
+            consume();
+            if (maybe) {
+                const int64_t left = n - r0;
+                const int valid = quad < n_quads ? (left < 4 ? static_cast<int>(left) : 4) : 0;
+                const uint32_t inside = (1u << valid) - 1u;
+                fetch(hit_a & inside, hit_b & inside, r0);
+            }
+            __syncthreads();
+            const int ca = *A.s_count, cb = *B.s_count;
+            __syncthreads();
+            if (ca >= compact_at) tighten(A);
+            if (cb >= compact_at) tighten(B);
+        };
+
+        for (int it = 0; it < iters; it += kDepth) {
+    #pragma unroll
+            for (int sidx = 0; sidx < kDepth; ++sidx) {
+                load_tile(ring[(sidx + kDepth - 1) % kDepth], it + sidx + kDepth - 1);
+                if (it + sidx < iters) process_tile(ring[sidx], it + sidx);
+            }
+        }
+        consume();
+
+        if (lane == 0 && A.n_rescored + B.n_rescored) atomicAdd(&sm->rescored, A.n_rescored + B.n_rescored);
+        __syncthreads();
+        if (tid == 0) rescored[bid] += static_cast<unsigned long long>(sm->rescored);
+        auto finish = [&](Mine& m, uint64_t* block_lists) {
+            if (*m.s_count > kRankCountMax && *m.s_count > topk)
+                compact_candidates<kBlock, Cfg::kCandPerThread>(m.s_cand, m.s_count, topk, false, s_sel);
+            __syncthreads();
+            block_rank_and_store<kBlock>(m.s_cand, *m.s_count, block_lists + static_cast<int64_t>(bid) * topk, topk);
+            __syncthreads();
+        };
+        finish(A, args.a[0].block_lists);
+        finish(B, args.a[1].block_lists);
+        return;
+    }
+
+    int dig_hi[kGroupMax][3], dig_lo[kGroupMax][3], cut_d[kGroupMax], cut_hi[kGroupMax];
+#pragma unroll
+    for (int x = 0; x < kGroupMax; ++x) {
+        dig_hi[x][0] = dig_hi[x][1] = dig_hi[x][2] = 0;
+        dig_lo[x][0] = dig_lo[x][1] = dig_lo[x][2] = 0;
+        cut_d[x] = cut_hi[x] = 0x7fffffff;
+    }
 
     constexpr int kDepth = Cfg::kDepth;
-    const unsigned long long nbhd_raw_a = arg_a.seed_vals[kNbhdSlot], nbhd_raw_b = arg_b.seed_vals[kNbhdSlot];
-    float left_a = 0.0f, left_b = 0.0f;
-    SampleRaw raw_a, raw_b;
-#pragma unroll
-    for (int r = 0; r < kHalfSeedPerThread; ++r) raw_a.t[r] = raw_b.t[r] = 0ull;
-    const int n_sample_a = arg_a.n_seed < 0 ? -arg_a.n_seed : arg_a.n_seed, n_sample_b = arg_b.n_seed < 0 ? -arg_b.n_seed : arg_b.n_seed;
-    if (arg_a.cutoff_ready) left_a = untag_cutoff(*arg_a.cutoff_ready, arg_a.epoch);
-    else raw_a = sample_request<kBlock>(arg_a.seed_vals, n_sample_a);
-    if (arg_b.cutoff_ready) left_b = untag_cutoff(*arg_b.cutoff_ready, arg_b.epoch);
-    else raw_b = sample_request<kBlock>(arg_b.seed_vals, n_sample_b);
+    unsigned long long nbhd_raw[kGroupMax];
+    float left[kGroupMax];
+#pragma unroll
+    for (int x = 0; x < kGroupMax; ++x) {
+        nbhd_raw[x] = 0ull;
+        left[x] = 0.0f;
+        if (x < nq) {
+            const Q8PairArg& arg = args.a[x];
+            nbhd_raw[x] = arg.seed_vals[kNbhdSlot];
+            if (arg.cutoff_ready) left[x] = untag_cutoff(*arg.cutoff_ready, arg.epoch);
+        }
+    }
     HalfTile ring[kDepth];
 #pragma unroll
     for (int d = 0; d < kDepth - 1; ++d) load_tile(ring[d], d);
-    q8_load_query(arg_a.query_ptr, arg_a.qarg.q, A.q);
-    q8_load_query(arg_b.query_ptr, arg_b.qarg.q, B.q);
-    A.qn = q8_uniform(query_norm(A.q));
-    B.qn = q8_uniform(query_norm(B.q));
-    A.hq = q8_uniform(q8_query(A.q, A.qn));
-    B.hq = q8_uniform(q8_query(B.q, B.qn));
+    float qf[kGroupMax][kDim];
+#pragma unroll
+    for (int x = 0; x < kGroupMax; ++x) {
+#pragma unroll
+        for (int j = 0; j < kDim; ++j) qf[x][j] = 0.0f;
+        if (x < nq) q8_load_query(args.a[x].query_ptr, args.a[x].qarg.q, qf[x]);
+    }
 
     if (tid == 0) {
-        sm->count[0] = sm->count[1] = 0;
-        sm->seeds[0] = sm->seeds[1] = 0;
+#pragma unroll
+        for (int x = 0; x < kGroupMax; ++x) sm->count[x] = sm->seeds[x] = 0;
         sm->rescored = 0;
     }
     __syncthreads();
-    auto start = [&](Mine& m, const Q8PairArg& arg, const SampleRaw& raw, int n_sample, float left, unsigned long long nbhd_raw, int* s_seeds) {
-        if (arg.cutoff_ready) {
-            m.cutoff = left;
-        } else {
-            const Sample sample = sample_finish(raw, arg.epoch);
-            m.cutoff = q8_cutoff_from_sample<kBlock>(sample, n_sample, topk, arg.n_seed < 0, m.hq, s_seeds, s_sel, reinterpret_cast<int*>(m.s_cand));
-        }
-        m.thr = 0;
-        if (const uint32_t nbv = untag_value(nbhd_raw, arg.epoch)) {
-            m.thr = (static_cast<uint64_t>(nbv) << 32) - 1ull;
-            if (m.hq.ok) {
-                const float nb_cut = ordered_to_score(nbv) - m.hq.margin;
-                m.cutoff = nb_cut > m.cutoff ? nb_cut : m.cutoff;
-            }
-        }
-        m.cutoff = q8_uniform(m.cutoff);
-        m.thr = q8_uniform(m.thr);
-        m.cut_d = q8_uniform(q8_threshold(m.cutoff));
-        m.n_rescored = 0;
-    };
-    start(A, arg_a, raw_a, n_sample_a, left_a, nbhd_raw_a, &sm->seeds[0]);
+#pragma unroll
+    for (int x = 0; x < kGroupMax; ++x) {
+        if (x < nq) {
+            const Q8PairArg& arg = args.a[x];
+            const float (&q)[kDim] = qf[x];
+            const float qn = q8_uniform(query_norm(q));
+            const Q8Query hq = q8_uniform(q8_query(q, qn));
+            float cutoff;
+            if (arg.cutoff_ready) {
+                cutoff = left[x];
+            } else {
+                const int n_sample = arg.n_seed < 0 ? -arg.n_seed : arg.n_seed;
+                const Sample sample = sample_finish(sample_request<kBlock>(arg.seed_vals, n_sample), arg.epoch);
+                cutoff = q8_cutoff_from_sample<kBlock>(sample, arg.n_seed < 0 ? -arg.n_seed : arg.n_seed, topk, arg.n_seed < 0, hq,
+                                                       &sm->seeds[x], s_sel, reinterpret_cast<int*>(sm->cand[x]));
+            }
+            uint64_t thr = 0;
+            if (const uint32_t nbv = untag_value(nbhd_raw[x], arg.epoch)) {
+                thr = (static_cast<uint64_t>(nbv) << 32) - 1ull;
+                if (hq.ok) {
+                    const float nb_cut = ordered_to_score(nbv) - hq.margin;
+                    cutoff = nb_cut > cutoff ? nb_cut : cutoff;
+                }
+            }
+            cutoff = q8_uniform(cutoff);
+            thr = q8_uniform(thr);
+#pragma unroll
+            for (int j = 0; j < 3; ++j) {
+                dig_hi[x][j] = hq.hi[j];
+                dig_lo[x][j] = hq.lo[j];
+            }
+            cut_d[x] = q8_uniform(q8_threshold(cutoff));
+            const int low_bound = q8_uniform(q8_low_bound(hq));
+            cut_hi[x] = q8_hi_threshold(cut_d[x], low_bound);
+            if (tid == 0) {
+                Q8GroupCold& c = sm->cold[x];
+#pragma unroll
+                for (int j = 0; j < kDim; ++j) c.q[j] = q[j];
+                c.qn = qn;
+                c.margin = hq.margin;
+                c.cutoff = cutoff;
+                c.ok = hq.ok ? 1 : 0;
+                c.thr = thr;
+                c.exclude_global = arg.exclude_global;
+                c.block_lists = arg.block_lists;
+                c.cut_d = cut_d[x];
+                c.low_bound = low_bound;
+            }
+            if (!arg.cutoff_ready) __syncthreads();
+        }
+    }
     __syncthreads();
-    start(B, arg_b, raw_b, n_sample_b, left_b, nbhd_raw_b, &sm->seeds[1]);
     int compact_at = 2 * topk > 256 ? 2 * topk : 256;
     if (compact_at > kPairCandLimit) compact_at = kPairCandLimit;
-
-    auto append = [&](Mine& m, int64_t exclude_global, bool have, const Row& row, int64_t r) {
-        const float s = cosine_score(m.q, m.qn, row);
+    int n_rescored = 0;
+
+    auto append = [&](int x, bool have, const Row& row, int64_t r) {
+        const Q8GroupCold& c = sm->cold[x];
+        const float4* const cq = reinterpret_cast<const float4*>(c.q);
+        const float4 q0 = cq[0], q1 = cq[1], q2 = cq[2];
+        const float q[kDim] = {q0.x, q0.y, q0.z, q0.w, q1.x, q1.y, q1.z, q1.w, q2.x, q2.y, q2.z, q2.w};
+        const float s = cosine_score(q, c.qn, row);
         const int64_t g = row_base + r;
         uint64_t key = pack_key(s, static_cast<uint32_t>(g));
-        if (g == exclude_global) key = 0;
-        const bool pass = have && key > m.thr;
+        if (g == c.exclude_global) key = 0;
+        const bool pass = have && key > c.thr;
         const uint64_t ballot = __ballot(pass);
         if (ballot) {
             int base = 0;
-            if (lane == 0) base = atomicAdd(m.s_count, __popcll(ballot));
+            if (lane == 0) base = atomicAdd(&sm->count[x], __popcll(ballot));
             base = __builtin_amdgcn_readfirstlane(base);
             const int pos = base + lanes_below(ballot);
-            if (pass) m.s_cand[pos] = key;
+            if (pass) sm->cand[x][pos] = key;
         }
     };
     Row pend;
@@ -938,75 +1191,140 @@
     int64_t pend_r = 0;
     uint32_t pend_for = 0u;
     auto score_row = [&](uint32_t who, const Row& row, int64_t r) {
-        if (__ballot((who & 1u) != 0u)) append(A, arg_a.exclude_global, (who & 1u) != 0u, row, r);
-        if (__ballot((who & 2u) != 0u)) append(B, arg_b.exclude_global, (who & 2u) != 0u, row, r);
+#pragma unroll 1
+        for (int x = 0; x < nq; ++x)
+            if (__ballot(((who >> x) & 1u) != 0u)) append(x, ((who >> x) & 1u) != 0u, row, r);
     };
     auto consume = [&]() {
         if (__ballot(pend_for != 0u)) score_row(pend_for, pend, pend_r);
         pend_for = 0u;
     };
-    auto fetch = [&](uint32_t mask_a, uint32_t mask_b, int64_t r0) {
-        const uint32_t both = mask_a | mask_b;
-        if (!__ballot(both != 0u)) return;
-        auto whose = [&](int u) { return ((mask_a >> u) & 1u) | (((mask_b >> u) & 1u) << 1); };
+    auto fetch = [&](uint32_t w, int64_t r0) {
+        if (!__ballot(w != 0u)) return;
         auto count = [&](uint32_t who) {
-            A.n_rescored += __popcll(__ballot((who & 1u) != 0u));
-            B.n_rescored += __popcll(__ballot((who & 2u) != 0u));
+#pragma unroll
+            for (int x = 0; x < kGroupMax; ++x) n_rescored += __popcll(__ballot(((who >> x) & 1u) != 0u));
         };
-        const int first = both ? __builtin_ctz(both) : 0;
+        const int first = w ? (__builtin_ctz(w) >> 2) : 0;
         pend_r = r0 + first;
-        pend = load_row(feats, both ? pend_r : static_cast<int64_t>(0));
-        pend_for = both ? whose(first) : 0u;
+        pend = load_row(feats, w ? pend_r : static_cast<int64_t>(0));
+        pend_for = (w >> (4 * first)) & 0xfu;
         count(pend_for);
-        uint32_t rest = both & (both - 1u);
+        uint32_t rest = w & ~(0xfu << (4 * first));
         while (__ballot(rest != 0u)) {
-            const int u = rest ? __builtin_ctz(rest) : 0;
-            const uint32_t who = rest ? whose(u) : 0u;
+            const int u = rest ? (__builtin_ctz(rest) >> 2) : 0;
+            const uint32_t who = rest ? (rest >> (4 * u)) & 0xfu : 0u;
             count(who);
             const Row extra = load_row(feats, rest ? r0 + u : static_cast<int64_t>(0));
             score_row(who, extra, r0 + u);
-            rest &= rest - 1u;
+            rest &= ~(0xfu << (4 * u));
         }
     };
-    auto tighten = [&](Mine& m) {
-        const uint64_t local_thr = compact_candidates<kBlock, Cfg::kCandPerThread>(m.s_cand, m.s_count, topk, false, s_sel);
-        if (local_thr > m.thr) {
-            m.thr = q8_uniform(local_thr);
-            if (m.hq.ok) {
-                const float local_cut = ordered_to_score(static_cast<uint32_t>(m.thr >> 32)) - m.hq.margin;
-                m.cutoff = q8_uniform(local_cut > m.cutoff ? local_cut : m.cutoff);
-                m.cut_d = q8_uniform(q8_threshold(m.cutoff));
-            }
+    auto tighten = [&](int x) {
+        Q8GroupCold& c = sm->cold[x];
+        const uint64_t thr = c.thr;
+        const float cutoff = c.cutoff, margin = c.margin;
+        const bool ok = c.ok != 0;
+        const int low_bound = c.low_bound;
+        const uint64_t local_thr = compact_candidates<kBlock, Cfg::kCandPerThread>(sm->cand[x], &sm->count[x], topk, false, s_sel);
+        if (local_thr > thr) {
+            float cut = cutoff;
+            int cd = 0;
+            if (ok) {
+                const float local_cut = ordered_to_score(static_cast<uint32_t>(local_thr >> 32)) - margin;
+                cut = local_cut > cutoff ? local_cut : cutoff;
+                cd = q8_uniform(q8_threshold(cut));
+#pragma unroll
+                for (int k = 0; k < kGroupMax; ++k) {
+                    cut_d[k] = k == x ? cd : cut_d[k];
+                    cut_hi[k] = k == x ? q8_hi_threshold(cd, low_bound) : cut_hi[k];
+                }
+            }
+            if (tid == 0) {
+                c.thr = local_thr;
+                if (ok) {
+                    c.cutoff = cut;
+                    c.cut_d = cd;
+                }
+            }
+            __syncthreads();
         }
     };
 
     auto process_tile = [&](const HalfTile& t, int it) {
         const int64_t quad = quad_begin + static_cast<int64_t>(it) * quad_stride;
         const int64_t r0 = quad * 4;
-        uint32_t hit_a = 0u, hit_b = 0u;
-        {
-            int a[4];
-            bool special[4];
-            q8_dot4(A.hq, t, a, special);
-#pragma unroll
-            for (int u = 0; u < 4; ++u) hit_a |= (special[u] | (a[u] >= A.cut_d)) ? (1u << u) : 0u;
-            q8_dot4(B.hq, t, a, special);
-#pragma unroll
-            for (int u = 0; u < 4; ++u) hit_b |= (special[u] | (a[u] >= B.cut_d)) ? (1u << u) : 0u;
-        }
-        const uint64_t maybe = __ballot((hit_a | hit_b) != 0u);
+        bool hit[kGroupMax][4];
+        bool some = false;
+#pragma unroll
+        for (int x = 0; x < kGroupMax; ++x) {
+#pragma unroll
+            for (int u = 0; u < 4; ++u) hit[x][u] = false;
+            if (x < 2 || x < nq) {
+                Q8Query hq;
+#pragma unroll
+                for (int j = 0; j < 3; ++j) {
+                    hq.hi[j] = dig_hi[x][j];
+                    hq.lo[j] = dig_lo[x][j];
+                }
+                if constexpr (kQ8QueryBits == 16) {
+                    const uint32_t first[4] = {t.t0.x, t.t0.w, t.t1.z, t.t2.y};
+                    const uint32_t second[4] = {t.t0.y, t.t1.x, t.t1.w, t.t2.z};
+                    const uint32_t third[4] = {t.t0.z, t.t1.y, t.t2.x, t.t2.w};
+                    int H[4];
+                    bool pre[4], special[4];
+#pragma unroll
+                    for (int u = 0; u < 4; ++u) {
+                        special[u] = (first[u] & 0xffu) == kQ8Special;
+                        H[u] = __builtin_amdgcn_sdot4(static_cast<int>(first[u]), hq.hi[0], 0, false);
+                        H[u] = __builtin_amdgcn_sdot4(static_cast<int>(second[u]), hq.hi[1], H[u], false);
+                        H[u] = __builtin_amdgcn_sdot4(static_cast<int>(third[u]), hq.hi[2], H[u], false);
+                        pre[u] = special[u] | (H[u] >= cut_hi[x]);
+                    }
+                    if (__ballot(pre[0] | pre[1] | pre[2] | pre[3])) {
+#pragma unroll
+                        for (int u = 0; u < 4; ++u) {
+                            int L = __builtin_amdgcn_sdot4(static_cast<int>(first[u]), hq.lo[0], 0, false);
+                            L = __builtin_amdgcn_sdot4(static_cast<int>(second[u]), hq.lo[1], L, false);
+                            L = __builtin_amdgcn_sdot4(static_cast<int>(third[u]), hq.lo[2], L, false);
+                            hit[x][u] = special[u] | ((H[u] << 8) + L >= cut_d[x]);
+                            some |= hit[x][u];
+                        }
+                    }
+                } else {
+                    int a[4];
+                    bool special[4];
+                    q8_dot4(hq, t, a, special);
+#pragma unroll
+                    for (int u = 0; u < 4; ++u) {
+                        hit[x][u] = special[u] | (a[u] >= cut_d[x]);
+                        some |= hit[x][u];
+                    }
+                }
+            }
+        }
         consume();
-        if (maybe) {
-            const int64_t left = n - r0;
-            const int valid = quad < n_quads ? (left < 4 ? static_cast<int>(left) : 4) : 0;
-            const uint32_t inside = (1u << valid) - 1u;
-            fetch(hit_a & inside, hit_b & inside, r0);
+        if (__ballot(some)) {
+            const int64_t rows_left = n - r0;
+            const int valid = quad < n_quads ? (rows_left < 4 ? static_cast<int>(rows_left) : 4) : 0;
+            const uint32_t inside = (1u << (4 * valid)) - 1u;
+            uint32_t w = 0u;
+#pragma unroll
+            for (int x = 0; x < kGroupMax; ++x)
+#pragma unroll
+                for (int u = 0; u < 4; ++u) w |= hit[x][u] ? (1u << (4 * u + x)) : 0u;
+            fetch(w & inside, r0);
         }
         __syncthreads();
-        const int ca = *A.s_count, cb = *B.s_count;
+        int c[kGroupMax];
+#pragma unroll
+        for (int x = 0; x < kGroupMax; ++x) c[x] = sm->count[x];
         __syncthreads();
-        if (ca >= compact_at) tighten(A);
-        if (cb >= compact_at) tighten(B);
+        if ((c[0] >= compact_at) | (c[1] >= compact_at) | (c[2] >= compact_at) | (c[3] >= compact_at)) {
+#pragma unroll
+            for (int x = 0; x < kGroupMax; ++x)
+                if (c[x] >= compact_at) tighten(x);
+        }
     };
 
     for (int it = 0; it < iters; it += kDepth) {
@@ -1018,18 +1336,17 @@
     }
     consume();
 
-    if (lane == 0 && A.n_rescored + B.n_rescored) atomicAdd(&sm->rescored, A.n_rescored + B.n_rescored);
+    if (lane == 0 && n_rescored) atomicAdd(&sm->rescored, n_rescored);
     __syncthreads();
     if (tid == 0) rescored[bid] += static_cast<unsigned long long>(sm->rescored);
-    auto finish = [&](Mine& m, uint64_t* block_lists) {
-        if (*m.s_count > kRankCountMax && *m.s_count > topk)
-            compact_candidates<kBlock, Cfg::kCandPerThread>(m.s_cand, m.s_count, topk, false, s_sel);
+#pragma unroll 1
+    for (int x = 0; x < nq; ++x) {
+        if (sm->count[x] > kRankCountMax && sm->count[x] > topk)
+            compact_candidates<kBlock, Cfg::kCandPerThread>(sm->cand[x], &sm->count[x], topk, false, s_sel);
         __syncthreads();
-        block_rank_and_store<kBlock>(m.s_cand, *m.s_count, block_lists + static_cast<int64_t>(bid) * topk, topk);
+        block_rank_and_store<kBlock>(sm->cand[x], sm->count[x], sm->cold[x].block_lists + static_cast<int64_t>(bid) * topk, topk);
         __syncthreads();
-    };
-    finish(A, arg_a.block_lists);
-    finish(B, arg_b.block_lists);
-}
-
-}
+    }
+}
+
+}
diff --git a/spotify_recommender_amd/csrc/stream_groups.h b/spotify_recommender_amd/csrc/stream_groups.h
--- /dev/null
+++ b/spotify_recommender_amd/csrc/stream_groups.h
@@ -0,0 +1,79 @@
+#pragma once
+
+#include <cstdint>
+
+namespace mi355 {
+
+constexpr int kGroupMax = 4;
+constexpr int kGroupFirstMax = 2;
+
+enum GroupStepKind {
+    kGroupLaunch,
+    kGroupPromote,
+    kGroupMerge,
+    kGroupSingle,
+};
+
+struct GroupStep {
+    int kind;
+    int n;
+    int n_next;
+    bool sampled;
+};
+
+struct GroupSteps {
+    int count = 0;
+    GroupStep step[6];
+    void push(int kind, int n, int n_next = 0, bool sampled = false) { step[count++] = GroupStep{kind, n, n_next, sampled}; }
+};
+
+struct StreamGroups {
+    int n_wait = 0;
+    int n_form = 0;
+    int n_pend = 0;
+    bool later = false;
+    uint64_t key = 0;
+
+    bool open() const { return n_wait > 0 || n_form > 0 || n_pend > 0; }
+
+    void close(GroupSteps& out) {
+        const bool launch = n_wait > 0;
+        if (launch) {
+            out.push(kGroupLaunch, n_wait, n_form);
+            n_pend = n_wait;
+        }
+        out.push(kGroupPromote, n_form, 0, launch);
+        n_wait = n_form;
+        n_form = 0;
+        later = true;
+    }
+
+    void drain(GroupSteps& out) {
+        if (n_form >= 2) close(out);
+        if (n_wait > 0) {
+            out.push(kGroupLaunch, n_wait, 0);
+            n_pend = n_wait;
+            n_wait = 0;
+        }
+        if (n_pend > 0) {
+            out.push(kGroupMerge, n_pend);
+            n_pend = 0;
+        }
+        if (n_form == 1) {
+            out.push(kGroupSingle, 1);
+            n_form = 0;
+        }
+        later = false;
+    }
+
+    void add(uint64_t k, int cap_later, GroupSteps& out) {
+        if (n_form > 0 && k != key) drain(out);
+        key = k;
+        ++n_form;
+        int cap = later ? cap_later : kGroupFirstMax;
+        cap = cap < 2 ? 2 : (cap > kGroupMax ? kGroupMax : cap);
+        if (n_form >= cap) close(out);
+    }
+};
+
+}
```
